# ChenWu98/cycle-diffusion

Measured on AMD Instinct MI355X. Metric: images/sec, SD-v1.4 512px CycleDiffusion 100+100 steps, 1/2/4/8 MI355X, higher is better.
Workload: dtype fp16; 1 GPU; C2: Stable-Diffusion-v1.4-shaped U-Net + KL-f8 VAE, 512x512, custom_steps=99 white_box_steps=100 eta=0.1 skip 0, 1 trial, encoder scale 1, decoder CFG 3; batch_per_gpu=4, global_batch=4, parallelism=dp1, steps_per_launch_set=5, launch_set_cap=16, launch_sets_in_flight_per_gpu=1, images_in_flight_per_gpu=20, distributed=single process, weights=synthetic(seed=0)

## Files before the change

cycle-diffusion_amd/_ffi.py:

```python
import ctypes as C
import os

import numpy as np

_HERE = os.path.dirname(os.path.abspath(__file__))
LIB_PATH = os.path.join(_HERE, "lib", "libcyclediff.so")

CD_NET_UNET_OPENAI, CD_NET_UNET_HO, CD_NET_VAE_KL, CD_NET_CLIP_TEXT, CD_NET_BERT_XTR = 1, 2, 3, 4, 5
CD_NET_OCLIP_TEXT, CD_NET_OCLIP_VISION, CD_NET_INCEPTION_FID = 6, 7, 8
CD_SCHED_DDIM, CD_SCHED_DDPM = 0, 1
CD_PREC_16, CD_PREC_F32, CD_PREC_F32X3 = 0, 1, 2
CD_MASK_QSAMPLE, CD_MASK_ENCODER = 0, 1
MASK_SOURCES = {"q_sample": CD_MASK_QSAMPLE, "encoder": CD_MASK_ENCODER}
ACT_NONE, ACT_SILU, ACT_GELU, ACT_GEGLU, ACT_QGELU, ACT_RELU = 0, 1, 2, 3, 4, 5


class NetDesc(C.Structure):
    _fields_ = [
        ("kind", C.c_int), ("image_size", C.c_int), ("in_channels", C.c_int), ("out_channels", C.c_int),
        ("model_channels", C.c_int), ("num_res_blocks", C.c_int),
        ("n_mult", C.c_int), ("channel_mult", C.c_int * 8),
        ("n_attn", C.c_int), ("attn", C.c_int * 8),
        ("num_heads", C.c_int), ("num_head_channels", C.c_int),
        ("use_spatial_transformer", C.c_int), ("context_dim", C.c_int), ("transformer_depth", C.c_int),
        ("use_scale_shift_norm", C.c_int), ("resblock_updown", C.c_int), ("conv_resample", C.c_int),
        ("z_channels", C.c_int), ("embed_dim", C.c_int), ("double_z", C.c_int),
        ("precision", C.c_int), ("n_embed", C.c_int), ("reserved", C.c_int * 6),
    ]


class StepCoef(C.Structure):
    _fields_ = [("sa", C.c_float), ("s1a", C.c_float), ("sap", C.c_float), ("dirc", C.c_float),
                ("sigma", C.c_float), ("r", C.c_float), ("t_mask", C.c_float), ("t", C.c_int32)]


STEP_COEF_DTYPE = np.dtype([("sa", "<f4"), ("s1a", "<f4"), ("sap", "<f4"), ("dirc", "<f4"), ("sigma", "<f4"),
                            ("r", "<f4"), ("t_mask", "<f4"), ("t", "<i4")])

_VP, _I, _F, _U64, _SZ, _I64 = C.c_void_p, C.c_int, C.c_float, C.c_uint64, C.c_size_t, C.c_int64

SIGNATURES = {
    "cd_last_error": [],
    "cd_version": [],
    "cd_act_format": [],
    "cd_engine_create": [_VP, _SZ, C.POINTER(_VP)],
    "cd_engine_destroy": [_VP],
    "cd_engine_synchronize": [_VP],
    "cd_engine_workspace_high_water": [_VP, C.POINTER(_SZ)],
    "cd_prof_enable": [_VP, _I],
    "cd_prof_collect": [_VP, C.POINTER(_I), C.POINTER(C.c_double), C.POINTER(C.c_double)],
    "cd_net_create": [_VP, C.POINTER(NetDesc), C.POINTER(_I)],
    "cd_net_param_count": [_VP, _I, C.POINTER(_I)],
    "cd_net_param_info": [_VP, _I, _I, C.c_char_p, _I, C.POINTER(_I), C.POINTER(_I64)],
    "cd_net_load_param": [_VP, _I, C.c_char_p, _VP, _I, C.POINTER(_I64)],
    "cd_net_missing_params": [_VP, _I, C.POINTER(_I), C.c_char_p, _I],
    "cd_unet_forward": [_VP, _I, _VP, _VP, _VP, _I, _I, _VP],
    "cd_text_encode": [_VP, _I, _VP, _I, _I, _VP],
    "cd_clip_text_features": [_VP, _I, _VP, _I, _I, _VP],
    "cd_clip_image_features": [_VP, _I, _VP, _I, _VP],
    "cd_inception_features": [_VP, _I, _VP, _I, _I, _VP],
    "cd_vae_encode": [_VP, _I, _VP, _VP, _U64, _I, _I, _I, _F, _VP],
    "cd_vae_decode": [_VP, _I, _VP, _I, _I, _F, _F, _F, _VP],
    "cd_dpm_encode": [_VP, _I, _I, _VP, _VP, _VP, _I, _F, _I, _I, _VP, _VP, _U64, _I, _VP],
    "cd_ddim_decode": [_VP, _I, _I, _VP, _I, _I, _VP, _VP, _I, _F, _I, _I, _VP, _VP, _U64, _VP],
    "cd_ddim_decode_v": [_VP, _I, _I, _VP, _I, _I, _VP, _VP, _I, _VP, _I, _I, _VP, _VP, _U64, _VP],
    "cd_ddim_invert": [_VP, _I, _I, _VP, _VP, _VP, _I, _F, _I, _I, _VP, _VP, _VP],
    "cd_cycle_translate": [_VP, _I, _I, _VP, _VP, _VP, _F, _VP, _VP, _F, _VP, _I, _I, _I, _I, _VP, _VP, _VP, _U64, _I, _VP,
                           _VP],
    "cd_ddim_decode_masked": [_VP, _I, _I, _VP, _I, _I, _VP, _VP, _I, _F, _VP, _I, _I, _VP, _VP, _U64, _VP, _VP, _I, _I, _VP, _VP,
                              _U64, _VP],
    "cd_cycle_translate_masked": [_VP, _I, _I, _VP, _VP, _VP, _F, _VP, _VP, _F, _VP, _I, _I, _I, _I, _VP, _VP, _VP, _U64, _I,
                                  _VP, _VP, _I, _I, _VP, _VP, _U64, _VP, _VP],
    "cd_pix_refine": [_VP, _I, _I, _VP, _I, _I, _VP, _VP, _U64],
    "cd_op_pack_conv_weight": [_VP, _VP, _I, _I, _I, _I, _I, C.POINTER(_VP), C.POINTER(_I), C.POINTER(_I)],
    "cd_op_free": [_VP, _VP],
    "cd_op_conv2d": [_VP, _VP, _I, _VP, _I, _I, _I, _I, _VP, _I, _I, _I, _I, _I, _I, _I, _VP, _VP, _VP, _I, _I, _VP],
    "cd_op_conv2d_16": [_VP, _VP, _I, _VP, _I, _I, _I, _I, _VP, _I, _I, _I, _I, _I, _I, _I, _VP, _VP, _VP, _I, _I, _VP,
                        _VP],
    "cd_op_last_gemm_config": [_VP] + [C.POINTER(_I)] * 5,
    "cd_op_groupnorm": [_VP, _VP, _I, _I, _I, _I, _I, _F, _VP, _VP, _VP, _I, _VP],
    "cd_op_layernorm": [_VP, _VP, _I, _I, _VP, _VP, _F, _VP],
    "cd_op_attention": [_VP, _VP, _VP, _VP, _I, _I, _I, _I, _I, _F, _I, _VP],
    "cd_op_softmax_rows": [_VP, _VP, _I64, _I, _VP],
    "cd_op_timestep_embedding": [_VP, _VP, _I, _I, _I, _VP],
    "cd_op_sched_step": [_VP, _I, _I, _VP, _VP, _VP, _VP, _I, _F, _VP, _VP, _I, _I, _I, _I, _VP],
    "cd_op_sched_step_masked": [_VP, _I, _VP, _VP, _VP, _I, _F, _VP, _VP, _VP, _I, _I, _F, _F, _VP, _I, _I, _I, _I, _VP, _I],
    "cd_op_bench_conv": [_VP, _I, _I, _I, _I, _I, _I, _I, _I, _I, _I, _I, _I, C.POINTER(C.c_float)],
    "cd_op_bench_mfma_sustained": [_VP, _I, C.POINTER(C.c_float), C.POINTER(C.c_float)],
    "cd_op_probe": [_VP, _I, _VP, _VP, _SZ],
}
_RESTYPES = {"cd_last_error": C.c_char_p}

_lib = None


class EngineError(RuntimeError):
    pass


def load_library(build_if_missing=True):
    global _lib
    if _lib is not None:
        return _lib
    if not os.path.exists(LIB_PATH):
        if not build_if_missing:
            raise EngineError("libcyclediff.so has not been built: run `python -c 'import __graft_entry__ as g; g.build()'`")
        import importlib.util
        spec = importlib.util.spec_from_file_location("_cd_build", os.path.join(_HERE, "build.py"))
        mod = importlib.util.module_from_spec(spec)
        spec.loader.exec_module(mod)
        mod.build()
    os.environ.setdefault("CYCLEDIFF_TUNE_DEFAULT", os.path.join(_HERE, "tune_gfx950.txt"))
    lib = C.CDLL(os.environ.get("CYCLEDIFF_LIB") or LIB_PATH)
    for name, args in SIGNATURES.items():
        fn = getattr(lib, name)
        fn.argtypes = args
        fn.restype = _RESTYPES.get(name, C.c_int)
    _lib = lib
    return lib


def check(rc):
    if rc != 0:
        raise EngineError(load_library().cd_last_error().decode("utf-8", "replace"))


def ptr(t):
    if t is None:
        return None
    if not t.is_contiguous():
        raise EngineError("tensor crossing the C ABI must be contiguous")
    return C.c_void_p(t.data_ptr())


def coef_array(rows):
    arr = np.zeros(len(rows), dtype=STEP_COEF_DTYPE)
    for i, r in enumerate(rows):
        arr[i] = tuple(r)
    return arr
```

cycle-diffusion_amd/csrc/capi.hip:

```cpp
#include <stdlib.h>
#include <string.h>
#include <unistd.h>

#include <algorithm>

#include "engine.h"

using namespace cd;

struct StepPacer {
  static constexpr int kAhead = 2, kRing = kAhead + 1;
  hipEvent_t ev[kRing] = {nullptr, nullptr, nullptr};
  long n = 0;
  bool enabled = true;
  void init() {
    const char* e = getenv("CYCLEDIFF_HOST_PACING");
    enabled = !(e && e[0] == '0');
    for (auto& x : ev) HIP_CHECK(hipEventCreateWithFlags(&x, hipEventBlockingSync | hipEventDisableTiming));
  }
  static void sleep_until_done(hipEvent_t e) {
    for (;;) {
      const hipError_t q = hipEventQuery(e);
      if (q == hipSuccess) return;
      if (q != hipErrorNotReady) HIP_CHECK(q);
// ... 698 lines not shown
    CD_CHECK(Dc > 0 && ctx_len > 0, "network has no cross-attention but a context was given");
    const size_t esz = f32 ? 4 : 2, per = (size_t)ctx_len * Dc;
    char* cx = (char*)h->arena.alloc((size_t)Bn * per * esz);
    auto put = [&](const float* src, int rows, size_t row0) {
      if (f32) HIP_CHECK(hipMemcpyAsync(cx + row0 * per * 4, src, (size_t)rows * per * 4, hipMemcpyDeviceToDevice, h->st));
      else launch_nchw_to_nhwc(h->st, src, (bf16_t*)cx + row0 * per, rows * ctx_len, Dc, 1, Dc, 1.f, 0.f, 0);
    };
    if (ge.cfg) { put(enc_ctx_uc, B, 0); put(enc_ctx_c, B, B); } else put(ge.ctx_single, B, 0);
    if (gd.cfg) { put(dec_ctx_uc, Bd, Ben); put(dec_ctx_c, Bd, Ben + Bd); } else put(gd.ctx_single, Bd, Ben);
    u->set_context(c, (const bf16_t*)cx, Bn, ctx_len);
  } else {
    CD_CHECK(u->desc.context_dim <= 0 || !u->desc.use_spatial_transformer, "network expects a cross-attention context");
  }
  const size_t esz = f32 ? 4 : 2;
  const int64_t chw = (int64_t)C * HW, n = (int64_t)B * chw;
  float* xt_e = (float*)h->arena.alloc((size_t)B * chw * 4);
  float* xt_d = (float*)h->arena.alloc((size_t)Bd * chw * 4);
  char* xin = (char*)h->arena.alloc((size_t)Bn * HW * cpad * esz);
  HIP_CHECK(hipMemsetAsync(xin, 0, (size_t)Bn * HW * cpad * esz, h->st));
  float* eh = (float*)h->arena.alloc((size_t)Bn * HW * out_ld * 4);
  const size_t row_in = (size_t)HW * cpad * esz;
  bf16_t* xin_e = f32 ? nullptr : (bf16_t*)xin;
  bf16_t* xin_d = f32 ? nullptr : (bf16_t*)(xin + (size_t)Ben * row_in);
  EpsHat eh_e, eh_d;
  eh_e.p = eh; eh_e.sb = (int64_t)HW * out_ld; eh_e.sc = 1; eh_e.sp = out_ld; eh_e.cfg = ge.cfg ? 1 : 0; eh_e.g = enc_guidance;
  eh_d = eh_e; eh_d.p = eh + (int64_t)Ben * HW * out_ld; eh_d.cfg = gd.cfg ? 1 : 0; eh_d.g = dec_guidance;
  eh_d.gvec = dec_guidance_per_sample;
  StepCoef* tab_e = upload_coef(h, coef_enc_host, K + 1);
  StepCoef* tab_d = upload_coef(h, coef_dec_host, K);
  const int64_t zbs = (int64_t)(K + 1) * chw;
  launch_init_xt(h->st, x0, noise, seed, 0u, xt_e, z_out, zbs, B, C, HW, tab_e, K, xin_e, cpad, ge.cfg ? 1 : 0);
  for (int j = 0; j < n_dec; ++j)
    HIP_CHECK(hipMemcpyAsync(xt_d + (int64_t)j * n, xt_e, (size_t)n * 4, hipMemcpyDeviceToDevice, h->st));
  const float2* qtab = nullptr;
  if (mk && mk->source == CD_MASK_QSAMPLE) qtab = (const float2*)upload_table(h, mk->qcoef_host, (size_t)K * 2 * sizeof(float));
  auto blend_of = [&](int k, int slot) {
    MaskBlend b = mask_blend_of(*mk, qtab, k, slot, (int64_t)Bd * chw);
    if (mk->source == CD_MASK_ENCODER) { b.src = xt_e; b.src_bmod = B; }
    return b;
  };
  if (mk) launch_mask_blend_init(h->st, xt_d, blend_of(K - 1, 0), Bd, C, HW, xin_d, cpad, gd.cfg ? 1 : 0);
  else if (!f32) launch_nchw_to_nhwc(h->st, xt_d, xin_d, Bd, C, HW, cpad, 1.f, 0.f, gd.cfg ? 1 : 0);
  const int dup_tail = (gd.cfg && !ge.cfg) ? Bd : 0;
  for (int i = 0; i < K; ++i) {
    const int k = K - 1 - i;
    if (f32) {
      float* xf = (float*)xin;
      launch_nchw_to_nhwc_f32(h->st, xt_e, xf, B, C, HW, cpad, 1.f, 0.f, u->x3 ? 1 : 0, h->overflow_dev);
      if (ge.cfg) launch_nchw_to_nhwc_f32(h->st, xt_e, xf + (size_t)B * HW * cpad, B, C, HW, cpad, 1.f, 0.f, u->x3 ? 1 : 0, h->overflow_dev);
      float* xd = xf + (size_t)Ben * HW * cpad;
      launch_nchw_to_nhwc_f32(h->st, xt_d, xd, Bd, C, HW, cpad, 1.f, 0.f, u->x3 ? 1 : 0, h->overflow_dev);
      if (gd.cfg) launch_nchw_to_nhwc_f32(h->st, xt_d, xd + (size_t)Bd * HW * cpad, Bd, C, HW, cpad, 1.f, 0.f, u->x3 ? 1 : 0, h->overflow_dev);
    }
    UNetIO io;
    io.xin = (const bf16_t*)xin; io.B = Bn; io.tab = tab_d; io.step = k; io.t_shared = true;
    io.dup_tail = dup_tail;
    io.out = eh; io.out_ld = out_ld;
    u->forward(c, io);
    const int is_last = (last_uses_x0 && k == 0) ? 1 : 0;
    const float* nz = (noise && !is_last) ? noise + (int64_t)(1 + i) * n : nullptr;
    float* zslot = z_out + (1 + i) * chw;
    launch_encode_step(h->st, sched_kind, x0, xt_e, eh_e, nz, seed, (uint32_t)(1 + i), zslot, zbs, B, C, HW, tab_e, nullptr, k,
                       is_last, xin_e, cpad, ge.cfg ? 1 : 0);
    if (mk)
      launch_decode_step_masked(h->st, xt_d, eh_d, zslot, zbs, nullptr, seed, (uint32_t)(0x1000 + i), Bd, C, HW, tab_d, nullptr, k,
                                xin_d, cpad, gd.cfg ? 1 : 0, n_dec > 1 ? B : 0, blend_of(k - 1, i + 1), k > 0 ? 1 : 0);
    else
    launch_decode_step(h->st, sched_kind, xt_d, eh_d, zslot, zbs, nullptr, seed, (uint32_t)(0x1000 + i), Bd, C, HW, tab_d,
                       nullptr, k, xin_d, cpad, gd.cfg ? 1 : 0, nullptr, n_dec > 1 ? B : 0);
    h->pacer.tick(h->st);
  }
  HIP_CHECK(hipMemcpyAsync(x_out, xt_d, (size_t)Bd * chw * 4, hipMemcpyDeviceToDevice, h->st));
}

int cd_cycle_translate(cd_handle h, int net, int sched_kind, const float* x0, const float* enc_ctx_c,
                       const float* enc_ctx_uc, float enc_guidance, const float* dec_ctx_c, const float* dec_ctx_uc,
                       float dec_guidance, const float* dec_guidance_per_sample, int ctx_len, int B, int n_dec, int K,
                       const cd_step_coef* coef_enc_host, const cd_step_coef* coef_dec_host, const float* noise,
                       uint64_t seed, int last_uses_x0, float* z_out, float* x_out) {
  CD_API_BEGIN
  enter_engine(h);
  cycle_translate_impl(h, net, sched_kind, x0, enc_ctx_c, enc_ctx_uc, enc_guidance, dec_ctx_c, dec_ctx_uc, dec_guidance,
                       dec_guidance_per_sample, ctx_len, B, n_dec, K, coef_enc_host, coef_dec_host, noise, seed, last_uses_x0,
                       z_out, x_out, nullptr);
  CD_API_END
}

int cd_cycle_translate_masked(cd_handle h, int net, int sched_kind, const float* x0, const float* enc_ctx_c,
                              const float* enc_ctx_uc, float enc_guidance, const float* dec_ctx_c, const float* dec_ctx_uc,
                              float dec_guidance, const float* dec_guidance_per_sample, int ctx_len, int B, int n_dec, int K,
                              const cd_step_coef* coef_enc_host, const cd_step_coef* coef_dec_host, const float* noise,
                              uint64_t seed, int last_uses_x0, const float* mask, const float* mask_x0, int B_mask,
                              int mask_source, const float* qsample_coef_host, const float* mask_noise, uint64_t mask_seed,
                              float* z_out, float* x_out) {
  CD_API_BEGIN
  enter_engine(h);
  MaskArgs mk;
  mk.mask = mask; mk.x0 = mask_x0; mk.B_mask = B_mask; mk.source = mask_source; mk.qcoef_host = qsample_coef_host;
  mk.noise = mask_noise; mk.seed = mask_seed;
  cycle_translate_impl(h, net, sched_kind, x0, enc_ctx_c, enc_ctx_uc, enc_guidance, dec_ctx_c, dec_ctx_uc, dec_guidance,
                       dec_guidance_per_sample, ctx_len, B, n_dec, K, coef_enc_host, coef_dec_host, noise, seed, last_uses_x0,
                       z_out, x_out, &mk);
  CD_API_END
}

int cd_pix_refine(cd_handle h, int net, int sched_kind, float* x, int B, int R, const cd_step_coef* coef_host,
                  const float* noise, uint64_t seed) {
  CD_API_BEGIN
  enter_engine(h);
  CD_CHECK(h && x && coef_host && B > 0 && R > 0, "bad argument");
  ArenaScope arena_scope(h->arena);
  SamplerState s = setup_sampler(h, net, nullptr, nullptr, 0, 1.f, B);
  s.tab = upload_coef(h, coef_host, R + 1);
  const int64_t n = (int64_t)B * s.C * s.HW;
  launch_init_xt(h->st, x, noise, seed, 0x2000u, s.xt, nullptr, 0, B, s.C, s.HW, s.tab, R, s.xin16(), s.cpad, 0);
  for (int i = 0; i < R; ++i) {
    const int k = R - 1 - i;
    run_unet(h, s, k);
    const float* nz = noise ? noise + (int64_t)(1 + i) * n : nullptr;
    launch_decode_step(h->st, sched_kind, s.xt, s.ehv, nullptr, 0, nz, seed, (uint32_t)(0x2001 + i), B, s.C,
                       s.HW, s.tab, nullptr, k, s.xin16(), s.cpad, 0, nullptr);
    h->pacer.tick(h->st);
  }
  HIP_CHECK(hipMemcpyAsync(x, s.xt, (size_t)n * 4, hipMemcpyDeviceToDevice, h->st));
  CD_API_END
}

int cd_op_pack_conv_weight(cd_handle h, const float* w_host, int N, int Cin, int KH, int KW, int geglu,
                           void** packed_dev, int* Npad, int* Cpad) {
  CD_API_BEGIN
  enter_engine(h);
  CD_CHECK(h && w_host && packed_dev, "bad argument");
  static int counter = 0;
  ConvW* c = h->op_params.new_conv(N, Cin, KH, KW, false, geglu != 0);
  const std::string name = "op." + std::to_string(counter++);
  h->op_params.conv_weight(name, c);
  int64_t shape[4] = {N, Cin, KH, KW};
  h->op_params.load(h->st, name, w_host, 4, shape);
  *packed_dev = c;
  if (Npad) *Npad = c->Npad;
  if (Cpad) *Cpad = c->Cpad;
  CD_API_END
}

int cd_op_free(cd_handle, void*) { return 0; }

static void op_conv2d(cd_handle h, const float* x0, int C0, const float* x1, int C1, int B, int H, int W,
                      const void* packed_w, int N, int KH, int KW, int stride, int pad, int asym_pad, int up,
                      const float* bias, const float* rowvec, const float* resid, int act, int tile, bool out16,
                      float* y, float* stats) {
  CD_CHECK(h && x0 && packed_w && y, "bad argument");
  ArenaScope arena_scope(h->arena);
  Ctx c = h->ctx();
  ConvW w = *(const ConvW*)packed_w;
  CD_CHECK(w.N == N && w.KH == KH && w.KW == KW, "packed weight does not match the call");
  w.b = const_cast<float*>(bias);
  const int c0p = x1 ? C0 : round_up(C0, 32);
  Act a0 = alloc_act(c, B, H, W, c0p);
  launch_nchw_to_nhwc(h->st, x0, a0.p, B, C0, H * W, c0p, 1.f, 0.f, 0);
  Act a1;
  if (x1) {
    a1 = alloc_act(c, B, H, W, C1);
    launch_nchw_to_nhwc(h->st, x1, a1.p, B, C1, H * W, C1, 1.f, 0.f, 0);
  }
  ConvOpts o; o.stride = stride; o.pad = pad; o.asym = asym_pad != 0; o.up = up != 0; o.tile = tile;
  if (act & 0x400) {
    CD_CHECK(out16 && conv_ln_fold_available(c, w, (int64_t)B * H * W) , "LayerNorm fold needs tile 30 shapes");
    o.ln_fold = true;
    act &= ~0x400;
  }
  o.act = act;
  o.out_f32 = !out16;
  o.want_stats = stats != nullptr;
  const int Hin = up ? 2 * H : H, Win = up ? 2 * W : W;
  const int Ho = asym_pad ? (Hin + 1 - KH) / stride + 1 : (Hin + 2 * pad - KH) / stride + 1;
  const int Wo = asym_pad ? (Win + 1 - KW) / stride + 1 : (Win + 2 * pad - KW) / stride + 1;
  const int Nout = w.geglu ? N / 2 : N;
  if (rowvec) { o.rowvec = rowvec; o.rowvec_ld = N; o.rows_per_vec = Ho * Wo; }
  Act r;
  if (resid) {
    r = alloc_act(c, B, Ho, Wo, Nout);
    launch_nchw_to_nhwc(h->st, resid, r.p, B, Nout, Ho * Wo, Nout, 1.f, 0.f, 0);
    o.resid = &r;
  }
  Act out = conv_fwd(c, w, a0, x1 ? &a1 : nullptr, o);
  launch_nhwc_to_nchw(h->st, out.p, out16 ? 0 : 1, out.ld, y, B, Nout, Ho * Wo, 1.f, 0.f);
  if (stats) {
    CD_CHECK(out.stats, "this convolution produces no GroupNorm statistics (GEGLU, or rows %% 32 != 0)");
    HIP_CHECK(hipMemcpyAsync(stats, out.stats, (size_t)(out.rows() / 32) * 2 * Nout * sizeof(float),
                             hipMemcpyDeviceToDevice, h->st));
  }
}

int cd_op_conv2d(cd_handle h, const float* x0, int C0, const float* x1, int C1, int B, int H, int W,
                 const void* packed_w, int N, int KH, int KW, int stride, int pad, int asym_pad, int up,
                 const float* bias, const float* rowvec, const float* resid, int act, int tile, float* y) {
  CD_API_BEGIN
  enter_engine(h);
  op_conv2d(h, x0, C0, x1, C1, B, H, W, packed_w, N, KH, KW, stride, pad, asym_pad, up, bias, rowvec, resid, act, tile,
            false, y, nullptr);
  CD_API_END
}

int cd_op_conv2d_16(cd_handle h, const float* x0, int C0, const float* x1, int C1, int B, int H, int W,
                    const void* packed_w, int N, int KH, int KW, int stride, int pad, int asym_pad, int up,
                    const float* bias, const float* rowvec, const float* resid, int act, int tile, float* y,
                    float* stats) {
  CD_API_BEGIN
  enter_engine(h);
  op_conv2d(h, x0, C0, x1, C1, B, H, W, packed_w, N, KH, KW, stride, pad, asym_pad, up, bias, rowvec, resid, act, tile,
            true, y, stats);
  CD_API_END
}

int cd_op_last_gemm_config(cd_handle h, int* tile_id, int* bk, int* splitk, int* chm, int* tile_group) {
  CD_API_BEGIN
  CD_CHECK(h, "bad argument");
  const GemmLaunchInfo li = conv_gemm_last_launch();
  if (tile_id) *tile_id = li.tile_id;
  if (bk) *bk = li.bk;
  if (splitk) *splitk = li.splitk;
  if (chm) *chm = li.chm;
  if (tile_group) *tile_group = li.tile_group;
  CD_API_END
}

int cd_op_groupnorm(cd_handle h, const float* x, int B, int C, int H, int W, int G, float eps,
                    const float* gamma, const float* beta, const float* film, int silu, float* y) {
  CD_API_BEGIN
  enter_engine(h);
  CD_CHECK(h && x && y && G == 32, "bad argument (G must be 32)");
  ArenaScope arena_scope(h->arena);
  Ctx c = h->ctx();
  Act a = alloc_act(c, B, H, W, C);
  launch_nchw_to_nhwc(h->st, x, a.p, B, C, H * W, C, 1.f, 0.f, 0);
  GNW w; w.g = const_cast<float*>(gamma); w.b = const_cast<float*>(beta); w.C = C; w.eps = eps;
  Act o = groupnorm_fwd(c, w, a, nullptr, silu != 0, film, film ? 2 * C : 0);
  launch_nhwc_to_nchw(h->st, o.p, 0, o.ld, y, B, C, H * W, 1.f, 0.f);
  CD_API_END
}

int cd_op_layernorm(cd_handle h, const float* x, int rows, int C, const float* gamma, const float* beta,
                    float eps, float* y) {
  CD_API_BEGIN
  enter_engine(h);
  CD_CHECK(h && x && y, "bad argument");
  ArenaScope arena_scope(h->arena);
  bf16_t* a = (bf16_t*)h->arena.alloc((size_t)rows * C * 2);
  bf16_t* o = (bf16_t*)h->arena.alloc((size_t)rows * C * 2);
  launch_nchw_to_nhwc(h->st, x, a, rows, C, 1, C, 1.f, 0.f, 0);
  launch_layernorm(h->st, a, C, o, C, rows, C, gamma, beta, eps);
  launch_nhwc_to_nchw(h->st, o, 0, C, y, rows, C, 1, 1.f, 0.f);
  CD_API_END
}

int cd_op_attention(cd_handle h, const float* q, const float* k, const float* v, int B, int H, int Tq,
                    int Tk, int D, float scale, int use_transpose_kernel, float* o) {
  CD_API_BEGIN
  enter_engine(h);
  CD_CHECK(h && q && k && v && o, "bad argument");
  ArenaScope arena_scope(h->arena);
  const int C = H * D, Tpad = round_up(Tk, 64);
  bf16_t* qb = (bf16_t*)h->arena.alloc((size_t)B * Tq * C * 2);
  bf16_t* kb = (bf16_t*)h->arena.alloc((size_t)B * Tk * C * 2);
  bf16_t* vb = (bf16_t*)h->arena.alloc((size_t)B * Tk * C * 2);
  bf16_t* ob = (bf16_t*)h->arena.alloc((size_t)B * Tq * C * 2);
  launch_nchw_to_nhwc(h->st, q, qb, B * Tq, C, 1, C, 1.f, 0.f, 0);
  launch_nchw_to_nhwc(h->st, k, kb, B * Tk, C, 1, C, 1.f, 0.f, 0);
  launch_nchw_to_nhwc(h->st, v, vb, B * Tk, C, 1, C, 1.f, 0.f, 0);
  AttnParams p;
  p.q = qb; p.k = kb; p.o = ob; p.B = B; p.H = H; p.Tq = Tq; p.Tk = Tk; p.D = D;
  p.ldq = C; p.ldk = C; p.ldo = C; p.q_bs = (int64_t)Tq * C; p.k_bs = (int64_t)Tk * C; p.o_bs = (int64_t)Tq * C;
  p.scale = scale;
  if (use_transpose_kernel) {
    bf16_t* vt = (bf16_t*)h->arena.alloc((size_t)B * C * Tpad * 2);
    launch_transpose_v(h->st, vb, C, (int64_t)Tk * C, vt, B, H, Tk, D, D, Tpad);
    p.vt = vt; p.vt_dpad = D; p.vt_tpad = Tpad;
  } else {
    p.v = vb; p.ldv = C; p.v_bs = (int64_t)Tk * C;
  }
  launch_attention(h->st, p);
  launch_nhwc_to_nchw(h->st, ob, 0, C, o, B * Tq, C, 1, 1.f, 0.f);
  CD_API_END
}

int cd_op_softmax_rows(cd_handle h, const float* s, int64_t rows, int cols, float* p) {
  CD_API_BEGIN
  enter_engine(h);
  CD_CHECK(h && s && p, "bad argument");
  ArenaScope arena_scope(h->arena);
  bf16_t* pb = (bf16_t*)h->arena.alloc((size_t)rows * cols * 2);
  launch_softmax_rows(h->st, s, cols, pb, cols, rows, cols);
  launch_nhwc_to_nchw(h->st, pb, 0, cols, p, (int)rows, cols, 1, 1.f, 0.f);
  CD_API_END
}

int cd_op_timestep_embedding(cd_handle h, const float* t, int B, int dim, int mode, float* out) {
  CD_API_BEGIN
  enter_engine(h);
  CD_CHECK(h && t && out, "bad argument");
  launch_timestep_embedding(h->st, nullptr, nullptr, 0, t, out, B, dim, mode);
  CD_API_END
}

int cd_op_sched_step(cd_handle h, int mode, int sched_kind, const cd_step_coef* coef_host, const float* x0,
                     float* xt, const float* eps_hat, int cfg, float guidance, const float* noise,
                     const float* eps_in, int is_last, int B, int C, int HW, float* z_slot) {
  CD_API_BEGIN
  enter_engine(h);
  CD_CHECK(h && coef_host && xt, "bad argument");
  ArenaScope arena_scope(h->arena);
  StepCoef* tab = upload_coef(h, coef_host, 1);
  const int64_t chw = (int64_t)C * HW;
  EpsHat eh; eh.p = eps_hat; eh.sb = chw; eh.sc = HW; eh.sp = 1; eh.cfg = cfg; eh.g = guidance;
  if (mode == 0) {
    launch_init_xt(h->st, x0, noise, 0, 0, xt, z_slot, chw, B, C, HW, tab, 0, nullptr, 0, 0);
  } else if (mode == 1) {
    launch_encode_step(h->st, sched_kind, x0, xt, eh, noise, 0, 0, z_slot, chw, B, C, HW, tab, nullptr, 0,
                       is_last, nullptr, 0, 0);
  } else {
    launch_decode_step(h->st, sched_kind, xt, eh, eps_in, chw, noise, 0, 0, B, C, HW, tab, nullptr, 0, nullptr,
                       0, 0, nullptr);
  }
  HIP_CHECK(hipStreamSynchronize(h->st));
  CD_API_END
}

int cd_op_sched_step_masked(cd_handle h, int mode, const cd_step_coef* coef_host, float* x, const float* eps_hat, int cfg,
                            float guidance, const float* eps_in, const float* mask, const float* src, int B_mask,
                            int mask_source, float qa, float qb, const float* mask_noise, int blend, int B, int C, int HW,
                            void* xin16_out, int cfg_dup) {
  CD_API_BEGIN
  enter_engine(h);
  CD_CHECK(h && x && mask && src && B > 0 && C > 0 && HW > 0, "bad argument");
  CD_CHECK(B_mask > 0 && B % B_mask == 0, "mask shape mismatch: %d mask rows for a batch of %d", B_mask, B);
  CD_CHECK(mode == 0 || (coef_host && eps_hat), "bad argument");
  ArenaScope arena_scope(h->arena);
  const int64_t chw = (int64_t)C * HW;
  MaskBlend mk;
  mk.mask = mask; mk.src = src; mk.mask_bmod = mk.src_bmod = B_mask; mk.noise = mask_noise;
  if (mask_source == CD_MASK_QSAMPLE) {
    CD_CHECK(mask_noise, "q_sample mode needs the noise tensor here");
    const float q[2] = {qa, qb};
    mk.qtab = (const float2*)upload_table(h, q, sizeof(q));
  }
  if (mode == 0) {
    launch_mask_blend_init(h->st, x, mk, B, C, HW, (bf16_t*)xin16_out, C, cfg_dup);
  } else {
    StepCoef* tab = upload_coef(h, coef_host, 1);
    EpsHat eh; eh.p = eps_hat; eh.sb = chw; eh.sc = HW; eh.sp = 1; eh.cfg = cfg; eh.g = guidance;
    launch_decode_step_masked(h->st, x, eh, eps_in, chw, nullptr, 0, 0, B, C, HW, tab, nullptr, 0, (bf16_t*)xin16_out, C,
                              cfg_dup, 0, mk, blend);
  }
  HIP_CHECK(hipStreamSynchronize(h->st));
  CD_API_END
}

}

namespace {
__global__ void k_probe_mfma(float* out) {
  const int lane = threadIdx.x & 63;
  bf16x8 a = {0, 0, 0, 0, 0, 0, 0, 0}, b = {0, 0, 0, 0, 0, 0, 0, 0};
  f32x16 acc;
// ... 167 lines not shown
```

cycle-diffusion_amd/csrc/conv_gemm.hip:

```cpp
#include <stdio.h>
#include <stdlib.h>
#include <string.h>

#include <algorithm>
#include <map>
#include <mutex>
#include <string>

#include "common.h"
#include "kernels.h"

namespace cd {

namespace gemm_detail {

#ifndef CD_EPI_STORE_AUX
#define CD_EPI_STORE_AUX 0
#endif
#ifndef CD_EPI_RESID_AUX
#define CD_EPI_RESID_AUX 0
#endif

typedef const __attribute__((address_space(1))) void* gptr_t;
typedef __attribute__((address_space(3))) void* lptr_t;

template <int BM, int BN, int BK, int WM, int WN, int NSTAGE>
struct TileCfg {
  static constexpr int NW = WM * WN;
  static constexpr int CPR = BK / 8;
  static constexpr int RPI = 64 / CPR;
  static constexpr int A_IPW = BM / RPI / NW;
  static constexpr int B_IPW = BN / RPI / NW;
  static constexpr int LPT = A_IPW + B_IPW;
  static constexpr int TM = BM / WM, TN = BN / WN;
  static constexpr int MT = TM / 32, NT = TN / 32;
  static constexpr int KS = BK / 16;
  static constexpr int SWZ_SHIFT = (CPR == 8) ? 1 : 2;
  static constexpr int CW = TN >= 64 ? 64 : TN;
  static constexpr int EPI_LD = CW + 4;
  static constexpr int PF = (MT * NT >= 8) ? 1 : 2;
  static constexpr int A_BYTES = BM * BK * 2, B_BYTES = BN * BK * 2;
  static constexpr int STAGE_BYTES = A_BYTES + B_BYTES;
  static constexpr int EPI_BYTES = NW * TM * EPI_LD * 4;
  static constexpr int LDS_BYTES = STAGE_BYTES * NSTAGE > EPI_BYTES ? STAGE_BYTES * NSTAGE : EPI_BYTES;
  static constexpr int TAB_BIAS_I = (BN / 4 + 63) / 64;
  static constexpr int TAB_RV_I = ((BM / 32) * (BN / 4) + 63) / 64;
  static constexpr bool HAS_TAB = LDS_BYTES + (TAB_BIAS_I + TAB_RV_I) * 1024 <= 160 * 1024;
  static constexpr int TAB_BYTES = HAS_TAB ? (TAB_BIAS_I + TAB_RV_I) * 1024 : 0;
  static_assert(NW == 4 || NW == 8 || NW == 16, "4, 8 or 16 waves");
  static_assert(A_IPW >= 1 && B_IPW >= 1, "tile too small for the wave count");
  static_assert(A_IPW * RPI * NW == BM && B_IPW * RPI * NW == BN, "tile rows must split evenly over waves");
  static_assert(MT >= 1 && NT >= 1, "wave tile");
  static_assert(NSTAGE >= 2 && NSTAGE <= 8, "ring depth");
  static_assert((NSTAGE - 2) * LPT <= 63, "vmcnt field");
  static_assert(LDS_BYTES + TAB_BYTES <= 160 * 1024, "LDS");
};

template <int N>
__device__ __forceinline__ void wait_vmcnt_barrier() {
  asm volatile("s_waitcnt vmcnt(%0)\n\ts_barrier" ::"n"(N) : "memory");
}

#ifdef CD_PROBE
__device__ __forceinline__ unsigned long long probe_time() {
  unsigned long long t;
  asm volatile("s_memtime %0\n\ts_waitcnt lgkmcnt(0)" : "=s"(t)::"memory");
  return t;
}
__device__ __forceinline__ unsigned long long probe_realtime() {
  unsigned long long t;
  asm volatile("s_memrealtime %0\n\ts_waitcnt lgkmcnt(0)" : "=s"(t)::"memory");
  return t;
}
#define CD_PROBE_ONLY(...) __VA_ARGS__
#else
#define CD_PROBE_ONLY(...)
#endif

__device__ __forceinline__ __amdgpu_buffer_rsrc_t uniform_rsrc(const void* base, int bytes) {
  const uint64_t u = (uint64_t)base;
  const uint32_t lo = (uint32_t)__builtin_amdgcn_readfirstlane((int)(uint32_t)u);
  const uint32_t hi = (uint32_t)__builtin_amdgcn_readfirstlane((int)(uint32_t)(u >> 32));
  return __builtin_amdgcn_make_buffer_rsrc((void*)(((uint64_t)hi << 32) | lo), 0, __builtin_amdgcn_readfirstlane(bytes), 0x00020000);
}

__device__ __forceinline__ bool fast_epilogue(const ConvGemmParams& p) {
  return p.act == ACT_NONE && !p.out_f32 && !p.resid_f32 && (p.N & 7) == 0 && (p.out_ld & 7) == 0 &&
         (((uintptr_t)p.out | (uintptr_t)p.resid | (uintptr_t)p.rowvec) & 15) == 0 && (p.o_bs & 7) == 0 &&
         (!p.resid || (p.resid_ld & 7) == 0) &&
         (!p.rowvec || ((p.rowvec_ld & 3) == 0 && (p.rows_per_vec >= p.M || (p.rows_per_vec & 31) == 0)));
}

template <int BM, int BN, int BK, int WM, int WN, int NSTAGE, bool CHM = false>
__global__ __launch_bounds__(64 * WM * WN, (WM * WN == 4 && BK == 32 && NSTAGE == 3 && BM * BN >= 128 * 256) ? 2 : 1) void k_conv_gemm(ConvGemmParams p) {
#if defined(__HIP_DEVICE_COMPILE__)
  using T = TileCfg<BM, BN, BK, WM, WN, NSTAGE>;
  constexpr int CPR = T::CPR, RPI = T::RPI, A_IPW = T::A_IPW, B_IPW = T::B_IPW, NW = T::NW;
  constexpr int MT = T::MT, NT = T::NT, KS = T::KS, TM = T::TM, TN = T::TN, LPT = T::LPT;
  extern __shared__ __attribute__((aligned(16))) char smem[];

  const int tid = threadIdx.x;
  const int lane = tid & 63;
  const int wave = __builtin_amdgcn_readfirstlane(tid >> 6);
  const int wm = wave / WN, wn = wave % WN;
  if constexpr (WM * WN == 4 && BK == 32 && NSTAGE == 3 && BM * BN >= 128 * 256) {
    if (p.dephase_ticks > 0 && (int)(blockIdx.x + gridDim.x * (blockIdx.y + gridDim.y * blockIdx.z)) < 2 * p.num_cus) {
      unsigned hwid;
      asm volatile("s_getreg_b32 %0, hwreg(HW_REG_HW_ID)" : "=s"(hwid));
      if (tid == 0) *(volatile int*)smem = (int)(hwid & 1u);
      __syncthreads();
      const int odd = *(volatile int*)smem;
      __syncthreads();
      if (odd) {
        unsigned long long t0, t1;
        asm volatile("s_memtime %0\n\ts_waitcnt lgkmcnt(0)" : "=s"(t0)::"memory");
        do {
          __builtin_amdgcn_s_sleep(32);
          asm volatile("s_memtime %0\n\ts_waitcnt lgkmcnt(0)" : "=s"(t1)::"memory");
        } while ((long long)(t1 - t0) < (long long)p.dephase_ticks);
      }
    }
  }
  CD_PROBE_ONLY(
  const unsigned long long pr_rt0 = probe_realtime();
  unsigned long long pr_t0 = probe_time(), pr_prol = 0, pr_first = 0, pr_wait = 0, pr_comp = 0, pr_maxw = 0, pr_loop = 0,
                     pr_drain = 0, pr_stage = 0, pr_rows = 0, pr_issued = 0, pr_last = 0;
  unsigned* pr_log = (unsigned*)(smem + T::LDS_BYTES + T::TAB_BYTES) + wave * 64;
  if (lane < 64) pr_log[lane] = 0;)

  const int tiles_n = (p.N + BN - 1) / BN;
  const int tiles_m = (p.M + BM - 1) / BM;
  const int ntiles = tiles_m * tiles_n;
  int tile;
  {
    const int bid = blockIdx.x;
    const int q = ntiles >> 3, r = ntiles & 7;
    const int xcd = bid & 7, loc = bid >> 3;
    tile = (xcd < r ? xcd * (q + 1) : r * (q + 1) + (xcd - r) * q) + loc;
  }
  const bool nmajor = (int64_t)p.N * p.Ktot > (int64_t)p.B * p.Hs * p.Ws * (p.C0 + p.C1);
  int tm, tn;
  if (p.tile_group > 0) {
    const int width = p.tile_group * tiles_n;
    const int grp = tile / width, within = tile - grp * width;
    const int first_m = grp * p.tile_group;
    const int gsz = (tiles_m - first_m) < p.tile_group ? (tiles_m - first_m) : p.tile_group;
    tn = within / gsz; tm = first_m + (within - tn * gsz);
  } else if (nmajor) { tn = tile / tiles_m; tm = tile - tn * tiles_m; }
  else { tm = tile / tiles_n; tn = tile - tm * tiles_n; }
  const int m0 = tm * BM, n0 = tn * BN;
  const int zb = blockIdx.z;

  constexpr unsigned kRange = 0x7fffffffu, kInvalid = 0x80000000u;
  const int HWo = p.Hout * p.Wout;
  const bool pow2 = ((HWo & (HWo - 1)) == 0) && ((p.Wout & (p.Wout - 1)) == 0);
  const int sh_hw = 31 - __builtin_clz(HWo), sh_w = 31 - __builtin_clz(p.Wout);
  int b_first = pow2 ? (m0 >> sh_hw) : (m0 / HWo);
  CD_PROBE_ONLY(if (p.dbg & 4) b_first = 0;)
  const int64_t samp0 = (int64_t)b_first * p.Hs * p.Ws;
  const bf16_t* base0 = p.src0 + (int64_t)zb * p.a_bs + samp0 * p.ld0;
  const bf16_t* base1 = p.src1 ? p.src1 + (int64_t)zb * p.a_bs + samp0 * p.ld1 : base0;
  const __amdgpu_buffer_rsrc_t rsw =
      __builtin_amdgcn_make_buffer_rsrc((void*)(p.wgt + (int64_t)zb * p.w_bs), 0, kRange, 0x00020000);

  const int srow = lane / CPR;
  const int pchunk = lane % CPR;
  int a_iy0[A_IPW], a_ix0[A_IPW], a_boff[A_IPW], a_lc8[A_IPW];
  unsigned a_voff[A_IPW];
  unsigned a_mk[A_IPW], a_base[A_IPW];
#pragma unroll
  for (int i = 0; i < A_IPW; ++i) {
    const int row = (i * NW + wave) * RPI + srow;
    int m = m0 + row;
    CD_PROBE_ONLY(if (p.dbg & 4) m = (m0 & 0x3ff) + row;)
    a_lc8[i] = (pchunk ^ ((row >> T::SWZ_SHIFT) & (CPR - 1))) * 8;
    a_voff[i] = kInvalid;
    a_mk[i] = 0; a_base[i] = 0;
    if (m < p.M) {
      int b, oy, ox;
      if (pow2) {
        b = m >> sh_hw;
        const int rem = m & (HWo - 1);
        oy = rem >> sh_w; ox = rem & (p.Wout - 1);
      } else {
        b = m / HWo;
        const int rem = m - b * HWo;
        oy = rem / p.Wout; ox = rem - oy * p.Wout;
      }
      a_iy0[i] = oy * p.stride - p.pad_t;
      a_ix0[i] = ox * p.stride - p.pad_l;
      a_boff[i] = (b - b_first) * p.Hs * p.Ws;
    } else {
      a_iy0[i] = -(1 << 28);
      a_ix0[i] = 0;
      a_boff[i] = 0;
    }
    if constexpr (CHM) {
      unsigned mk = 0;
      for (int r = 0; r < p.KH; ++r) mk |= ((unsigned)(a_iy0[i] + r) < (unsigned)p.Hin ? 1u : 0u) << r;
      for (int q = 0; q < p.KW; ++q) mk |= ((unsigned)(a_ix0[i] + q) < (unsigned)p.Win ? 1u : 0u) << (8 + q);
      a_mk[i] = mk;
    }
  }
  unsigned b_voff[B_IPW];
#pragma unroll
  for (int i = 0; i < B_IPW; ++i) {
    const int row = (i * NW + wave) * RPI + srow;
    const int lchunk = pchunk ^ ((row >> T::SWZ_SHIFT) & (CPR - 1));
    int nrow = n0 + row;
    if (nrow >= p.N) nrow = p.N - 1;
    b_voff[i] = (unsigned)((nrow * (p.ldw ? p.ldw : p.Ktot) + lchunk * 8) * 2);
  }

  const int Ctot = p.C0 + p.C1;
  const int nk = p.Ktot / BK;
  const int nsplit = gridDim.y, sidx = blockIdx.y;
  const int kper = (nk + nsplit - 1) / nsplit;
  const int kt0 = sidx * kper;
  const int kt1 = (kt0 + kper < nk) ? kt0 + kper : nk;
  int kr, kss, kc;
  if constexpr (CHM) {
    const int ntaps = p.KH * p.KW;
    const int slice = kt0 / ntaps, tap = kt0 - slice * ntaps;
    kc = slice * BK;
    kr = tap / p.KW;
    kss = tap - kr * p.KW;
  } else {
    const int k_el = kt0 * BK;
    const int tap = k_el / Ctot;
    kc = k_el - tap * Ctot;
    kr = tap / p.KW;
    kss = tap - kr * p.KW;
  }
  bool st_force = true;

  char* As = smem;
  char* Bs = smem + NSTAGE * T::A_BYTES;

  bool st_live = false;
  int st_soffa = 0, st_soffb = 0;
  const bf16_t* st_base = base0;
  auto prepare = [&](int kt) {
    st_live = kt < kt1;
    const int c_kc = kc, c_kr = kr, c_kss = kss;
    if constexpr (CHM) {
      const bool wk = c_kss + 1 >= p.KW;
      const bool wr = wk && (c_kr + 1 >= p.KH);
      kss = wk ? 0 : c_kss + 1;
      kr = wr ? 0 : c_kr + (wk ? 1 : 0);
      kc = c_kc + (wr ? BK : 0);
      if (st_live) {
        const int ld = (c_kc < p.C0) ? p.ld0 : p.ld1;
        if (st_force || ((c_kr | c_kss) == 0 && (c_kc == 0 || c_kc == p.C0))) {
          st_force = false;
#pragma unroll
          for (int i = 0; i < A_IPW; ++i) {
            const int pix = a_boff[i] + a_iy0[i] * p.Ws + a_ix0[i];
            a_base[i] = (unsigned)((pix * ld + a_lc8[i]) * 2);
          }
        }
        const unsigned dt = (unsigned)((c_kr * p.Ws + c_kss) * ld * 2);
#pragma unroll
        for (int i = 0; i < A_IPW; ++i) {
          const unsigned ok = (a_mk[i] >> c_kr) & (a_mk[i] >> (8 + c_kss)) & 1u;
          a_voff[i] = ok ? a_base[i] + dt : kInvalid;
        }
      }
    } else {
      kc += BK;
      if (kc >= Ctot) {
        kc = 0;
        if (++kss >= p.KW) { kss = 0; ++kr; }
      }
      if (st_live && (c_kc == 0 || c_kc == p.C0 || st_force)) {
        st_force = false;
        const int ld = (c_kc < p.C0) ? p.ld0 : p.ld1;
#pragma unroll
        for (int i = 0; i < A_IPW; ++i) {
          int iy = a_iy0[i] + c_kr, ix = a_ix0[i] + c_kss;
          const bool ok = ((unsigned)iy < (unsigned)p.Hin) && ((unsigned)ix < (unsigned)p.Win);
          if (p.up) { iy >>= 1; ix >>= 1; }
          const int pix = a_boff[i] + iy * p.Ws + ix;
          a_voff[i] = ok ? (unsigned)((pix * ld + a_lc8[i]) * 2) : kInvalid;
        }
      }
    }
    const bool first = c_kc < p.C0;
    st_base = first ? base0 : base1;
    st_soffa = (first ? c_kc : c_kc - p.C0) * 2;
    st_soffb = st_live ? (CHM ? ((c_kr * p.KW + c_kss) * Ctot + c_kc) * 2 : kt * (BK * 2)) : 0;
  };
  auto issue = [&](int idx, int buf) {
    if (idx < A_IPW) {
      const __amdgpu_buffer_rsrc_t rsa = __builtin_amdgcn_make_buffer_rsrc((void*)st_base, 0, kRange, 0x00020000);
      char* l = As + buf * T::A_BYTES + ((idx * NW + wave) * RPI) * (BK * 2);
      __builtin_amdgcn_raw_ptr_buffer_load_lds(rsa, (lptr_t)l, 16, st_live ? a_voff[idx < A_IPW ? idx : 0] : kInvalid,
                                               st_soffa, 0, 0);
    } else {
      const int i = idx - A_IPW;
      char* l = Bs + buf * T::B_BYTES + ((i * NW + wave) * RPI) * (BK * 2);
      __builtin_amdgcn_raw_ptr_buffer_load_lds(rsw, (lptr_t)l, 16, st_live ? b_voff[i < B_IPW ? i : 0] : kInvalid,
                                               st_soffb, 0, 0);
    }
  };

  f32x16 acc[MT][NT];
#pragma unroll
  for (int i = 0; i < MT; ++i)
#pragma unroll
    for (int j = 0; j < NT; ++j)
#pragma unroll
      for (int r = 0; r < 16; ++r) acc[i][j][r] = 0.0f;

  const int frow = lane & 31;
  const int fhalf = lane >> 5;

  constexpr int PF = T::PF, SYNC = KS - PF, NMF = MT * NT, HALF = NMF / 2;
  constexpr int SPREAD = (NSTAGE == 2) ? 1 : KS;
  static_assert(SYNC >= 0 && (NSTAGE - 1) * LPT <= 63, "fragment prefetch depth / vmcnt field");
#pragma unroll
  for (int s = 0; s < NSTAGE; ++s) {
    prepare(kt0 + s);
#pragma unroll
    for (int l = 0; l < LPT; ++l) issue(l, s);
  }
  constexpr int TAB_N = T::TAB_BIAS_I + T::TAB_RV_I;
  constexpr int TABI = T::HAS_TAB ? (TAB_N + NW - 1) / NW : 0;
  if constexpr (TABI > 0) {
    const bool fe = fast_epilogue(p);
    const bool tb = (fe || p.act == ACT_GEGLU) && p.bias != nullptr;
    char* tab = smem + T::LDS_BYTES;
    const __amdgpu_buffer_rsrc_t rsb = __builtin_amdgcn_make_buffer_rsrc(
        (void*)(tb ? (const void*)p.bias : (const void*)p.wgt), 0, tb ? p.N * 4 : 0, 0x00020000);
    const __amdgpu_buffer_rsrc_t rsv = __builtin_amdgcn_make_buffer_rsrc(
        (void*)((fe && p.rowvec) ? (const void*)p.rowvec : (const void*)p.wgt), 0, (fe && p.rowvec) ? kRange : 0, 0x00020000);
    const unsigned rpv = (unsigned)p.rows_per_vec;
    const bool rpv_pow2 = (rpv & (rpv - 1)) == 0;
    const int rpv_sh = 31 - __builtin_clz(rpv | 1u);
#pragma unroll
    for (int i = 0; i < TABI; ++i) {
      const int j = (i * NW + wave) % TAB_N;
      if (j < T::TAB_BIAS_I) {
        const int c4 = j * 64 + lane;
// ... 364 lines not shown
            __builtin_amdgcn_raw_buffer_store_b128((u32x4e){pk.x, pk.y, pk.z, pk.w}, rs_o,
                                                   vo_out + (unsigned)((rb * 32 + ps * 16) * p.out_ld * 2), 0, 0);
          }
        }
        CD_PROBE_ONLY(pr_rows += probe_time() - pr_c1;)
        continue;
      }
      float bias_v[8];
#pragma unroll
      for (int e = 0; e < 8; ++e) bias_v[e] = (p.bias && e < nvalid) ? p.bias[n + e] : 0.0f;
      float ssum[8], ssq[8];
#pragma unroll
      for (int e = 0; e < 8; ++e) { ssum[e] = 0.f; ssq[e] = 0.f; }
      for (int r0 = 0; r0 < TM; r0 += rpp) {
        const int row = r0 + vr;
        const int m = m0 + wm * TM + row;
        if (row < TM && m < p.M && n < p.N) {
        float v[8];
        {
          const f32x4 lo = *(const f32x4*)(E + row * T::EPI_LD + col);
          const f32x4 hi = *(const f32x4*)(E + row * T::EPI_LD + col + 4);
          v[0] = lo[0]; v[1] = lo[1]; v[2] = lo[2]; v[3] = lo[3];
          v[4] = hi[0]; v[5] = hi[1]; v[6] = hi[2]; v[7] = hi[3];
        }
#pragma unroll
        for (int e = 0; e < 8; ++e) v[e] += bias_v[e];
        int on = n;
        if (geglu) {
          float gt[8];
          const f32x4 lo = *(const f32x4*)(E + row * T::EPI_LD + col + 32);
          const f32x4 hi = *(const f32x4*)(E + row * T::EPI_LD + col + 36);
          gt[0] = lo[0]; gt[1] = lo[1]; gt[2] = lo[2]; gt[3] = lo[3];
          gt[4] = hi[0]; gt[5] = hi[1]; gt[6] = hi[2]; gt[7] = hi[3];
#pragma unroll
          for (int e = 0; e < 8; ++e) {
            const float gg = gt[e] + (p.bias ? p.bias[n + 32 + e] : 0.0f);
            v[e] = v[e] * gelu_fast(gg);
          }
          on = (n / 64) * 32 + (n % 64);
        } else {
          if (p.rowvec) {
            const int rvi = (p.rows_per_vec >= p.M) ? 0 : m / p.rows_per_vec;
            const float* rv = p.rowvec + (int64_t)rvi * p.rowvec_ld + n;
#pragma unroll
            for (int e = 0; e < 8; ++e) if (e < nvalid) v[e] += rv[e];
          }
          if (p.act == ACT_SILU) {
#pragma unroll
            for (int e = 0; e < 8; ++e) v[e] = silu_f(v[e]);
          } else if (p.act == ACT_GELU) {
#pragma unroll
            for (int e = 0; e < 8; ++e) {
              v[e] = gelu_fast(v[e]);
              if constexpr (NW == 16) {
                if (e == 3) asm volatile("" : "+v"(v[0]), "+v"(v[1]), "+v"(v[2]), "+v"(v[3]), "+v"(v[4]), "+v"(v[5]), "+v"(v[6]), "+v"(v[7]));
              }
            }
          } else if (p.act == ACT_QGELU) {
#pragma unroll
            for (int e = 0; e < 8; ++e) v[e] = v[e] / (1.0f + __expf(-1.702f * v[e]));
          } else if (p.act == ACT_RELU) {
#pragma unroll
            for (int e = 0; e < 8; ++e) v[e] = fmaxf(v[e], 0.0f);
          }
        }
        if (p.resid && p.resid_f32) {
          const float* rp = (const float*)p.resid + (int64_t)zb * p.o_bs + (int64_t)m * p.resid_ld + on;
          if (nvalid == 8 && ((p.resid_ld & 3) == 0)) {
            const f32x4 r0 = *(const f32x4*)rp, r1 = *(const f32x4*)(rp + 4);
#pragma unroll
            for (int e = 0; e < 4; ++e) { v[e] += r0[e]; v[4 + e] += r1[e]; }
          } else {
#pragma unroll
            for (int e = 0; e < 8; ++e) if (e < nvalid) v[e] += rp[e];
          }
        } else if (p.resid) {
          const bf16_t* rp = p.resid + (int64_t)zb * p.o_bs + (int64_t)m * p.resid_ld + on;
          if (nvalid == 8 && ((p.resid_ld & 7) == 0)) {
            float rr[8];
            unpack8(*(const uint4*)rp, rr);
#pragma unroll
            for (int e = 0; e < 8; ++e) v[e] += rr[e];
          } else {
#pragma unroll
            for (int e = 0; e < 8; ++e) if (e < nvalid) v[e] += bf2f(rp[e]);
          }
        }
        CD_PROBE_ONLY(if (!(p.dbg & 1)))
        if (p.out_f32) {
          float* op = (float*)outp + (int64_t)m * p.out_ld + on;
          if (nvalid == 8 && ((p.out_ld & 3) == 0)) {
            *(f32x4*)op = (f32x4){v[0], v[1], v[2], v[3]};
            *(f32x4*)(op + 4) = (f32x4){v[4], v[5], v[6], v[7]};
          } else {
#pragma unroll
            for (int e = 0; e < 8; ++e) if (e < nvalid) op[e] = v[e];
          }
        } else {
          bf16_t* op = (bf16_t*)outp + (int64_t)m * p.out_ld + on;
          if (nvalid == 8 && ((p.out_ld & 7) == 0)) {
            *(uint4*)op = pack8(v);
          } else {
#pragma unroll
            for (int e = 0; e < 8; ++e) if (e < nvalid) op[e] = f2bf(v[e]);
          }
        }
        CD_PROBE_ONLY(if (p.dbg & 1) { if (v[0] == 1.2345e-33f) ((float*)outp)[0] = v[1] + v[2] + v[3] + v[4] + v[5] + v[6] + v[7]; })
        if (p.stats) {
#pragma unroll
          for (int e = 0; e < 8; ++e) { ssum[e] += v[e]; ssq[e] += v[e] * v[e]; }
        }
        }
        if (p.stats && ((r0 + rpp) & 31) == 0) {
          for (int o = vpr; o < 64; o <<= 1) {
#pragma unroll
            for (int e = 0; e < 8; ++e) { ssum[e] += __shfl_xor(ssum[e], o); ssq[e] += __shfl_xor(ssq[e], o); }
          }
          const int rb = (m0 + wm * TM + r0 + rpp - 32) >> 5;
          if (vr == 0 && n < p.N && (rb << 5) < p.M) {
            float* sp = p.stats + ((int64_t)zb * ((p.M + 31) >> 5) + rb) * 2 * p.N + n;
#pragma unroll
            for (int e = 0; e < 8; ++e) if (e < nvalid) { sp[e] = ssum[e]; sp[p.N + e] = ssq[e]; }
          }
#pragma unroll
          for (int e = 0; e < 8; ++e) { ssum[e] = 0.f; ssq[e] = 0.f; }
        }
      }
      CD_PROBE_ONLY(pr_rows += probe_time() - pr_c1;)
    }
  }
  CD_PROBE_ONLY({
    pr_issued = probe_time();
    asm volatile("s_waitcnt vmcnt(0)" ::: "memory");
    const unsigned long long pr_done = probe_time();
    if (p.probe) {
      unsigned hwid, xcc;
      asm volatile("s_getreg_b32 %0, hwreg(HW_REG_HW_ID)" : "=s"(hwid));
      asm volatile("s_getreg_b32 %0, hwreg(HW_REG_XCC_ID)" : "=s"(xcc));
      unsigned long long* o = p.probe + ((size_t)(blockIdx.x + gridDim.x * (blockIdx.y + gridDim.y * blockIdx.z)) * NW + wave) * kProbeWords;
      if (lane == 0) {
        o[0] = pr_t0; o[1] = pr_prol; o[2] = pr_first; o[3] = pr_wait; o[4] = pr_comp; o[5] = pr_maxw; o[6] = pr_loop;
        o[7] = pr_drain; o[8] = pr_stage; o[9] = pr_rows; o[10] = pr_issued; o[11] = pr_done; o[12] = kt1 - kt0;
        o[13] = ((unsigned long long)xcc << 32) | hwid; o[14] = pr_rt0; o[15] = probe_realtime();
      }
      ((unsigned*)(o + 16))[lane] = pr_log[lane];
    }
  })
#endif
}


inline bool takes_channel_major(const ConvGemmParams& p) {
  const int64_t a_bytes = (int64_t)p.B * p.Hs * p.Ws * (p.C0 + p.C1) * 2;
  return p.korder != 0 && p.KH * p.KW > 1 && p.KH <= 8 && p.KW <= 8 && !p.up &&
         (p.korder == 2 || (p.Hs * p.Ws >= 4096 && a_bytes >= (32ll << 20)));
}

template <int BM, int BN, int BK, int WM, int WN, int NSTAGE>
int launch_cfg(hipStream_t st, const ConvGemmParams& p) {
  using T = TileCfg<BM, BN, BK, WM, WN, NSTAGE>;
  const int tiles = ceil_div(p.M, BM) * ceil_div(p.N, BN);
  const int split = p.splitk > 1 ? p.splitk : 1;
#ifdef CD_PROBE
  constexpr int kLds = T::LDS_BYTES + T::TAB_BYTES + T::NW * 256;
#else
  constexpr int kLds = T::LDS_BYTES + T::TAB_BYTES;
#endif
  const bool chm = takes_channel_major(p);
  static PerDeviceOnce attr_once;
  auto kern0 = k_conv_gemm<BM, BN, BK, WM, WN, NSTAGE, false>;
  auto kern1 = k_conv_gemm<BM, BN, BK, WM, WN, NSTAGE, true>;
  attr_once([&]() {
    HIP_CHECK(hipFuncSetAttribute((const void*)kern0, hipFuncAttributeMaxDynamicSharedMemorySize, kLds));
    HIP_CHECK(hipFuncSetAttribute((const void*)kern1, hipFuncAttributeMaxDynamicSharedMemorySize, kLds));
  });
  auto kern = chm ? kern1 : kern0;
  if (split > 1) {
    const SplitKWorkspace& ws = g_conv_splitk;
    CD_CHECK(p.sk_scratch && p.sk_flags, "conv_gemm: split-K without workspace");
    CD_CHECK((size_t)tiles * p.nbatch * split * BM * BN * 4 <= ws.scratch_bytes && tiles * p.nbatch <= ws.nflags,
             "conv_gemm: split-K workspace too small");
  }
  hipLaunchKernelGGL(kern, dim3(tiles, split, p.nbatch), dim3(64 * T::NW), kLds, st, p);
  return 0;
}

struct CfgInfo { int id, BM, BN, TN; const char* name; };
const CfgInfo kCfgs[] = {
    {1, 128, 128, 64, "128x128 w2x2 s2"},
    {2, 128, 64, 64, "128x64 w4x1 s2"},
    {3, 64, 64, 32, "64x64 w2x2 s2"},
    {4, 128, 128, 64, "128x128 w2x2 s3"},
    {5, 256, 128, 64, "256x128 w4x2 s3"},
    {6, 128, 256, 64, "128x256 w2x4 s3"},
    {7, 128, 64, 64, "128x64 w4x1 s4"},
    {8, 64, 64, 32, "64x64 w2x2 s4"},
    {9, 256, 64, 64, "256x64 w8x1 s4"},
    {10, 128, 128, 64, "128x128 w2x2 s4"},
    {11, 64, 128, 64, "64x128 w2x2 s4"},
    {12, 128, 64, 64, "128x64 w4x1 s3"},
    {13, 256, 64, 64, "256x64 w8x1 s3"},
    {14, 128, 128, 64, "128x128 w4x2 s3"},
    {15, 64, 64, 32, "64x64 w2x2 s8"},
    {16, 128, 64, 64, "128x64 w4x1 s6"},
    {17, 64, 128, 64, "64x128 w2x2 s6"},
    {18, 256, 128, 32, "256x128 w4x4 s3"},
    {19, 256, 128, 64, "256x128 w8x2 s3"},
    {20, 256, 320, 160, "256x320 w4x2 s2"},
    {21, 128, 320, 160, "128x320 w2x2 s2"},
    {22, 256, 256, 128, "256x256 w4x2 s2"},
    {23, 128, 320, 160, "128x320 w4x2 s2"},
    {24, 128, 256, 128, "128x256 w2x2 s3 bk32 x2/CU"},
    {25, 256, 128, 128, "256x128 w4x1 s3 bk32 x2/CU"},
};
inline bool cfg_needs_bk64(int id) { return id == 20 || id == 21 || id == 23; }
constexpr int kNumCfgs = sizeof(kCfgs) / sizeof(kCfgs[0]);
inline int bk32_alias(int id) { return id == 9 ? 7 : id == 13 ? 12 : id == 18 ? 5 : id == 19 ? 5 : id; }
inline bool cfg_always_bk32(int id) { return id == 24 || id == 25; }

}
thread_local SplitKWorkspace g_conv_splitk;
thread_local unsigned long long* g_conv_probe = nullptr;
namespace gemm_detail {

template <int BK>
int dispatch(hipStream_t st, const ConvGemmParams& p, int id) {
  switch (id) {
    case 1: return launch_cfg<128, 128, BK, 2, 2, 2>(st, p);
    case 2: return launch_cfg<128, 64, BK, 4, 1, 2>(st, p);
    case 3: return launch_cfg<64, 64, BK, 2, 2, 2>(st, p);
    case 4: return launch_cfg<128, 128, BK, 2, 2, 3>(st, p);
    case 5: return launch_cfg<256, 128, BK, 4, 2, 3>(st, p);
    case 6: return launch_cfg<128, 256, BK, 2, 4, 3>(st, p);
    case 7: return launch_cfg<128, 64, BK, 4, 1, 4>(st, p);
    case 8: return launch_cfg<64, 64, BK, 2, 2, 4>(st, p);
    case 9:
      if constexpr (BK == 64) return launch_cfg<256, 64, 64, 8, 1, 4>(st, p);
      else return launch_cfg<128, 64, 32, 4, 1, 4>(st, p);
     
    case 10: return launch_cfg<128, 128, BK, 2, 2, 4>(st, p);
    case 11: return launch_cfg<64, 128, BK, 2, 2, 4>(st, p);
    case 12: return launch_cfg<128, 64, BK, 4, 1, 3>(st, p);
    case 13:
      if constexpr (BK == 64) return launch_cfg<256, 64, 64, 8, 1, 3>(st, p);
      else return launch_cfg<128, 64, 32, 4, 1, 3>(st, p);
     
    case 14: return launch_cfg<128, 128, BK, 4, 2, 3>(st, p);
    case 15: return launch_cfg<64, 64, BK, 2, 2, 8>(st, p);
    case 16: return launch_cfg<128, 64, BK, 4, 1, 6>(st, p);
    case 17: return launch_cfg<64, 128, BK, 2, 2, 6>(st, p);
    case 18:
      if constexpr (BK == 64) return launch_cfg<256, 128, 64, 4, 4, 3>(st, p);
      else return launch_cfg<256, 128, 32, 4, 2, 3>(st, p);
     
    case 19:
      if constexpr (BK == 64) return launch_cfg<256, 128, 64, 8, 2, 3>(st, p);
      else return launch_cfg<256, 128, 32, 4, 2, 3>(st, p);
     
    case 20: case 21: case 22: case 23:
      if constexpr (BK == 64) {
        if (id == 20) return launch_cfg<256, 320, 64, 4, 2, 2>(st, p);
        else if (id == 21) return launch_cfg<128, 320, 64, 2, 2, 2>(st, p);
        else if (id == 22) return launch_cfg<256, 256, 64, 4, 2, 2>(st, p);
        else return launch_cfg<128, 320, 64, 4, 2, 2>(st, p);
      } else {
        if (id == 22) return launch_cfg<256, 256, 32, 4, 2, 4>(st, p);
        CD_CHECK(false, "conv_gemm: tile configuration %d needs channel counts that are multiples of 64", id);
      }
      return 0;
    case 24: return launch_cfg<128, 256, 32, 2, 2, 3>(st, p);
    case 25: return launch_cfg<256, 128, 32, 4, 1, 3>(st, p);
    default: CD_CHECK(false, "conv_gemm: unknown tile configuration %d", id);
  }
  return 0;
}

thread_local const char* g_last_cfg = "";
thread_local GemmLaunchInfo g_last_launch;

int device_cu_count() {
  static std::atomic<int> ncu_of[64];
  int dev = 0;
  if (hipGetDevice(&dev) != hipSuccess) return 256;
  int n = ncu_of[dev & 63].load(std::memory_order_relaxed);
  if (!n) {
    hipDeviceProp_t prop;
    n = (hipGetDeviceProperties(&prop, dev) == hipSuccess && prop.multiProcessorCount > 0) ? prop.multiProcessorCount : 256;
    ncu_of[dev & 63].store(n, std::memory_order_relaxed);
  }
  return n;
}

int pick_config(const ConvGemmParams& p) {
  const int64_t ncu = device_cu_count();
  const int64_t t128 = (int64_t)ceil_div(p.M, 128) * ceil_div(p.N, 128) * p.nbatch;
  const int64_t t12864 = (int64_t)ceil_div(p.M, 128) * ceil_div(p.N, 64) * p.nbatch;
  if (p.act == ACT_GEGLU) return (2 * t128 >= 3 * ncu) ? 1 : 2;
  if (2 * t128 >= 3 * ncu && p.N % 128 == 0) return 1;
  if (t128 >= 2 * ncu) return 1;
  if (t12864 >= ncu) return 2;
  return 3;
}

}
using namespace gemm_detail;

const char* conv_gemm_last_config() { return g_last_cfg; }
GemmLaunchInfo conv_gemm_last_launch() { return g_last_launch; }

thread_local KernelProfiler* g_conv_prof = nullptr;

void KernelProfiler::next_pair(hipEvent_t* a, hipEvent_t* b, double fl, const std::string& what) {
  labels.push_back(what);
  if (used + 2 > (int)events.size()) {
    const size_t old = events.size();
    events.resize(old + 1024);
    for (size_t i = old; i < events.size(); ++i) HIP_CHECK(hipEventCreate(&events[i]));
  }
  *a = events[used]; *b = events[used + 1];
  used += 2;
  flops.push_back(fl);
}
void KernelProfiler::collect(int* launches, double* total_ms, double* total_flops) {
  double ms = 0, fl = 0;
  for (int i = 0; i + 1 < used; i += 2) {
    HIP_CHECK(hipEventSynchronize(events[i + 1]));
    float t = 0;
    HIP_CHECK(hipEventElapsedTime(&t, events[i], events[i + 1]));
    ms += t; fl += flops[i / 2];
    if (verbose) {
      auto& e = per_shape[labels[i / 2]];
      e.n += 1; e.ms += t; e.flops += flops[i / 2];
    }
  }
  if (verbose) {
    std::vector<std::pair<std::string, Entry>> v(per_shape.begin(), per_shape.end());
    std::sort(v.begin(), v.end(), [](const auto& x, const auto& y) { return x.second.ms > y.second.ms; });
    fprintf(stderr, "[conv_gemm] %d launches %.3f ms %.1f TFLOP/s\n", used / 2, ms, fl / ms * 1e-9);
    for (auto& kv : v)
      fprintf(stderr, "  %-58s n=%4d %8.3f ms %7.1f us/launch %7.1f TF/s\n", kv.first.c_str(), kv.second.n,
              kv.second.ms, kv.second.ms / kv.second.n * 1e3, kv.second.flops / kv.second.ms * 1e-9);
    per_shape.clear();
  }
  *launches = used / 2; *total_ms = ms; *total_flops = fl;
  used = 0; flops.clear(); labels.clear();
}
KernelProfiler::~KernelProfiler() { for (auto e : events) (void)hipEventDestroy(e); }

ConvTuner g_conv_tuner;

namespace {
struct ShapeKey {
  int v[14];
  bool operator<(const ShapeKey& o) const { return memcmp(v, o.v, sizeof(v)) < 0; }
};
const char* tune_cache_path() {
  static const char* p = getenv("CYCLEDIFF_TUNE_CACHE");
  return (p && p[0]) ? p : nullptr;
}
std::map<ShapeKey, int>& tune_table() {
  static std::map<ShapeKey, int> t;
  static bool loaded = false;
  if (!loaded) {
    loaded = true;
    const char* paths[2] = {getenv("CYCLEDIFF_TUNE_DEFAULT"), tune_cache_path()};
    for (const char* path : paths) {
      if (!path || !path[0]) continue;
      if (FILE* f = fopen(path, "r")) {
        ShapeKey k; int val;
        for (;;) {
          int got = 0;
          for (int i = 0; i < 14; ++i) got += fscanf(f, "%d", &k.v[i]);
          got += fscanf(f, "%d", &val);
          if (got != 15) break;
          t[k] = val;
        }
        fclose(f);
      }
    }
  }
  return t;
}
void tune_cache_append(const ShapeKey& k, int val) {
  const char* path = tune_cache_path();
  if (!path) return;
  if (FILE* f = fopen(path, "a")) {
    for (int i = 0; i < 14; ++i) fprintf(f, "%d ", k.v[i]);
    fprintf(f, "%d\n", val);
    fclose(f);
  }
}

std::mutex g_tune_mu;

int tuned_config(hipStream_t st, const ConvGemmParams& p, bool k64) {
  std::lock_guard<std::mutex> lock(g_tune_mu);
  ConvTuner& tu = g_conv_tuner;
  if (!tu.enabled || !tu.scratch) return pick_config(p);
  const int nout = (p.act == ACT_GEGLU) ? p.N / 2 : p.N;
  const size_t need = (size_t)p.M * nout * (p.out_f32 ? 4 : 2) * p.nbatch;
  if (need > tu.scratch_bytes) return pick_config(p);
  ShapeKey key = {{p.M, p.N, p.Ktot, p.KH, p.C0, p.C1, p.stride, p.up, p.act, p.nbatch, p.out_f32, p.Hout, p.Wout,
                   (p.resid ? 1 : 0) | (p.rowvec ? 2 : 0)}};
  auto& tab = tune_table();
  auto it = tab.find(key);
  if (it != tab.end()) return it->second;
  ConvGemmParams q = p;
  q.out = tu.scratch; q.out_ld = nout; q.o_bs = (int64_t)p.M * nout;
  if (p.resid && p.nbatch > 1) q.resid = nullptr;
  hipEvent_t e0, e1;
  HIP_CHECK(hipEventCreate(&e0)); HIP_CHECK(hipEventCreate(&e1));
  int best = pick_config(p);
  float best_ms = 1e30f;
  const SplitKWorkspace& sk = g_conv_splitk;
  const int64_t t128 = (int64_t)ceil_div(p.M, 128) * ceil_div(p.N, 128) * p.nbatch;
  const int nk = p.Ktot / (k64 ? 64 : 32);
  static const int kSplits[] = {1, 2, 3, 4, 6, 8, 12, 16};
  static const bool tune_splitk = [] { const char* e = getenv("CYCLEDIFF_TUNE_SPLITK"); return e && e[0] == '1'; }();
  const int nbk = (k64 && p.Ktot <= 1280) ? 2 : 1;
  for (int bi = 0; bi < nbk; ++bi)
  for (int i = 0; i < kNumCfgs; ++i)
  for (int si = 0; si < 8; ++si) {
    const CfgInfo& c = kCfgs[i];
    const int split = kSplits[si];
    const bool use64 = k64 && bi == 0;
    if (bi == 1 && split > 1) continue;
    if (split > 1 && !tune_splitk) continue;
    if (p.act == ACT_GEGLU && (c.TN % 64) != 0) continue;
    if (c.BM >= 256 && p.M < 256) continue;
    if (cfg_needs_bk64(c.id) && !use64) continue;
    if ((c.id == 24 || c.id == 25) && bi == 1) continue;
    if (c.BN == 320 && (p.N % 320) != 0) continue;
    const int64_t tiles = (int64_t)ceil_div(p.M, c.BM) * ceil_div(p.N, c.BN) * p.nbatch;
    if (split > 1) {
      if (!sk.scratch || tiles >= device_cu_count() || nk < 4 * split || tiles * split > 2048) continue;
      if ((size_t)tiles * split * c.BM * c.BN * 4 > sk.scratch_bytes || tiles > sk.nflags) continue;
    }
    q.splitk = split; q.sk_scratch = sk.scratch; q.sk_flags = sk.flags;
    auto run = [&]() { if (use64) dispatch<64>(st, q, c.id); else dispatch<32>(st, q, c.id); };
    auto timed = [&](int reps) {
      HIP_CHECK(hipEventRecord(e0, st));
      for (int r = 0; r < reps; ++r) run();
      HIP_CHECK(hipEventRecord(e1, st));
      HIP_CHECK(hipEventSynchronize(e1));
      float t = 0;
      HIP_CHECK(hipEventElapsedTime(&t, e0, e1));
      return t / reps;
    };
    run();
    float ms = timed(2);
    const int reps = (int)fminf(24.f, fmaxf(2.f, 0.4f / fmaxf(ms, 1e-3f)));
    ms = fminf(ms, fminf(timed(reps), timed(reps)));
    if (ms < best_ms) { best_ms = ms; best = c.id | (split << 8) | ((k64 && !use64) ? (1 << 16) : 0); }
  }
  if (lin_stream_supports(q)) {
    auto timed = [&](int reps) {
      HIP_CHECK(hipEventRecord(e0, st));
      for (int r = 0; r < reps; ++r) launch_lin_stream(st, q);
      HIP_CHECK(hipEventRecord(e1, st));
      HIP_CHECK(hipEventSynchronize(e1));
      float t = 0;
      HIP_CHECK(hipEventElapsedTime(&t, e0, e1));
      return t / reps;
    };
    q.splitk = 0;
    launch_lin_stream(st, q);
    float ms = timed(2);
    const int reps = (int)fminf(24.f, fmaxf(2.f, 0.4f / fmaxf(ms, 1e-3f)));
    ms = fminf(ms, fminf(timed(reps), timed(reps)));
    if (ms < best_ms) { best_ms = ms; best = kLinStreamTile; }
  }
  (void)hipEventDestroy(e0); (void)hipEventDestroy(e1);
  tab[key] = best;
  tune_cache_append(key, best);
  ++tu.shapes_tuned;
  return best;
}
}

void launch_conv_gemm(hipStream_t st, const ConvGemmParams& p) {
  const int Ctot = p.C0 + p.C1;
  CD_CHECK(p.C0 % 32 == 0 && p.C1 % 32 == 0, "conv_gemm: channels must be multiples of 32 (C0=%d C1=%d)", p.C0, p.C1);
  CD_CHECK(p.Ktot == p.KH * p.KW * Ctot, "conv_gemm: Ktot mismatch");
  CD_CHECK(p.zeros != nullptr, "conv_gemm: zero page missing");
  CD_CHECK(p.M > 0 && p.N > 0, "conv_gemm: empty problem");
  CD_CHECK(((uintptr_t)p.src0 & 15) == 0 && ((uintptr_t)p.wgt & 15) == 0, "conv_gemm: 16-B alignment");
  CD_CHECK((p.ld0 % 8) == 0 && (p.src1 == nullptr || (p.ld1 % 8) == 0), "conv_gemm: ld must be a multiple of 8");
  if (p.act == ACT_GEGLU) CD_CHECK(p.N % 64 == 0, "GEGLU needs packed N %% 64 == 0");
  bool k64 = (p.C0 % 64 == 0) && (p.C1 % 64 == 0);
  if (p.ln_fold) CD_CHECK(p.tile == kLinStreamTile, "conv_gemm: a LayerNorm-folded layer runs on lin_stream only");
  int id = p.tile ? p.tile : tuned_config(st, p, k64);
  if (id & (1 << 16)) k64 = false;
  ConvGemmParams pk = p;
  id &= 0xffff;
  if ((id >> 8) > 1) pk.splitk = id >> 8;
  id &= 0xff;
  if (pk.splitk > 1 && !pk.sk_scratch) { pk.sk_scratch = g_conv_splitk.scratch; pk.sk_flags = g_conv_splitk.flags; }
  pk.probe = g_conv_probe;
  static const int korder_env = [] { const char* e = getenv("CYCLEDIFF_KORDER"); return e ? atoi(e) : -1; }();
  if (korder_env >= 0) pk.korder = korder_env;
  static const int tg_env = [] { const char* e = getenv("CYCLEDIFF_TILE_GROUP"); return e ? atoi(e) : 8; }();
  static const int tg_min_n = [] { const char* e = getenv("CYCLEDIFF_TILE_GROUP_MIN_N"); return e ? atoi(e) : 2048; }();
  if (tg_env > 0 && p.N >= tg_min_n && p.nbatch == 1) pk.tile_group = tg_env;
#ifdef CD_PROBE
  if (const char* e = getenv("CYCLEDIFF_PROBE_DBG")) pk.dbg = atoi(e);
  static const int dephase_env = [] { const char* e = getenv("CYCLEDIFF_DEPHASE_TICKS"); return e ? atoi(e) : 0; }();
  pk.dephase_ticks = dephase_env;
  pk.num_cus = device_cu_count();
  if (pk.dbg & 2) pk.stats = nullptr;
#endif
  static const CfgInfo kLinStreamCfg = {kLinStreamTile, 256, 64, 64, "lin_stream 256 x N, K = 320"};
  const CfgInfo* ci = nullptr;
  if (id == kLinStreamTile) {
    if (lin_stream_supports(pk)) ci = &kLinStreamCfg;
    else { CD_CHECK(!p.tile, "conv_gemm: lin_stream does not support this problem"); id = pick_config(p); }
  }
  for (int i = 0; i < kNumCfgs && !ci; ++i) if (kCfgs[i].id == id) ci = &kCfgs[i];
  CD_CHECK(ci, "conv_gemm: unknown tile configuration %d", id);
  if (p.act == ACT_GEGLU && (ci->TN % 64) != 0) { id = 2; ci = &kCfgs[1]; }
  if (cfg_needs_bk64(id)) CD_CHECK(k64, "conv_gemm: tile configuration %d needs channel counts that are multiples of 64", id);
  g_last_cfg = ci->name;
  {
    GemmLaunchInfo li;
    const bool lin = id == kLinStreamTile;
    li.bk = (lin || (k64 && !cfg_always_bk32(id))) ? 64 : 32;
    li.tile_id = li.bk == 32 ? bk32_alias(id) : id;
    li.splitk = pk.splitk > 1 ? pk.splitk : 1;
    li.chm = !lin && takes_channel_major(pk) ? 1 : 0;
    li.tile_group = lin ? 0 : pk.tile_group;
    g_last_launch = li;
  }
  static const bool trace = [] { const char* e = getenv("CYCLEDIFF_GEMM_TRACE"); return e && e[0] == '1'; }();
  if (trace) {
    const bool chm = id != kLinStreamTile && takes_channel_major(pk);
    fprintf(stderr, "[gemm_trace] %d %d %d %d %d %d %d %d %d %d %d %d | %s x%d\n", p.M, p.N, p.Ktot, p.KH, p.stride, p.up,
            p.src1 ? 1 : 0, p.nbatch, p.act, p.resid ? 1 : 0, p.out_f32, chm ? 1 : 0, ci->name, pk.splitk > 1 ? pk.splitk : 1);
  }
  KernelProfiler* prof = g_conv_prof;
  hipEvent_t e0 = nullptr, e1 = nullptr;
  if (prof && prof->enabled) {
    char what[112] = "";
    if (prof->verbose)
      snprintf(what, sizeof(what), "M%d N%d K%d k%d s%d%s%s z%d act%d | %s x%d", p.M, p.N, p.Ktot, p.KH, p.stride,
               p.up ? " up" : "", p.src1 ? " cat" : "", p.nbatch, p.act, ci->name, pk.splitk > 1 ? pk.splitk : 1);
    if (prof->verbose && !k64) strncat(what, " bk32", sizeof(what) - strlen(what) - 1);
    prof->next_pair(&e0, &e1, 2.0 * (double)p.M * (double)p.N * (double)p.Ktot * (double)p.nbatch * p.prof_flop_scale,
                    what);
    (void)hipEventRecord(e0, st);
  }
  struct Closer {
    hipEvent_t e; hipStream_t s;
    ~Closer() { if (e) (void)hipEventRecord(e, s); }
  } closer{e1, st};
  if (id == kLinStreamTile) launch_lin_stream(st, pk);
  else if (k64) dispatch<64>(st, pk, id);
  else dispatch<32>(st, pk, id);
}

int conv_gemm_num_configs() { return kNumCfgs; }
const char* conv_gemm_config_name(int id) {
  for (int i = 0; i < kNumCfgs; ++i) if (kCfgs[i].id == id) return kCfgs[i].name;
  return "?";
}

__global__ void k_repack_weight(const float* __restrict__ w, bf16_t* __restrict__ out, int N, int Cin,
                                int KH, int KW, int Npad, int Cpad, int geglu, int64_t src_row_offset) {
  const int64_t total = (int64_t)Npad * KH * KW * Cpad;
  for (int64_t i = blockIdx.x * (int64_t)blockDim.x + threadIdx.x; i < total;
       i += (int64_t)gridDim.x * blockDim.x) {
    const int c = (int)(i % Cpad);
    int64_t t = i / Cpad;
    const int s = (int)(t % KW); t /= KW;
    const int r = (int)(t % KH); t /= KH;
    const int np = (int)t;
    int n = np;
    if (geglu) {
      const int blk = np / 64, within = np % 64;
      n = (within < 32) ? blk * 32 + within : N / 2 + blk * 32 + (within - 32);
    }
    float v = 0.0f;
    if (np < N && c < Cin) v = w[(((int64_t)(n + src_row_offset) * Cin + c) * KH + r) * KW + s];
    out[i] = f2bf(v);
  }
}

void launch_repack_weight(hipStream_t st, const float* w, bf16_t* out, int N, int Cin, int KH,
                          int KW, int Npad, int Cpad, int geglu, int64_t src_row_offset) {
  const int64_t total = (int64_t)Npad * KH * KW * Cpad;
  int grid = (int)((total + 255) / 256);
  if (grid > 4096) grid = 4096;
  hipLaunchKernelGGL(k_repack_weight, dim3(grid), dim3(256), 0, st, w, out, N, Cin, KH, KW, Npad,
                     Cpad, geglu, src_row_offset);
}

}
```

cycle-diffusion_amd/csrc/elementwise.hip:

```cpp
#include "common.h"
#include <mutex>

#include "kernels.h"

namespace cd {

namespace {

__device__ inline void philox_round2(uint32_t (&c)[4], uint32_t k0, uint32_t k1) {
  const uint32_t M0 = 0xD2511F53u, M1 = 0xCD9E8D57u;
  uint32_t hi0 = __umulhi(M0, c[0]), lo0 = M0 * c[0];
  uint32_t hi1 = __umulhi(M1, c[2]), lo1 = M1 * c[2];
  uint32_t n0 = hi1 ^ c[1] ^ k0, n1 = lo1, n2 = hi0 ^ c[3] ^ k1, n3 = lo0;
  c[0] = n0; c[1] = n1; c[2] = n2; c[3] = n3;
}
__device__ inline float philox_normal2(uint64_t seed, uint32_t stream, uint64_t idx) {
  uint32_t c[4] = {(uint32_t)(idx >> 1), (uint32_t)(idx >> 33), stream, 0x9E3779B9u};
  uint32_t k0 = (uint32_t)seed, k1 = (uint32_t)(seed >> 32);
#pragma unroll
  for (int i = 0; i < 10; ++i) { philox_round2(c, k0, k1); k0 += 0x9E3779B9u; k1 += 0xBB67AE85u; }
  float u1 = ((float)(c[0] >> 8) + 0.5f) * (1.0f / 16777216.0f);
  float u2 = ((float)(c[1] >> 8) + 0.5f) * (1.0f / 16777216.0f);
  float rad = sqrtf(-2.0f * __logf(u1));
  float ang = 6.28318530717958647692f * u2;
// ... 46 lines not shown
    const float f = expf(-9.210340371976184f * (float)k / (float)half);
    const float a = t * f;
    o[k] = cosf(a);
    o[half + k] = sinf(a);
  } else {
    const float e = 9.210340371976184f / (float)(half - 1);
    const float f = expf((float)k * -e);
    const float a = t * f;
    o[k] = sinf(a);
    o[half + k] = cosf(a);
  }
  if ((dim & 1) && k == 0) o[dim - 1] = 0.f;
}

__global__ __launch_bounds__(256) void k_vec_linear(const float* __restrict__ x, int ldx,
                                                    const float* __restrict__ W,
                                                    const float* __restrict__ bias, float* __restrict__ y,
                                                    int ldy, int B, int K, int N, int silu_in,
                                                    int silu_out) {
  const int lane = threadIdx.x & 63;
  const int64_t o = (int64_t)blockIdx.x * 4 + (threadIdx.x >> 6);
  if (o >= (int64_t)B * N) return;
  const int b = (int)(o / N), n = (int)(o % N);
  const float* xr = x + (int64_t)b * ldx;
  const float* wr = W + (int64_t)n * K;
  float acc = 0.f;
  if ((K & 3) == 0 && (ldx & 3) == 0) {
    float a4[4] = {0.f, 0.f, 0.f, 0.f};
    const int nv = K >> 2;
    for (int v0 = lane; v0 < nv; v0 += 256) {
#pragma unroll
      for (int u = 0; u < 4; ++u) {
        const int v = v0 + u * 64;
        if (v < nv) {
          const f32x4 wv = __builtin_nontemporal_load((const f32x4*)wr + v);
          f32x4 xv = *((const f32x4*)xr + v);
          if (silu_in) { xv[0] = silu_acc(xv[0]); xv[1] = silu_acc(xv[1]); xv[2] = silu_acc(xv[2]); xv[3] = silu_acc(xv[3]); }
          a4[u] += xv[0] * wv[0] + xv[1] * wv[1] + xv[2] * wv[2] + xv[3] * wv[3];
        }
      }
    }
    acc = (a4[0] + a4[1]) + (a4[2] + a4[3]);
  } else {
    for (int k = lane; k < K; k += 64) {
      float xv = xr[k];
      if (silu_in) xv = silu_acc(xv);
      acc += xv * wr[k];
    }
  }
#pragma unroll
  for (int s = 32; s > 0; s >>= 1) acc += __shfl_xor(acc, s);
  if (lane == 0) {
    float v = acc + (bias ? bias[n] : 0.f);
    if (silu_out) v = silu_acc(v);
    y[(int64_t)b * ldy + n] = v;
  }
}

__global__ void k_embed_tokens(const int* __restrict__ ids, const float* __restrict__ tok,
                               const float* __restrict__ pos, bf16_t* __restrict__ out, int B, int L, int D, int vocab) {
  const int nvec = D / 8;
  const int64_t n = (int64_t)B * L * nvec;
  for (int64_t i = blockIdx.x * (int64_t)blockDim.x + threadIdx.x; i < n; i += (int64_t)gridDim.x * blockDim.x) {
    const int v = (int)(i % nvec);
    const int64_t bl = i / nvec;
    const int l = (int)(bl % L);
    int id = ids[bl];
    id = id < 0 ? 0 : (id >= vocab ? vocab - 1 : id);
    const float* tr = tok + (int64_t)id * D + v * 8;
    const float* pr = pos + (int64_t)l * D + v * 8;
    float f[8];
#pragma unroll
    for (int e = 0; e < 8; ++e) f[e] = tr[e] + pr[e];
    *(uint4*)(out + bl * D + v * 8) = pack8(f);
  }
}

__global__ void k_vit_tokens(const bf16_t* __restrict__ patch, const float* __restrict__ cls,
                             const float* __restrict__ pos, bf16_t* __restrict__ out, int B, int T, int D) {
  const int nvec = D / 8;
  const int64_t n = (int64_t)B * (T + 1) * nvec;
  for (int64_t i = blockIdx.x * (int64_t)blockDim.x + threadIdx.x; i < n; i += (int64_t)gridDim.x * blockDim.x) {
    const int v = (int)(i % nvec);
    const int64_t bt = i / nvec;
    const int t = (int)(bt % (T + 1));
    const int b = (int)(bt / (T + 1));
    float f[8];
    if (t == 0) {
#pragma unroll
      for (int e = 0; e < 8; ++e) f[e] = cls[v * 8 + e];
    } else {
      unpack8(*(const uint4*)(patch + ((int64_t)b * T + (t - 1)) * D + v * 8), f);
    }
    const float* pr = pos + (int64_t)t * D + v * 8;
#pragma unroll
    for (int e = 0; e < 8; ++e) f[e] += pr[e];
    *(uint4*)(out + bt * D + v * 8) = pack8(f);
  }
}

__global__ void k_gather_eot(const bf16_t* __restrict__ x, const int* __restrict__ ids, bf16_t* __restrict__ out,
                             int L, int D) {
  const int b = blockIdx.x;
  int best = 0, bv = ids[(int64_t)b * L];
  for (int l = 1; l < L; ++l) {
    const int v = ids[(int64_t)b * L + l];
    if (v > bv) { bv = v; best = l; }
  }
  const bf16_t* src = x + ((int64_t)b * L + best) * D;
  for (int i = threadIdx.x; i < D; i += blockDim.x) out[(int64_t)b * D + i] = src[i];
}

__global__ void k_avgpool2(const bf16_t* __restrict__ x, bf16_t* __restrict__ y, int B, int H, int W, int C) {
  const int Ho = H / 2, Wo = W / 2, nvec = C / 8;
  const int64_t n = (int64_t)B * Ho * Wo * nvec;
  for (int64_t i = blockIdx.x * (int64_t)blockDim.x + threadIdx.x; i < n;
       i += (int64_t)gridDim.x * blockDim.x) {
    const int v = (int)(i % nvec);
    int64_t t = i / nvec;
    const int ox = (int)(t % Wo); t /= Wo;
    const int oy = (int)(t % Ho);
    const int b = (int)(t / Ho);
    float a[8] = {0, 0, 0, 0, 0, 0, 0, 0};
#pragma unroll
    for (int dy = 0; dy < 2; ++dy)
#pragma unroll
      for (int dx = 0; dx < 2; ++dx) {
        float f[8];
        unpack8(*(const uint4*)(x + (((int64_t)b * H + oy * 2 + dy) * W + ox * 2 + dx) * C + v * 8), f);
#pragma unroll
        for (int e = 0; e < 8; ++e) a[e] += f[e];
      }
#pragma unroll
    for (int e = 0; e < 8; ++e) a[e] *= 0.25f;
    *(uint4*)(y + (((int64_t)b * Ho + oy) * Wo + ox) * C + v * 8) = pack8(a);
  }
}

__global__ void k_upsample2(const bf16_t* __restrict__ x, bf16_t* __restrict__ y, int B, int H, int W, int C) {
  const int Ho = H * 2, Wo = W * 2, nvec = C / 8;
  const int64_t n = (int64_t)B * Ho * Wo * nvec;
  for (int64_t i = blockIdx.x * (int64_t)blockDim.x + threadIdx.x; i < n;
       i += (int64_t)gridDim.x * blockDim.x) {
    const int v = (int)(i % nvec);
    int64_t t = i / nvec;
    const int ox = (int)(t % Wo); t /= Wo;
    const int oy = (int)(t % Ho);
    const int b = (int)(t / Ho);
    *(uint4*)(y + (((int64_t)b * Ho + oy) * Wo + ox) * C + v * 8) =
        *(const uint4*)(x + (((int64_t)b * H + (oy >> 1)) * W + (ox >> 1)) * C + v * 8);
  }
}

__global__ void k_posterior_sample(const float* __restrict__ mom, int ld, const float* __restrict__ noise,
                                   uint64_t seed, float* __restrict__ z, int B, int zc, int HW,
                                   float scale, int use_mean) {
  const int64_t n = (int64_t)B * zc * HW;
  for (int64_t i = blockIdx.x * (int64_t)blockDim.x + threadIdx.x; i < n;
       i += (int64_t)gridDim.x * blockDim.x) {
    const int pix = (int)(i % HW);
    const int64_t bc = i / HW;
    const int c = (int)(bc % zc);
    const int b = (int)(bc / zc);
    const float* m = mom + ((int64_t)b * HW + pix) * ld;
    const float mean = m[c];
    float v = mean;
    if (!use_mean) {
      float lv = m[zc + c];
      lv = fminf(fmaxf(lv, -30.0f), 20.0f);
      const float sd = expf(0.5f * lv);
      const float nz = noise ? noise[i] : philox_normal2(seed, 0x7a65u, (uint64_t)i);
      v = mean + sd * nz;
    }
    z[i] = scale * v;
  }
}

__global__ __launch_bounds__(256) void k_vq_quantize(const float* __restrict__ z, float in_mul,
                                                     const float* __restrict__ codebook, int n_embed, int zc, int B,
                                                     int HW, bf16_t* __restrict__ out, int Cpad) {
  extern __shared__ float cb[];
  for (int i = threadIdx.x; i < n_embed * zc; i += blockDim.x) cb[i] = codebook[i];
  __syncthreads();
  const int64_t n = (int64_t)B * HW;
  for (int64_t v = blockIdx.x * (int64_t)blockDim.x + threadIdx.x; v < n; v += (int64_t)gridDim.x * blockDim.x) {
    const int b = (int)(v / HW), pix = (int)(v - (int64_t)b * HW);
    float zv[8];
    float z2 = 0.f;
    for (int c = 0; c < zc; ++c) {
      zv[c] = z[((int64_t)b * zc + c) * HW + pix] * in_mul;
      z2 += zv[c] * zv[c];
    }
    int best = 0;
    float bd = INFINITY;
    for (int k = 0; k < n_embed; ++k) {
      const float* e = cb + k * zc;
      float e2 = 0.f, dot = 0.f;
      for (int c = 0; c < zc; ++c) { e2 += e[c] * e[c]; dot += zv[c] * e[c]; }
      const float d = (z2 + e2) - 2.0f * dot;
      if (d < bd) { bd = d; best = k; }
    }
    bf16_t* o = out + v * Cpad;
    for (int c = 0; c < Cpad; ++c) o[c] = f2bf(c < zc ? zv[c] + (cb[best * zc + c] - zv[c]) : 0.f);
  }
}

__global__ void k_fill_f32(float* p, float v, int64_t n) {
  for (int64_t i = blockIdx.x * (int64_t)blockDim.x + threadIdx.x; i < n;
       i += (int64_t)gridDim.x * blockDim.x) p[i] = v;
}

__global__ void k_copy_strided_bf16(const bf16_t* __restrict__ src, int lds_, bf16_t* __restrict__ dst,
                                    int ldd, int64_t rows, int cols) {
  const int nvec = cols / 8;
  const int64_t n = rows * nvec;
  for (int64_t i = blockIdx.x * (int64_t)blockDim.x + threadIdx.x; i < n;
       i += (int64_t)gridDim.x * blockDim.x) {
    const int64_t r = i / nvec;
    const int v = (int)(i % nvec);
    *(uint4*)(dst + r * ldd + v * 8) = *(const uint4*)(src + r * lds_ + v * 8);
  }
}

inline int ew_grid(int64_t n) {
  int64_t g = (n + 255) / 256;
  return (int)(g > 4096 ? 4096 : (g < 1 ? 1 : g));
}

}

void launch_nchw_to_nhwc(hipStream_t st, const float* x, bf16_t* y, int B, int C, int HW, int Cpad,
                         float scale, float shift, int dup) {
  const int64_t n = (int64_t)B * HW * Cpad;
  hipLaunchKernelGGL(k_nchw_to_nhwc, dim3(ew_grid(n)), dim3(256), 0, st, x, y, B, C, HW, Cpad, scale,
                     shift, dup);
}
void launch_nhwc_to_nchw(hipStream_t st, const void* x, int x_f32, int ldx, float* y, int B, int C,
                         int HW, float scale, float shift) {
  const int64_t n = (int64_t)B * C * HW;
  hipLaunchKernelGGL(k_nhwc_to_nchw, dim3(ew_grid(n)), dim3(256), 0, st, x, x_f32, ldx, y, B, C, HW,
                     scale, shift);
}
void launch_timestep_embedding(hipStream_t st, const StepCoef* tab, const int* step_ptr, int step,
                               const float* t_explicit, float* out, int B, int dim, int mode) {
  const int n = B * (dim / 2);
  hipLaunchKernelGGL(k_timestep_embedding, dim3(ceil_div(n, 256)), dim3(256), 0, st, tab, step_ptr,
                     step, t_explicit, out, B, dim, mode);
}
void launch_vec_linear(hipStream_t st, const float* x, int ldx, const float* W, const float* bias,
                       float* y, int ldy, int B, int K, int N, int silu_in, int silu_out) {
  const int64_t outs = (int64_t)B * N;
  hipLaunchKernelGGL(k_vec_linear, dim3((unsigned)ceil_div64(outs, 4)), dim3(256), 0, st, x, ldx, W,
                     bias, y, ldy, B, K, N, silu_in, silu_out);
}
void launch_avgpool2(hipStream_t st, const bf16_t* x, bf16_t* y, int B, int H, int W, int C) {
  const int64_t n = (int64_t)B * (H / 2) * (W / 2) * (C / 8);
  hipLaunchKernelGGL(k_avgpool2, dim3(ew_grid(n)), dim3(256), 0, st, x, y, B, H, W, C);
}
void launch_upsample2(hipStream_t st, const bf16_t* x, bf16_t* y, int B, int H, int W, int C) {
  const int64_t n = (int64_t)B * H * 2 * W * 2 * (C / 8);
  hipLaunchKernelGGL(k_upsample2, dim3(ew_grid(n)), dim3(256), 0, st, x, y, B, H, W, C);
}
void launch_posterior_sample(hipStream_t st, const float* mom, int ld, const float* noise,
                             uint64_t seed, float* z, int B, int zc, int HW, float scale,
                             int use_mean) {
  const int64_t n = (int64_t)B * zc * HW;
  hipLaunchKernelGGL(k_posterior_sample, dim3(ew_grid(n)), dim3(256), 0, st, mom, ld, noise, seed, z,
                     B, zc, HW, scale, use_mean);
}
void launch_vq_quantize(hipStream_t st, const float* z, float in_mul, const float* codebook, int n_embed, int zc,
                        int B, int HW, bf16_t* out, int Cpad) {
  CD_CHECK(zc >= 1 && zc <= 8 && n_embed > 0, "vq_quantize: embed_dim %d / n_embed %d", zc, n_embed);
  const size_t lds = (size_t)n_embed * zc * sizeof(float);
  CD_CHECK(lds <= 150 * 1024, "vq_quantize: codebook of %zu bytes does not fit LDS", lds);
  static PerDeviceOnce attr_once;
  attr_once([&]() {
    HIP_CHECK(hipFuncSetAttribute((const void*)k_vq_quantize, hipFuncAttributeMaxDynamicSharedMemorySize, 150 * 1024));
  });
  const int64_t n = (int64_t)B * HW;
  int grid = (int)((n + 255) / 256);
  if (grid > 512) grid = 512;
  hipLaunchKernelGGL(k_vq_quantize, dim3(grid), dim3(256), lds, st, z, in_mul, codebook, n_embed, zc, B, HW, out, Cpad);
}
void launch_embed_tokens(hipStream_t st, const int* ids, const float* tok, const float* pos, bf16_t* out, int B,
                         int L, int D, int vocab) {
  CD_CHECK(D % 8 == 0, "embed_tokens: width %% 8");
  const int64_t n = (int64_t)B * L * (D / 8);
  hipLaunchKernelGGL(k_embed_tokens, dim3(ew_grid(n)), dim3(256), 0, st, ids, tok, pos, out, B, L, D, vocab);
}
void launch_vit_tokens(hipStream_t st, const bf16_t* patch, const float* cls, const float* pos, bf16_t* out, int B,
                       int T, int D) {
  CD_CHECK(D % 8 == 0, "vit_tokens: width %% 8");
  const int64_t n = (int64_t)B * (T + 1) * (D / 8);
  hipLaunchKernelGGL(k_vit_tokens, dim3(ew_grid(n)), dim3(256), 0, st, patch, cls, pos, out, B, T, D);
}
void launch_gather_eot(hipStream_t st, const bf16_t* x, const int* ids, bf16_t* out, int B, int L, int D) {
  hipLaunchKernelGGL(k_gather_eot, dim3(B), dim3(256), 0, st, x, ids, out, L, D);
}
void launch_fill_f32(hipStream_t st, float* p, float v, int64_t n) {
  hipLaunchKernelGGL(k_fill_f32, dim3(ew_grid(n)), dim3(256), 0, st, p, v, n);
}
void launch_copy_strided_bf16(hipStream_t st, const bf16_t* src, int lds_, bf16_t* dst, int ldd,
                              int64_t rows, int cols) {
  const int64_t n = rows * (cols / 8);
  hipLaunchKernelGGL(k_copy_strided_bf16, dim3(ew_grid(n)), dim3(256), 0, st, src, lds_, dst, ldd,
                     rows, cols);
}

}
```

cycle-diffusion_amd/csrc/engine.h:

```cpp
#pragma once
#include <map>
#include <memory>
#include <string>
#include <vector>

#include "common.h"
#include "kernels.h"
#include "../../include/cyclediff.h"

namespace cd {

class Arena {
 public:
  ~Arena();
  void init(size_t bytes);
  void* alloc(size_t bytes);
  size_t mark() const { return off_; }
  void release(size_t m) { off_ = m; }
  void reset() { off_ = 0; }
  size_t capacity() const { return cap_; }
  size_t high_water() const { return high_; }
 private:
  char* base_ = nullptr;
  size_t cap_ = 0, off_ = 0, high_ = 0;
};

struct Act {
  bf16_t* p = nullptr;
  int B = 0, H = 0, W = 0, C = 0;
  int ld = 0;
  bool f32 = false;
  bool split = false;
  float* pf() const { return (float*)p; }
  float* stats = nullptr;
  float* stats_buf = nullptr;
  int64_t rows() const { return (int64_t)B * H * W; }
};

struct ConvW {
  bf16_t* w = nullptr;
  bf16_t* wfrag = nullptr;
  bf16_t* w3 = nullptr;
  bool f32 = false;
  float* b = nullptr;
  int N = 0, Cin = 0, Cpad = 0, KH = 1, KW = 1, Npad = 0;
  bool geglu = false;
  int Ktot() const { return KH * KW * Cpad; }
};

struct PackTarget {
  enum Kind { MATRIX_BF16, VECTOR_F32, MATRIX_F32 } kind;
  ConvW* conv = nullptr;
  int dst_row0 = 0, rows = 0, src_base = 0, grp = 0, grp_stride = 0;
  float* fdst = nullptr;
  int dst_off = 0, K = 1;
  bool geglu = false;
  int geglu_N = 0;
  float scale = 1.f;
};

struct ParamDecl {
  std::string name;
  std::vector<int64_t> shape;
  std::vector<PackTarget> targets;
  bool loaded = false;
  bool transposed = false;
};

class ParamStore {
 public:
  ~ParamStore();
  bool f32 = false;
  bool x3 = false;
  int* overflow = nullptr;
  int version = 0;
  ConvW* new_conv(int N, int Cin, int KH, int KW, bool bias, bool geglu = false);
  float* new_vec(int n, float init = 0.f);
  ParamDecl& declare(const std::string& name, std::vector<int64_t> shape);
  void conv_weight(const std::string& name, ConvW* c, int ref_ndim = 0, float scale = 1.f);
  void conv_weight_t(const std::string& name, ConvW* c);
  void conv_bias(const std::string& name, ConvW* c);
  void conv_rows(const std::string& name, std::vector<int64_t> shape, ConvW* c, int dst_row0, int rows,
                 int src_base, int grp, int grp_stride, float scale = 1.f);
  void bias_rows(const std::string& name, int64_t n_total, float* dst, int dst_off, int rows, int src_base,
                 int grp, int grp_stride);
  void vec(const std::string& name, float* dst, int n);
  void mat_f32(const std::string& name, float* dst, int N, int K, int dst_row0 = 0);

  void load(hipStream_t st, const std::string& name, const float* host, int ndim, const int64_t* shape);
  int missing(std::string* first = nullptr) const;
  const std::vector<std::unique_ptr<ParamDecl>>& decls() const { return decls_; }
  size_t device_bytes() const { return dev_bytes_; }
 private:
  std::vector<std::unique_ptr<ParamDecl>> decls_;
  std::map<std::string, ParamDecl*> by_name_;
  std::vector<std::unique_ptr<ConvW>> convs_;
  std::vector<void*> allocs_;
  float* staging_ = nullptr;
  size_t staging_bytes_ = 0;
  size_t dev_bytes_ = 0;
  void* dmalloc(size_t bytes);
};

struct Ctx {
  hipStream_t st = nullptr;
  Arena* arena = nullptr;
  const bf16_t* zeros = nullptr;
  float* gn_partial = nullptr;
  size_t gn_partial_floats = 0;
  bool f32 = false;
  bool x3 = false;
  int* overflow = nullptr;
};

struct ConvOpts {
  int stride = 1;
  int pad = 1;
  bool asym = false;
  bool up = false;
  const float* rowvec = nullptr; int rowvec_ld = 0; int rows_per_vec = 1;
  const Act* resid = nullptr;
  int act = ACT_NONE;
  float alpha = 1.f;
  bool out_f32 = false;
  void* out = nullptr;
  int out_ld = 0;
  bool ln_fold = false;
  float ln_eps = 1e-5f;
  bool raw_geglu = false;
  bool want_stats = false;
  float* out_stats = nullptr;
  int tile = 0;
};
Act attention_flash_f32_fwd(Ctx& c, const float* q, int ldq, const float* k, int ldk, int64_t k_bs, const float* v, int ldv,
                            int64_t v_bs, int B, int H, int Tq, int Tk, int D, float scale, int Himg, int Wimg, bool q_log2);
Act geglu_f32_fwd(Ctx& c, const Act& h);
Act split_rows_f32_fwd(Ctx& c, const Act& x, const Act* x2 = nullptr);
Act alloc_act(Ctx& c, int B, int H, int W, int C, bool with_stats = false);
Act conv_fwd(Ctx& c, const ConvW& w, const Act& x, const Act* x2, const ConvOpts& o);
bool conv_ln_fold_available(const Ctx& c, const ConvW& w, int64_t rows);

struct GNW { float* g = nullptr; float* b = nullptr; int C = 0; float eps = 1e-5f; };
Act groupnorm_fwd(Ctx& c, const GNW& w, const Act& x, const Act* x2, bool silu, const float* film = nullptr,
                  int film_ld = 0);
struct LNW { float* g = nullptr; float* b = nullptr; int C = 0; };
Act layernorm_fwd(Ctx& c, const LNW& w, const Act& x);

Act avgpool2_fwd(Ctx& c, const Act& x);
Act upsample2_fwd(Ctx& c, const Act& x);
Act attention_f32_fwd(Ctx& c, const Act& qk, const Act& v, int H, int D, float scale, const float* obias);

Act attention_fwd(Ctx& c, const bf16_t* q, int ldq, const bf16_t* k, int ldk, const bf16_t* v, int ldv, int B,
                  int H, int Tq, int Tk, int D, float scale, int Himg, int Wimg, bool q_log2 = false);
Act attention_vt_fwd(Ctx& c, const bf16_t* q, int ldq, const bf16_t* k, int ldk, const bf16_t* vt, int B,
                     int H, int Tq, int Tk, int Tpad, int D, float scale, int Himg, int Wimg, bool q_log2 = false);

class Net {
 public:
  virtual ~Net() {}
  ParamStore params;
  cd_net_desc desc;
  bool f32 = false;
  bool x3 = false;
  virtual int kind() const = 0;
};

struct TimeEmb {
  int mode = 0, dim = 0, hidden = 0;
  float *w0 = nullptr, *b0 = nullptr, *w1 = nullptr, *b1 = nullptr;
  float* proj_w = nullptr; float* proj_b = nullptr;
  int proj_total = 0;
};

struct UNetIO {
  const bf16_t* xin = nullptr;
  int B = 0;
  const StepCoef* tab = nullptr; const int* step_ptr = nullptr; int step = 0;
  const float* t_explicit = nullptr;
  bool t_shared = true;
  bool cfg_dup = false;
  int dup_tail = 0;
  float* out = nullptr;
  int out_ld = 0;
};

class UNet : public Net {
 public:
  virtual void forward(Ctx& c, const UNetIO& io) = 0;
  virtual void set_context(Ctx& c, const bf16_t* ctx, int B, int L) { (void)c; (void)ctx; (void)B; (void)L; }
  int in_cpad = 32;
  int out_channels = 0;
  int image_size = 0;
  virtual size_t workspace_hint(int B) const = 0;
};

std::unique_ptr<UNet> make_unet_openai(const cd_net_desc& d);
std::unique_ptr<UNet> make_unet_ho(const cd_net_desc& d);

class VAE : public Net {
 public:
  int kind() const override { return CD_NET_VAE_KL; }
  virtual void encode_moments(Ctx& c, const bf16_t* img_nhwc, int B, int R, float* moments) = 0;
  virtual void decode(Ctx& c, const bf16_t* z_nhwc, int B, int h, float* img) = 0;
  int z_channels = 4, factor = 8;
  int moments_channels = 8;
  const float* codebook = nullptr;
  int n_embed = 0;
};
std::unique_ptr<VAE> make_vae_kl(const cd_net_desc& d);

class TextEncoder : public Net {
 public:
  virtual void encode(Ctx& c, const int* ids_dev, int B, int L, float* out) = 0;
  virtual void text_features(Ctx&, const int*, int, int, float*) { CD_CHECK(false, "net has no pooled text features"); }
  virtual void image_features(Ctx&, const float*, int, float*) { CD_CHECK(false, "net has no image tower"); }
  virtual int width() const = 0;
  virtual int max_positions() const = 0;
};
std::unique_ptr<TextEncoder> make_clip_text(const cd_net_desc& d);

std::unique_ptr<Net> make_inception_fid(const cd_net_desc& d);
void inception_fid_features(Net* n, Ctx& c, const float* img, int B, int stop_block, float* out);

}
```

cycle-diffusion_amd/csrc/engine.hip:

```cpp
#include <stdlib.h>

#include "engine.h"

#include <string.h>

namespace cd {

Arena::~Arena() { if (base_) (void)hipFree(base_); }
void Arena::init(size_t bytes) {
  if (base_) { (void)hipFree(base_); base_ = nullptr; }
  HIP_CHECK(hipMalloc((void**)&base_, bytes));
  cap_ = bytes; off_ = 0; high_ = 0;
}
void* Arena::alloc(size_t bytes) {
  size_t a = (off_ + 255) & ~(size_t)255;
  CD_CHECK(a + bytes <= cap_, "workspace arena exhausted: need %zu more bytes (capacity %zu); "
           "create the engine with a larger workspace", a + bytes - cap_, cap_);
  off_ = a + bytes;
  if (off_ > high_) high_ = off_;
  return base_ + a;
}

ParamStore::~ParamStore() {
  for (void* p : allocs_) (void)hipFree(p);
  if (staging_) (void)hipFree(staging_);
}
void* ParamStore::dmalloc(size_t bytes) {
  void* p = nullptr;
  HIP_CHECK(hipMalloc(&p, bytes < 256 ? 256 : bytes));
  HIP_CHECK(hipMemset(p, 0, bytes < 256 ? 256 : bytes));
  allocs_.push_back(p);
  dev_bytes_ += bytes;
  return p;
}
ConvW* ParamStore::new_conv(int N, int Cin, int KH, int KW, bool bias, bool geglu) {
  convs_.emplace_back(new ConvW());
  ConvW* c = convs_.back().get();
  c->N = N; c->Cin = Cin; c->KH = KH; c->KW = KW; c->geglu = geglu;
  c->Cpad = round_up(Cin, 32);
  c->Npad = round_up(N, 128);
  c->f32 = f32;
  c->w = (bf16_t*)dmalloc((size_t)c->Npad * c->Ktot() * (f32 ? sizeof(float) : sizeof(bf16_t)));
  if (!f32 && KH == 1 && KW == 1 && c->Cpad == 320)
    c->wfrag = (bf16_t*)dmalloc((size_t)c->Npad * c->Cpad * sizeof(bf16_t));
  if (f32 && x3) c->w3 = (bf16_t*)dmalloc((size_t)c->Npad * c->Ktot() * 3 * sizeof(bf16_t));
  if (bias) c->b = (float*)dmalloc((size_t)c->Npad * sizeof(float));
  return c;
}
float* ParamStore::new_vec(int n, float init) {
  float* p = (float*)dmalloc((size_t)n * sizeof(float));
  if (init != 0.f) {
    std::vector<float> h(n, init);
    HIP_CHECK(hipMemcpy(p, h.data(), (size_t)n * sizeof(float), hipMemcpyHostToDevice));
  }
  return p;
}
ParamDecl& ParamStore::declare(const std::string& name, std::vector<int64_t> shape) {
  auto it = by_name_.find(name);
  if (it != by_name_.end()) {
    CD_CHECK(it->second->shape == shape, "parameter %s declared twice with different shapes", name.c_str());
    return *it->second;
  }
  decls_.emplace_back(new ParamDecl());
  ParamDecl* d = decls_.back().get();
  d->name = name; d->shape = std::move(shape);
  by_name_[name] = d;
  return *d;
}
void ParamStore::conv_weight(const std::string& name, ConvW* c, int ref_ndim, float scale) {
  std::vector<int64_t> shape;
  if (ref_ndim == 0) ref_ndim = (c->KH == 1 && c->KW == 1) ? 2 : 4;
  if (ref_ndim == 2) shape = {c->N, c->Cin};
  else if (ref_ndim == 3) shape = {c->N, c->Cin, 1};
  else shape = {c->N, c->Cin, c->KH, c->KW};
  ParamDecl& d = declare(name, shape);
  PackTarget t; t.kind = PackTarget::MATRIX_BF16; t.conv = c; t.dst_row0 = 0; t.rows = c->N;
  t.src_base = 0; t.grp = c->N; t.grp_stride = 0; t.geglu = c->geglu; t.scale = scale;
  d.targets.push_back(t);
}
void ParamStore::conv_weight_t(const std::string& name, ConvW* c) {
  CD_CHECK(c->KH == 1 && c->KW == 1, "transposed weights are linear layers");
  ParamDecl& d = declare(name, {c->Cin, c->N});
  d.transposed = true;
  PackTarget t; t.kind = PackTarget::MATRIX_BF16; t.conv = c; t.dst_row0 = 0; t.rows = c->N;
  t.src_base = 0; t.grp = c->N; t.grp_stride = 0; t.geglu = false;
  d.targets.push_back(t);
}
void ParamStore::conv_bias(const std::string& name, ConvW* c) {
  CD_CHECK(c->b, "conv %s has no bias storage", name.c_str());
  ParamDecl& d = declare(name, {c->N});
  PackTarget t; t.kind = PackTarget::VECTOR_F32; t.fdst = c->b; t.dst_off = 0; t.rows = c->N;
  t.src_base = 0; t.grp = c->N; t.grp_stride = 0; t.geglu = c->geglu; t.geglu_N = c->N;
  d.targets.push_back(t);
}
void ParamStore::conv_rows(const std::string& name, std::vector<int64_t> shape, ConvW* c, int dst_row0,
                           int rows, int src_base, int grp, int grp_stride, float scale) {
  ParamDecl& d = declare(name, std::move(shape));
  PackTarget t; t.kind = PackTarget::MATRIX_BF16; t.conv = c; t.dst_row0 = dst_row0; t.rows = rows;
  t.src_base = src_base; t.grp = grp; t.grp_stride = grp_stride; t.scale = scale;
  d.targets.push_back(t);
}
void ParamStore::bias_rows(const std::string& name, int64_t n_total, float* dst, int dst_off, int rows,
                           int src_base, int grp, int grp_stride) {
  ParamDecl& d = declare(name, {n_total});
  PackTarget t; t.kind = PackTarget::VECTOR_F32; t.fdst = dst; t.dst_off = dst_off; t.rows = rows;
  t.src_base = src_base; t.grp = grp; t.grp_stride = grp_stride;
  d.targets.push_back(t);
}
void ParamStore::vec(const std::string& name, float* dst, int n) {
  bias_rows(name, n, dst, 0, n, 0, n, 0);
}
void ParamStore::mat_f32(const std::string& name, float* dst, int N, int K, int dst_row0) {
  ParamDecl& d = declare(name, {N, K});
  PackTarget t; t.kind = PackTarget::MATRIX_F32; t.fdst = dst; t.dst_off = dst_row0; t.rows = N; t.K = K;
  t.src_base = 0; t.grp = N; t.grp_stride = 0;
  d.targets.push_back(t);
}

template <typename OutT>
__global__ void k_pack_rows(const float* __restrict__ w, OutT* __restrict__ out, int rows, int Cin,
                            int KH, int KW, int Cpad, int dst_row0, int src_base, int grp,
                            int grp_stride, int geglu, int Ntot, float scale) {
  const int64_t total = (int64_t)rows * KH * KW * Cpad;
  for (int64_t i = blockIdx.x * (int64_t)blockDim.x + threadIdx.x; i < total;
       i += (int64_t)gridDim.x * blockDim.x) {
    const int c = (int)(i % Cpad);
    int64_t t = i / Cpad;
    const int s = (int)(t % KW); t /= KW;
    const int r = (int)(t % KH); t /= KH;
    const int j = (int)t;
    int jj = j;
    if (geglu) {
      const int blk = j / 64, within = j % 64;
      jj = (within < 32) ? blk * 32 + within : Ntot / 2 + blk * 32 + (within - 32);
    }
    const int src = src_base + (jj / grp) * grp_stride + (jj % grp);
    float v = 0.f;
    if (c < Cin) v = w[(((int64_t)src * Cin + c) * KH + r) * KW + s] * scale;
    const int64_t o = ((int64_t)(dst_row0 + j) * KH * KW + (int64_t)r * KW + s) * Cpad + c;
    if constexpr (sizeof(OutT) == 4) out[o] = v;
    else out[o] = f2bf(v);
  }
}

void ParamStore::load(hipStream_t st, const std::string& name, const float* host, int ndim,
                      const int64_t* shape) {
  ++version;
  auto it = by_name_.find(name);
  CD_CHECK(it != by_name_.end(), "unknown parameter name '%s'", name.c_str());
  ParamDecl& d = *it->second;
  int64_t n = 1, nd = 1;
  for (int i = 0; i < ndim; ++i) n *= shape[i];
  for (auto s : d.shape) nd *= s;
  bool ok = (n == nd) && ndim >= 1 && shape[0] == d.shape[0];
  if (ok && d.shape.size() >= 2 && ndim >= 2) ok = (shape[1] == d.shape[1]);
  CD_CHECK(ok, "parameter %s: shape mismatch (got %lld elements, ndim %d; expected %lld)", name.c_str(),
           (long long)n, ndim, (long long)nd);
  const size_t bytes = (size_t)n * sizeof(float);
  if (bytes > staging_bytes_) {
    if (staging_) HIP_CHECK(hipFree(staging_));
    staging_bytes_ = bytes < (1u << 20) ? (1u << 20) : bytes;
    HIP_CHECK(hipMalloc((void**)&staging_, staging_bytes_));
  }
  HIP_CHECK(hipStreamSynchronize(st));
  if (d.transposed) {
    const int64_t K = d.shape[0], N = d.shape[1];
    std::vector<float> tr((size_t)n);
    for (int64_t k = 0; k < K; ++k)
      for (int64_t j = 0; j < N; ++j) tr[(size_t)j * K + k] = host[(size_t)k * N + j];
    HIP_CHECK(hipMemcpy(staging_, tr.data(), bytes, hipMemcpyHostToDevice));
  } else {
    HIP_CHECK(hipMemcpy(staging_, host, bytes, hipMemcpyHostToDevice));
  }
  for (const PackTarget& t : d.targets) {
    if (t.kind == PackTarget::MATRIX_BF16) {
      const ConvW* c = t.conv;
      const int64_t total = (int64_t)t.rows * c->KH * c->KW * c->Cpad;
      int grid = (int)((total + 255) / 256);
      if (grid > 8192) grid = 8192;
      if (c->f32)
        hipLaunchKernelGGL(k_pack_rows<float>, dim3(grid), dim3(256), 0, st, staging_, (float*)c->w, t.rows, c->Cin,
                           c->KH, c->KW, c->Cpad, t.dst_row0, t.src_base, t.grp, t.grp_stride, t.geglu ? 1 : 0, c->N,
                           t.scale);
      else
        hipLaunchKernelGGL(k_pack_rows<bf16_t>, dim3(grid), dim3(256), 0, st, staging_, c->w, t.rows, c->Cin, c->KH,
                           c->KW, c->Cpad, t.dst_row0, t.src_base, t.grp, t.grp_stride, t.geglu ? 1 : 0, c->N, t.scale);
      if (c->wfrag) launch_pack_wfrag(st, c->w, c->Ktot(), c->wfrag, c->Npad);
      if (c->w3) launch_pack_w3(st, (const float*)c->w, c->w3, c->Npad, c->KH * c->KW, c->Cpad, overflow);
    } else {
      const int K = (t.kind == PackTarget::MATRIX_F32) ? t.K : 1;
      std::vector<float> tmp((size_t)t.rows * K);
      for (int j = 0; j < t.rows; ++j) {
        int jj = j;
        if (t.geglu) {
          const int blk = j / 64, within = j % 64;
          jj = (within < 32) ? blk * 32 + within : t.geglu_N / 2 + blk * 32 + (within - 32);
        }
        const int src = t.src_base + (jj / t.grp) * t.grp_stride + (jj % t.grp);
        memcpy(&tmp[(size_t)j * K], host + (size_t)src * K, (size_t)K * sizeof(float));
      }
      HIP_CHECK(hipMemcpy(t.fdst + (size_t)t.dst_off * K, tmp.data(), tmp.size() * sizeof(float),
                          hipMemcpyHostToDevice));
    }
  }
  HIP_CHECK(hipStreamSynchronize(st));
  d.loaded = true;
}

int ParamStore::missing(std::string* first) const {
  int n = 0;
  for (auto& d : decls_)
    if (!d->loaded) {
      if (n == 0 && first) *first = d->name;
      ++n;
    }
  return n;
}

Act alloc_act(Ctx& c, int B, int H, int W, int C, bool with_stats) {
  Act a; a.B = B; a.H = H; a.W = W; a.C = C; a.ld = C; a.f32 = c.f32;
  a.p = (bf16_t*)c.arena->alloc((size_t)B * H * W * C * (c.f32 ? sizeof(float) : sizeof(bf16_t)));
  if ((!c.f32 || c.x3) && with_stats && ((H * W) % 32) == 0)
    a.stats_buf = (float*)c.arena->alloc((size_t)(B * H * W / 32) * 2 * C * sizeof(float));
  return a;
}

static Act conv_split_fwd(Ctx& c, const ConvW& w, const Act& x, const ConvOpts& o) {
  CD_CHECK(c.f32 && c.x3 && w.w3 && (!w.geglu || o.raw_geglu), "conv: split input outside the split-fp16 mode");
  CD_CHECK(x.C == w.Cpad && x.ld == 2 * x.C, "conv: split input of %d channels (ld %d) against Cpad %d", x.C, x.ld, w.Cpad);
  CD_CHECK(!o.ln_fold && (!o.resid || (o.resid->f32 && !o.resid->split)), "conv: split-mode operands");
  ConvGemmParams p;
  p.src0 = x.p; p.C0 = 2 * x.C; p.ld0 = x.ld;
  p.src1 = x.p; p.C1 = x.C; p.ld1 = x.ld;
  p.B = x.B; p.Hs = x.H; p.Ws = x.W; p.up = o.up ? 1 : 0;
  p.Hin = o.up ? x.H * 2 : x.H; p.Win = o.up ? x.W * 2 : x.W;
  p.KH = w.KH; p.KW = w.KW; p.stride = o.stride;
  if (o.asym) { p.pad_t = 0; p.pad_l = 0; p.Hout = (p.Hin + 1 - w.KH) / o.stride + 1; p.Wout = (p.Win + 1 - w.KW) / o.stride + 1; }
  else {
    p.pad_t = o.pad; p.pad_l = o.pad;
    p.Hout = (p.Hin + 2 * o.pad - w.KH) / o.stride + 1;
    p.Wout = (p.Win + 2 * o.pad - w.KW) / o.stride + 1;
  }
  p.M = x.B * p.Hout * p.Wout;
  p.wgt = w.w3; p.Ktot = 3 * w.Ktot(); p.N = w.N;
  p.alpha = o.alpha * (1.0f / (kX3ActScale * kX3WgtScale)); p.bias = w.b;
  p.rowvec = o.rowvec; p.rowvec_ld = o.rowvec_ld; p.rows_per_vec = o.rows_per_vec;
  p.act = o.act;
  Act y; y.B = x.B; y.H = p.Hout; y.W = p.Wout; y.C = w.N; y.f32 = true;
  if (o.out) { y.p = (bf16_t*)o.out; y.ld = o.out_ld; }
  else { y.ld = w.N; y.p = (bf16_t*)c.arena->alloc((size_t)p.M * w.N * 4); }
  if (o.resid) {
    CD_CHECK(o.resid->rows() == p.M && o.resid->C == w.N, "conv: residual shape mismatch");
    p.resid = o.resid->p; p.resid_ld = o.resid->ld; p.resid_f32 = 1;
  }
  p.out = y.p; p.out_ld = y.ld; p.out_f32 = 1;
  p.zeros = c.zeros; p.tile = o.tile;
  p.prof_flop_scale = 1.0f / 3.0f;
  if (((p.Hout * p.Wout) % 32) == 0) {
    if (o.out && o.out_stats) y.stats_buf = o.out_stats;
    else if (!o.out && o.want_stats)
      y.stats_buf = (float*)c.arena->alloc((size_t)(p.M / 32) * 2 * w.N * sizeof(float));
    p.stats = y.stats_buf;
    y.stats = y.stats_buf;
  }
  launch_conv_gemm(c.st, p);
  return y;
}

Act conv_fwd(Ctx& c, const ConvW& w, const Act& x, const Act* x2, const ConvOpts& o) {
  if (x.split) {
    CD_CHECK(!x2, "conv: a split activation cannot be concatenated");
    return conv_split_fwd(c, w, x, o);
  }
  ConvGemmParams p;
  CD_CHECK(w.f32 == c.f32 && x.f32 == c.f32 && (!x2 || x2->f32 == c.f32) && (!o.resid || o.resid->f32 == c.f32),
           "conv: operand precision does not match the running network");
  CD_CHECK((!x2 || !x2->split) && (!o.resid || !o.resid->split), "conv: split activation as a second source / residual");
  p.src0 = x.p; p.C0 = round_up(x.C, 32); p.ld0 = x.ld;
  if (x2) {
    CD_CHECK(x2->B == x.B && x2->H == x.H && x2->W == x.W, "conv: concat sources differ in shape");
    p.src1 = x2->p; p.C1 = x2->C; p.ld1 = x2->ld;
    CD_CHECK(x.C % 32 == 0 && x2->C % 32 == 0, "conv: concat channels must be multiples of 32");
  }
  CD_CHECK(p.C0 + p.C1 == w.Cpad, "conv: input channels %d+%d do not match weight Cpad %d", p.C0, p.C1, w.Cpad);
  CD_CHECK(x.ld >= p.C0, "conv: source row shorter than padded channel count");
  p.B = x.B; p.Hs = x.H; p.Ws = x.W; p.up = o.up ? 1 : 0;
  p.Hin = o.up ? x.H * 2 : x.H; p.Win = o.up ? x.W * 2 : x.W;
  p.KH = w.KH; p.KW = w.KW; p.stride = o.stride;
  if (o.asym) { p.pad_t = 0; p.pad_l = 0; p.Hout = (p.Hin + 1 - w.KH) / o.stride + 1; p.Wout = (p.Win + 1 - w.KW) / o.stride + 1; }
  else {
    p.pad_t = o.pad; p.pad_l = o.pad;
    p.Hout = (p.Hin + 2 * o.pad - w.KH) / o.stride + 1;
    p.Wout = (p.Win + 2 * o.pad - w.KW) / o.stride + 1;
  }
  p.M = x.B * p.Hout * p.Wout;
  p.wgt = w.w; p.wgt_frag = w.wfrag; p.Ktot = w.Ktot(); p.N = w.N;
  p.alpha = o.alpha; p.bias = w.b;
  p.rowvec = o.rowvec; p.rowvec_ld = o.rowvec_ld; p.rows_per_vec = o.rows_per_vec;
  const bool fuse_geglu = w.geglu && !o.raw_geglu;
  p.act = fuse_geglu ? ACT_GEGLU : o.act;
  const int Nout = fuse_geglu ? w.N / 2 : w.N;
  Act y; y.B = x.B; y.H = p.Hout; y.W = p.Wout; y.C = Nout; y.f32 = c.f32;
  if (o.out) { y.p = (bf16_t*)o.out; y.ld = o.out_ld; }
  else {
    y.ld = Nout;
    y.p = (bf16_t*)c.arena->alloc((size_t)p.M * Nout * ((o.out_f32 || c.f32) ? 4 : 2));
  }
  if (o.resid) {
    CD_CHECK(o.resid->rows() == p.M && o.resid->C == Nout, "conv: residual shape mismatch");
    p.resid = o.resid->p; p.resid_ld = o.resid->ld;
  }
  p.out = y.p; p.out_ld = y.ld; p.out_f32 = o.out_f32 ? 1 : 0;
  p.zeros = c.zeros; p.tile = o.tile;
  if (o.ln_fold) { p.ln_fold = 1; p.ln_eps = o.ln_eps; p.tile = kLinStreamTile; }
  if (c.f32) {
    p.out_f32 = 1;
    launch_conv_gemm_f32(c.st, p);
    return y;
  }
  if (!w.geglu && !o.out_f32 && ((p.Hout * p.Wout) % 32) == 0) {
    if (o.out && o.out_stats) y.stats_buf = o.out_stats;
    else if (!o.out && o.want_stats)
      y.stats_buf = (float*)c.arena->alloc((size_t)(p.M / 32) * 2 * Nout * sizeof(float));
    p.stats = y.stats_buf;
    y.stats = y.stats_buf;
  }
  launch_conv_gemm(c.st, p);
  return y;
}

bool conv_ln_fold_available(const Ctx& c, const ConvW& w, int64_t rows) {
  static const bool on = [] { const char* e = getenv("CYCLEDIFF_LN_FOLD"); return !(e && e[0] == '0'); }();
  static const int64_t min_rows = [] { const char* e = getenv("CYCLEDIFF_LN_FOLD_MIN_ROWS"); return e ? atoll(e) : 32768ll; }();
  return on && !c.f32 && w.wfrag && w.KH == 1 && w.KW == 1 && w.Cpad == 320 && rows >= min_rows && rows % 32 == 0 &&
         w.N % 64 == 0 && w.N <= 2560;
}

Act groupnorm_fwd(Ctx& c, const GNW& w, const Act& x, const Act* x2, bool silu, const float* film,
                  int film_ld) {
  GroupNormParams p;
  p.x = x.p; p.C0 = x.C; p.ld0 = x.ld;
  if (x2) { p.x1 = x2->p; p.C1 = x2->C; p.ld1 = x2->ld; }
  const int C = p.C0 + p.C1;
  CD_CHECK(C == w.C, "groupnorm: channels %d != weight %d", C, w.C);
  p.B = x.B; p.HW = x.H * x.W; p.G = 32; p.eps = w.eps; p.gamma = w.g; p.beta = w.b;
  p.film = film; p.film_ld = film_ld; p.silu = silu ? 1 : 0;
  Act y = alloc_act(c, x.B, x.H, x.W, C);
  p.y = y.p;
  if (c.f32) {
    CD_CHECK(x.f32 && (!x2 || x2->f32) && !x.split && (!x2 || !x2->split), "groupnorm: operand precision");
    if (c.x3) { p.split_out = 1; p.overflow = c.overflow; y.split = true; y.ld = 2 * C; }
    if (x.stats && x.ld == x.C && (!x2 || (x2->stats && x2->ld == x2->C))) {
      p.pre0 = x.stats;
      p.pre1 = x2 ? x2->stats : nullptr;
    }
    const size_t mk = c.arena->mark();
    void* ws = c.arena->alloc(groupnorm_f32_workspace(p.B, p.HW, C));
    launch_groupnorm_f32(c.st, p, ws);
    c.arena->release(mk);
    return y;
  }
  p.S = groupnorm_slabs(p.B, p.HW, C);
  const size_t part_floats = round_up((size_t)p.B * p.S * p.G * 2, (size_t)64);
  CD_CHECK(part_floats + (size_t)p.B * 2 * C <= c.gn_partial_floats, "groupnorm: workspace too small");
  p.partial = c.gn_partial;
  p.coef = c.gn_partial + part_floats;
  if (x.stats && x.ld == x.C && (!x2 || (x2->stats && x2->ld == x2->C))) {
    p.pre0 = x.stats;
    p.pre1 = x2 ? x2->stats : nullptr;
  }
  launch_groupnorm(c.st, p);
  return y;
}

Act avgpool2_fwd(Ctx& c, const Act& x) {
  if (x.split) {
    Act y = alloc_act(c, x.B, x.H / 2, x.W / 2, x.C);
    y.split = true; y.ld = 2 * x.C;
    launch_avgpool2_split(c.st, x.p, y.p, x.B, x.H, x.W, x.C, c.overflow);
    return y;
  }
  CD_CHECK(x.ld == x.C, "avgpool: dense input expected");
  Act y = alloc_act(c, x.B, x.H / 2, x.W / 2, x.C);
  if (c.f32) launch_avgpool2_f32(c.st, x.pf(), y.pf(), x.B, x.H, x.W, x.C);
  else launch_avgpool2(c.st, x.p, y.p, x.B, x.H, x.W, x.C);
  return y;
}
Act upsample2_fwd(Ctx& c, const Act& x) {
  CD_CHECK(x.ld == x.C && !x.split, "upsample: dense input expected");
  Act y = alloc_act(c, x.B, x.H * 2, x.W * 2, x.C);
  if (c.f32) launch_upsample2_f32(c.st, x.pf(), y.pf(), x.B, x.H, x.W, x.C);
  else launch_upsample2(c.st, x.p, y.p, x.B, x.H, x.W, x.C);
  return y;
}
Act attention_f32_fwd(Ctx& c, const Act& qk, const Act& v, int H, int D, float scale, const float* obias) {
  CD_CHECK(c.f32 && qk.f32 && v.f32 && !qk.split && !v.split && qk.C == 2 * H * D && v.C == H * D,
           "attention_f32: operands");
  Act o = alloc_act(c, qk.B, qk.H, qk.W, H * D);
  const int T = qk.H * qk.W;
  if (D <= 160 && (D % 4) == 0 && (qk.ld % 4) == 0 && (v.ld % 4) == 0) {
    launch_flash_f32(c.st, qk.pf(), qk.ld, (int64_t)T * qk.ld, qk.pf() + H * D, qk.ld, (int64_t)T * qk.ld, v.pf(), v.ld,
                     (int64_t)T * v.ld, o.pf(), o.ld, (int64_t)T * o.ld, qk.B, H, T, T, D, scale * 1.44269504088896340736f, 0,
                     c.overflow, obias);
    return o;
  }
  launch_attention_f32(c.st, qk.pf(), qk.ld, qk.pf() + H * D, qk.ld, v.pf(), v.ld, o.pf(), o.ld, qk.B, H, T, D, scale, obias);
  return o;
}

Act layernorm_fwd(Ctx& c, const LNW& w, const Act& x) {
  CD_CHECK(x.C == w.C, "layernorm: channels");
  if (c.f32) {
    CD_CHECK(x.f32 && !x.split, "layernorm_f32: operand precision");
    Act y = alloc_act(c, x.B, x.H, x.W, x.C);
    if (c.x3) { y.split = true; y.ld = 2 * x.C; }
    launch_layernorm_f32(c.st, x.pf(), x.ld, y.pf(), x.rows(), x.C, w.g, w.b, 1e-5f, c.x3 ? 1 : 0, c.overflow);
    return y;
  }
  Act y = alloc_act(c, x.B, x.H, x.W, x.C);
  launch_layernorm(c.st, x.p, x.ld, y.p, y.ld, (int)x.rows(), x.C, w.g, w.b, 1e-5f);
  return y;
}
// ... 61 lines not shown
```

cycle-diffusion_amd/csrc/kernels.h:

```cpp
#pragma once
#include <map>
#include <string>
#include <vector>

#include "common.h"

namespace cd {

struct StepCoef {
  float sa, s1a, sap, dirc, sigma, r, t_mask;
  int t;
};
enum { SCHED_DDIM = 0, SCHED_DDPM = 1 };

struct EpsHat {
  const float* p;
  int64_t sb, sc, sp;
  int cfg;
  float g;
  const float* gvec = nullptr;
};

void launch_init_xt(hipStream_t st, const float* x0, const float* noise, uint64_t seed,
                    uint32_t stream, float* xt, float* z, int64_t z_bstride, int B, int C, int HW,
                    const StepCoef* tab, int step, bf16_t* xin, int xin_cpad, int cfg_dup);
void launch_encode_step(hipStream_t st, int kind, const float* x0, float* xt, const EpsHat& eh,
                        const float* noise, uint64_t seed, uint32_t stream, float* z,
                        int64_t z_bstride, int B, int C, int HW, const StepCoef* tab,
                        const int* step_ptr, int step, int is_last, bf16_t* xin, int xin_cpad,
                        int cfg_dup_next);
void launch_decode_step(hipStream_t st, int kind, float* x, const EpsHat& eh, const float* eps,
                        int64_t eps_bstride, const float* noise, uint64_t seed, uint32_t stream,
                        int B, int C, int HW, const StepCoef* tab, const int* step_ptr, int step,
                        bf16_t* xin, int xin_cpad, int cfg_dup_next, float* x0_pred, int eps_bmod = 0);
struct MaskBlend {
  const float* mask = nullptr;
  const float* src = nullptr;
  int mask_bmod = 1, src_bmod = 1;
  const float2* qtab = nullptr;
  int qrow = 0;
  const float* noise = nullptr;
  uint64_t seed = 0;
  uint32_t stream = 0;
};
void launch_mask_blend_init(hipStream_t st, float* x, const MaskBlend& mk, int B, int C, int HW, bf16_t* xin, int xin_cpad,
                            int cfg_dup);
void launch_decode_step_masked(hipStream_t st, float* x, const EpsHat& eh, const float* eps, int64_t eps_bstride,
                               const float* noise, uint64_t seed, uint32_t stream, int B, int C, int HW,
                               const StepCoef* tab, const int* step_ptr, int step, bf16_t* xin, int xin_cpad,
                               int cfg_dup_next, int eps_bmod, const MaskBlend& mk, int blend);
void launch_set_int(hipStream_t st, int* p, int v);
void launch_add_int(hipStream_t st, int* p, int d);

enum { ACT_NONE = 0, ACT_SILU = 1, ACT_GELU = 2, ACT_GEGLU = 3, ACT_QGELU = 4, ACT_RELU = 5 };

struct ConvGemmParams {
  const bf16_t* src0 = nullptr;
  const bf16_t* src1 = nullptr;
  int C0 = 0, C1 = 0;
  int ld0 = 0, ld1 = 0;
  int B = 1, Hs = 1, Ws = 1;
  int up = 0;
  int Hin = 1, Win = 1;
  int KH = 1, KW = 1, stride = 1, pad_t = 0, pad_l = 0;
  int Hout = 1, Wout = 1;
  int M = 0;
  const bf16_t* wgt = nullptr;
  const bf16_t* wgt_frag = nullptr;
  int Ktot = 0, N = 0;
  int ldw = 0;
  int nbatch = 1;
  int64_t a_bs = 0, w_bs = 0, o_bs = 0;
  float alpha = 1.0f;
  const float* bias = nullptr;
  const float* rowvec = nullptr;
  int rowvec_ld = 0, rows_per_vec = 1;
  const bf16_t* resid = nullptr;
  int resid_ld = 0;
  int resid_f32 = 0;
  int act = ACT_NONE;
  void* out = nullptr;
  int out_ld = 0;
  int out_f32 = 0;
  float* stats = nullptr;
  const bf16_t* zeros = nullptr;
  int ln_fold = 0;
  float ln_eps = 1e-5f;
  int tile = 0;
  float prof_flop_scale = 1.f;
  int splitk = 0;
  float* sk_scratch = nullptr;
  int* sk_flags = nullptr;
  unsigned long long* probe = nullptr;
  int korder = 1;
  int tile_group = 0;
  int dephase_ticks = 0;
  int num_cus = 256;
  int dbg = 0;
};
constexpr int kProbeWords = 48;
extern thread_local unsigned long long* g_conv_probe;
struct SplitKWorkspace {
  float* scratch = nullptr;
  size_t scratch_bytes = 0;
  int* flags = nullptr;
  int nflags = 0;
};
extern thread_local SplitKWorkspace g_conv_splitk;
void launch_conv_gemm(hipStream_t st, const ConvGemmParams& p);
const char* conv_gemm_last_config();
struct GemmLaunchInfo {
  int tile_id = 0;
  int bk = 0;
  int splitk = 1;
  int chm = 0;
  int tile_group = 0;
};
GemmLaunchInfo conv_gemm_last_launch();
int conv_gemm_num_configs();
const char* conv_gemm_config_name(int id);

struct LinStreamParams {
  const bf16_t* a = nullptr; int lda = 0;
  const bf16_t* wfrag = nullptr;
  const float* bias = nullptr;
  const bf16_t* resid = nullptr; int ldr = 0;
  bf16_t* out = nullptr; int ldo = 0;
  float* stats = nullptr;
  int M = 0, N = 0;
  float ln_eps = 1e-5f;
  int geglu_direct = 0;
};
constexpr int kLinStreamTile = 30;
bool lin_stream_supports(const ConvGemmParams& p);
void launch_lin_stream(hipStream_t st, const ConvGemmParams& p);
void launch_fold_ln(hipStream_t st, const bf16_t* w, int ldw, const float* gamma, const float* beta, const float* bias,
                    bf16_t* w_out, float* bias_out, int N, int Kc);
void launch_pack_wfrag(hipStream_t st, const bf16_t* w, int ldw, bf16_t* out, int N);

struct KernelProfiler {
  bool enabled = false;
  std::vector<hipEvent_t> events;
  std::vector<double> flops;
  std::vector<std::string> labels;
  int used = 0;
  bool verbose = false;
  struct Entry { int n = 0; double ms = 0, flops = 0; };
  std::map<std::string, Entry> per_shape;
  void next_pair(hipEvent_t* a, hipEvent_t* b, double fl, const std::string& what);
  void collect(int* launches, double* total_ms, double* total_flops);
  ~KernelProfiler();
};
extern thread_local KernelProfiler* g_conv_prof;

struct ConvTuner {
  bool enabled = false;
  void* scratch = nullptr;
  size_t scratch_bytes = 0;
  int shapes_tuned = 0;
};
extern ConvTuner g_conv_tuner;

void launch_repack_weight(hipStream_t st, const float* w, bf16_t* out, int N, int Cin, int KH,
                          int KW, int Npad, int Cpad, int geglu, int64_t src_row_offset);

struct GroupNormParams {
  const bf16_t* x = nullptr;
  const bf16_t* x1 = nullptr;
  int C0 = 0, C1 = 0, ld0 = 0, ld1 = 0;
  int B = 0, HW = 0, G = 32;
  float eps = 1e-5f;
  const float* gamma = nullptr;
  const float* beta = nullptr;
  const float* film = nullptr;
  int film_ld = 0;
  int silu = 0;
  int split_out = 0;
  int* overflow = nullptr;
  bf16_t* y = nullptr;
  float* partial = nullptr;
  int S = 0;
  float* coef = nullptr;
  const float* pre0 = nullptr;
  const float* pre1 = nullptr;
};
int groupnorm_slabs(int B, int HW, int C);
void launch_groupnorm(hipStream_t st, const GroupNormParams& p);

void launch_layernorm(hipStream_t st, const bf16_t* x, int ldx, bf16_t* y, int ldy, int rows,
                      int C, const float* gamma, const float* beta, float eps);
void launch_softmax_rows(hipStream_t st, const float* s, int lds, bf16_t* p, int ldp, int64_t rows,
                         int cols);

struct AttnParams {
  const bf16_t* q = nullptr;
  const bf16_t* k = nullptr;
  const bf16_t* v = nullptr;
  const bf16_t* vt = nullptr;
  int ldv = 0; int64_t v_bs = 0;
  bf16_t* o = nullptr;
  int B = 0, H = 0, Tq = 0, Tk = 0, D = 0;
  int ldq = 0, ldk = 0, ldo = 0;
  int64_t q_bs = 0, k_bs = 0, o_bs = 0;
  int vt_dpad = 0, vt_tpad = 0;
  float scale = 1.0f;
  int q_log2 = 0;
  const float* obias = nullptr;
  int causal = 0;
};
void launch_attention(hipStream_t st, const AttnParams& p);
void launch_transpose_v(hipStream_t st, const bf16_t* v, int ldv, int64_t v_bs, bf16_t* vt, int B,
                        int H, int Tk, int D, int Dpad, int Tpad);

void launch_mfma_sustained(hipStream_t st, int target_ms, float* tflops, float* ghz);

void launch_nchw_to_nhwc(hipStream_t st, const float* x, bf16_t* y, int B, int C, int HW, int Cpad,
                         float scale, float shift, int dup);
void launch_nhwc_to_nchw(hipStream_t st, const void* x, int x_f32, int ldx, float* y, int B, int C,
                         int HW, float scale, float shift);
void launch_timestep_embedding(hipStream_t st, const StepCoef* tab, const int* step_ptr, int step,
                               const float* t_explicit, float* out, int B, int dim, int mode);
void launch_vec_linear(hipStream_t st, const float* x, int ldx, const float* W, const float* bias,
                       float* y, int ldy, int B, int K, int N, int silu_in, int silu_out);
void launch_avgpool2(hipStream_t st, const bf16_t* x, bf16_t* y, int B, int H, int W, int C);
void launch_upsample2(hipStream_t st, const bf16_t* x, bf16_t* y, int B, int H, int W, int C);
void launch_posterior_sample(hipStream_t st, const float* mom, int ld, const float* noise,
                             uint64_t seed, float* z, int B, int zc, int HW, float scale,
                             int use_mean);
void launch_vq_quantize(hipStream_t st, const float* z, float in_mul, const float* codebook, int n_embed, int zc,
                        int B, int HW, bf16_t* out, int Cpad);
void launch_fill_f32(hipStream_t st, float* p, float v, int64_t n);
void launch_vit_tokens(hipStream_t st, const bf16_t* patch, const float* cls, const float* pos, bf16_t* out, int B,
                       int T, int D);
void launch_gather_eot(hipStream_t st, const bf16_t* x, const int* ids, bf16_t* out, int B, int L, int D);
void launch_embed_tokens(hipStream_t st, const int* ids, const float* tok, const float* pos, bf16_t* out, int B,
                         int L, int D, int vocab);
void launch_conv_gemm_f32(hipStream_t st, const ConvGemmParams& p);
size_t groupnorm_f32_workspace(int B, int HW, int C);
void launch_groupnorm_f32(hipStream_t st, const GroupNormParams& p, void* workspace);
void launch_attention_f32(hipStream_t st, const float* q, int ldq, const float* k, int ldk, const float* v, int ldv,
                          float* o, int ldo, int B, int H, int T, int D, float scale, const float* obias);
void launch_nchw_to_nhwc_f32(hipStream_t st, const float* x, float* y, int B, int C, int HW, int Cpad, float scale,
                             float shift, int split = 0, int* overflow = nullptr);
void launch_avgpool2_f32(hipStream_t st, const float* x, float* y, int B, int H, int W, int C);
void launch_flash_f32(hipStream_t st, const float* q, int ldq, int64_t q_bs, const float* k, int ldk, int64_t k_bs,
                      const float* v, int ldv, int64_t v_bs, float* o, int ldo, int64_t o_bs, int B, int H, int Tq, int Tk,
                      int D, float qmul, int split, int* overflow, const float* obias = nullptr);
void launch_layernorm_f32(hipStream_t st, const float* x, int ldx, float* y, int64_t rows, int C, const float* gamma,
                          const float* beta, float eps, int split, int* overflow);
void launch_geglu_f32(hipStream_t st, const float* h, float* y, int64_t rows, int Nout, int split, int* overflow);
void launch_split_rows_f32(hipStream_t st, const float* x0, int ld0, int C0, const float* x1, int ld1, int C1, bf16_t* y,
                           int64_t rows, int* overflow);
void launch_upsample2_f32(hipStream_t st, const float* x, float* y, int B, int H, int W, int C);
constexpr float kX3ActScale = 16.f;
constexpr float kX3WgtScale = 256.f;
void launch_pack_w3(hipStream_t st, const float* w, bf16_t* w3, int Npad, int taps, int Cpad, int* overflow);
void launch_avgpool2_split(hipStream_t st, const bf16_t* x, bf16_t* y, int B, int H, int W, int C, int* overflow);

void launch_copy_strided_bf16(hipStream_t st, const bf16_t* src, int lds, bf16_t* dst, int ldd,
                              int64_t rows, int cols);

}
```

cycle-diffusion_amd/csrc/unet_openai.hip:

```cpp
#include <limits.h>

#include <algorithm>

#include "engine.h"

namespace cd {

namespace {

struct ResW {
  int cin = 0, cout = 0;
  bool up = false, down = false, film = false;
  GNW gn1, gn2;
  ConvW *conv1 = nullptr, *conv2 = nullptr, *skip = nullptr;
  int emb_off = 0;
};

struct STW {
  int C = 0, heads = 0, dh = 0, ctx = 0;
  GNW norm;
  ConvW *proj_in = nullptr, *proj_out = nullptr;
  LNW ln1, ln2, ln3;
  ConvW *qkv1 = nullptr, *qk1 = nullptr, *v1 = nullptr, *o1 = nullptr;
  ConvW *q2 = nullptr, *k2 = nullptr, *v2 = nullptr, *o2 = nullptr;
// ... 76 lines not shown
}

int UNetOpenAI::add_res(const std::string& pfx, int cin, int cout, bool up, bool down) {
  ResW r; r.cin = cin; r.cout = cout; r.up = up; r.down = down; r.film = desc.use_scale_shift_norm != 0;
  r.gn1 = make_gn(params, pfx + ".in_layers.0", cin, 1e-5f);
  r.conv1 = make_conv(params, pfx + ".in_layers.2", cout, cin, 3, true);
  r.gn2 = make_gn(params, pfx + ".out_layers.0", cout, 1e-5f);
  r.conv2 = make_conv(params, pfx + ".out_layers.3", cout, cout, 3, true);
  if (cin != cout) r.skip = make_conv(params, pfx + ".skip_connection", cout, cin, 1, true);
  r.emb_off = te_.proj_total;
  te_.proj_total += r.film ? 2 * cout : cout;
  res_.push_back(r);
  return (int)res_.size() - 1;
}

int UNetOpenAI::add_st(const std::string& pfx, int C, int heads, int dh) {
  STW s; s.C = C; s.heads = heads; s.dh = dh; s.ctx = desc.context_dim;
  CD_CHECK(heads * dh == C, "spatial transformer: inner dim %d != channels %d", heads * dh, C);
  CD_CHECK(desc.transformer_depth == 1, "only transformer_depth=1 is supported");
  s.norm = make_gn(params, pfx + ".norm", C, 1e-6f);
  s.proj_in = make_conv(params, pfx + ".proj_in", C, C, 1, true);
  s.proj_out = make_conv(params, pfx + ".proj_out", C, C, 1, true);
  const std::string tb = pfx + ".transformer_blocks.0";
  s.ln1 = make_ln(params, tb + ".norm1", C);
  s.ln2 = make_ln(params, tb + ".norm2", C);
  s.ln3 = make_ln(params, tb + ".norm3", C);
  const float qscale = 1.44269504088896340736f / sqrtf((float)dh);
  if (dh == 40) {
    s.qk1 = params.new_conv(2 * C, C, 1, 1, false);
    params.conv_rows(tb + ".attn1.to_q.weight", {C, C}, s.qk1, 0, C, 0, C, 0, qscale);
    params.conv_rows(tb + ".attn1.to_k.weight", {C, C}, s.qk1, C, C, 0, C, 0);
    s.v1 = make_conv(params, tb + ".attn1.to_v", C, C, 1, false, false, 2);
  } else {
    s.qkv1 = params.new_conv(3 * C, C, 1, 1, false);
    params.conv_rows(tb + ".attn1.to_q.weight", {C, C}, s.qkv1, 0, C, 0, C, 0, qscale);
    params.conv_rows(tb + ".attn1.to_k.weight", {C, C}, s.qkv1, C, C, 0, C, 0);
    params.conv_rows(tb + ".attn1.to_v.weight", {C, C}, s.qkv1, 2 * C, C, 0, C, 0);
  }
  s.o1 = make_conv(params, tb + ".attn1.to_out.0", C, C, 1, true, false, 2);
  s.q2 = make_conv(params, tb + ".attn2.to_q", C, C, 1, false, false, 2, qscale);
  s.k2 = make_conv(params, tb + ".attn2.to_k", C, s.ctx, 1, false, false, 2);
  s.v2 = make_conv(params, tb + ".attn2.to_v", C, s.ctx, 1, false, false, 2);
  s.o2 = make_conv(params, tb + ".attn2.to_out.0", C, C, 1, true, false, 2);
  s.ff1 = make_conv(params, tb + ".ff.net.0.proj", 8 * C, C, 1, true, true, 2);
  s.ff2 = make_conv(params, tb + ".ff.net.2", C, 4 * C, 1, true, false, 2);
  if (s.q2->wfrag) {
    s.q2_ln = params.new_conv(C, C, 1, 1, true);
    s.ff1_ln = params.new_conv(8 * C, C, 1, 1, true, true);
  }
  st_.push_back(s);
  return (int)st_.size() - 1;
}

int UNetOpenAI::add_ab(const std::string& pfx, int C, int heads) {
  ABW a; a.C = C; a.heads = heads; a.dh = C / heads;
  a.norm = make_gn(params, pfx + ".norm", C, 1e-5f);
  const int ch = a.dh;
  a.qk = params.new_conv(2 * C, C, 1, 1, true);
  a.v = params.new_conv(C, C, 1, 1, false);
  a.vbias = params.new_vec(C);
  const std::string wn = pfx + ".qkv.weight", bn = pfx + ".qkv.bias";
  params.conv_rows(wn, {3 * C, C, 1}, a.qk, 0, C, 0, ch, 3 * ch);
  params.conv_rows(wn, {3 * C, C, 1}, a.qk, C, C, ch, ch, 3 * ch);
  params.conv_rows(wn, {3 * C, C, 1}, a.v, 0, C, 2 * ch, ch, 3 * ch);
  params.bias_rows(bn, 3 * C, a.qk->b, 0, C, 0, ch, 3 * ch);
  params.bias_rows(bn, 3 * C, a.qk->b, C, C, ch, ch, 3 * ch);
  params.bias_rows(bn, 3 * C, a.vbias, 0, C, 2 * ch, ch, 3 * ch);
  a.proj = make_conv(params, pfx + ".proj_out", C, C, 1, true, false, 3);
  ab_.push_back(a);
  return (int)ab_.size() - 1;
}

UNetOpenAI::UNetOpenAI(const cd_net_desc& d) {
  desc = d;
  f32 = d.precision == CD_PREC_F32 || d.precision == CD_PREC_F32X3;
  x3 = d.precision == CD_PREC_F32X3;
  params.f32 = f32; params.x3 = x3;

  mc_ = d.model_channels; hidden_ = 4 * mc_;
  image_size = d.image_size; out_channels = d.out_channels;
  in_cpad = round_up(d.in_channels, 32);
  CD_CHECK(mc_ % 32 == 0, "model_channels must be a multiple of 32");
  const bool use_st = d.use_spatial_transformer != 0;
  auto has_attn = [&](int ds) { for (int i = 0; i < d.n_attn; ++i) if (d.attn[i] == ds) return true; return false; };
  auto heads_for = [&](int ch, int& heads, int& dh) {
    if (d.num_head_channels == -1) { heads = d.num_heads; dh = ch / heads; }
    else { heads = ch / d.num_head_channels; dh = d.num_head_channels; }
  };
  std::vector<std::string> res_pfx;
  auto add_res_named = [&](const std::string& pfx, int cin, int cout, bool up, bool down) {
    res_pfx.push_back(pfx);
    return add_res(pfx, cin, cout, up, down);
  };
  auto add_attn = [&](Block& blk, const std::string& pfx, int ch) {
    int heads, dh; heads_for(ch, heads, dh);
    Layer l;
    if (use_st) { l.kind = Layer::ST; l.idx = add_st(pfx, ch, heads, dh); }
    else { l.kind = Layer::AB; l.idx = add_ab(pfx, ch, heads); }
    blk.layers.push_back(l);
  };

  {
    Block b; Layer l; l.kind = Layer::CONV_IN;
    l.conv = make_conv(params, "input_blocks.0.0", mc_, d.in_channels, 3, true);
    b.layers.push_back(l); in_blocks_.push_back(b);
  }
  std::vector<int> chans{mc_};
  int ch = mc_, ds = 1, bi = 1;
  for (int level = 0; level < d.n_mult; ++level) {
    const int mult = d.channel_mult[level];
    for (int r = 0; r < d.num_res_blocks; ++r) {
      Block b; Layer l; l.kind = Layer::RES;
      const std::string pfx = "input_blocks." + std::to_string(bi);
      l.idx = add_res_named(pfx + ".0", ch, mult * mc_, false, false);
      b.layers.push_back(l);
      ch = mult * mc_;
      if (has_attn(ds)) add_attn(b, pfx + ".1", ch);
      in_blocks_.push_back(b); chans.push_back(ch); ++bi;
    }
    if (level != d.n_mult - 1) {
      Block b; Layer l;
      const std::string pfx = "input_blocks." + std::to_string(bi) + ".0";
      if (d.resblock_updown) { l.kind = Layer::RES; l.idx = add_res_named(pfx, ch, ch, false, true); }
      else {
        CD_CHECK(d.conv_resample, "Downsample without conv (avg-pool) only exists inside resblock_updown");
        l.kind = Layer::DOWN_CONV; l.conv = make_conv(params, pfx + ".op", ch, ch, 3, true);
      }
      b.layers.push_back(l); in_blocks_.push_back(b); chans.push_back(ch); ++bi; ds *= 2;
    }
  }
  {
    Layer l; l.kind = Layer::RES; l.idx = add_res_named("middle_block.0", ch, ch, false, false);
    mid_.layers.push_back(l);
    add_attn(mid_, "middle_block.1", ch);
    Layer l2; l2.kind = Layer::RES; l2.idx = add_res_named("middle_block.2", ch, ch, false, false);
    mid_.layers.push_back(l2);
  }
  int oi = 0;
  for (int level = d.n_mult - 1; level >= 0; --level) {
    const int mult = d.channel_mult[level];
    for (int i = 0; i <= d.num_res_blocks; ++i) {
      const int ich = chans.back(); chans.pop_back();
      Block b; Layer l; l.kind = Layer::RES;
      const std::string pfx = "output_blocks." + std::to_string(oi);
      l.idx = add_res_named(pfx + ".0", ch + ich, mc_ * mult, false, false);
      b.layers.push_back(l);
      ch = mc_ * mult;
      int sub = 1;
      if (has_attn(ds)) { add_attn(b, pfx + "." + std::to_string(sub), ch); ++sub; }
      if (level && i == d.num_res_blocks) {
        Layer u;
        const std::string up = pfx + "." + std::to_string(sub);
        if (d.resblock_updown) { u.kind = Layer::RES; u.idx = add_res_named(up, ch, ch, true, false); }
        else { u.kind = Layer::UP_CONV; u.conv = make_conv(params, up + ".conv", ch, ch, 3, true); }
        b.layers.push_back(u);
        ds /= 2;
      }
      out_blocks_.push_back(b); ++oi;
    }
  }
  out_norm_ = make_gn(params, "out.0", ch, 1e-5f);
  out_conv_ = make_conv(params, "out.2", d.out_channels, mc_, 3, true);
  CD_CHECK(ch == mc_, "channel bookkeeping: final channels %d != model_channels %d", ch, mc_);

  te_.mode = 0; te_.dim = mc_; te_.hidden = hidden_;
  te_.w0 = params.new_vec(hidden_ * mc_); te_.b0 = params.new_vec(hidden_);
  te_.w1 = params.new_vec(hidden_ * hidden_); te_.b1 = params.new_vec(hidden_);
  params.mat_f32("time_embed.0.weight", te_.w0, hidden_, mc_);
  params.vec("time_embed.0.bias", te_.b0, hidden_);
  params.mat_f32("time_embed.2.weight", te_.w1, hidden_, hidden_);
  params.vec("time_embed.2.bias", te_.b1, hidden_);
  te_.proj_w = params.new_vec(te_.proj_total * hidden_);
  te_.proj_b = params.new_vec(te_.proj_total);
  for (size_t i = 0; i < res_.size(); ++i) {
    const int n = res_[i].film ? 2 * res_[i].cout : res_[i].cout;
    params.mat_f32(res_pfx[i] + ".emb_layers.1.weight", te_.proj_w, n, hidden_, res_[i].emb_off);
    params.bias_rows(res_pfx[i] + ".emb_layers.1.bias", n, te_.proj_b, res_[i].emb_off, n, 0, n, 0);
  }
}

size_t UNetOpenAI::workspace_hint(int B) const {
  const size_t hw = (size_t)image_size * image_size;
  size_t widest = 0;
  for (auto& r : res_) widest = std::max(widest, (size_t)std::max(r.cin, r.cout));
  return (size_t)B * hw * std::max(widest, (size_t)8 * mc_) * 2 * 24 + (64u << 20);
}

Act UNetOpenAI::res_fwd(Ctx& c, const ResW& r, const Act& x, const Act* x2, const float* proj, int proj_ld,
                        bool t_shared) {
  const int Ho = r.up ? x.H * 2 : (r.down ? x.H / 2 : x.H);
  const int Wo = r.up ? x.W * 2 : (r.down ? x.W / 2 : x.W);
  Act out = alloc_act(c, x.B, Ho, Wo, r.cout, true);
  const int rpv = t_shared ? INT_MAX : Ho * Wo;
  const size_t mk = c.arena->mark();
  Act h = groupnorm_fwd(c, r.gn1, x, x2, true);
  Act xs = x;
  const Act* xs2 = x2;
  bool up_in_conv = false;
  if (r.down) {
    CD_CHECK(!x2, "resblock_updown with concat input is not produced by the reference");
    h = avgpool2_fwd(c, h);
    xs = avgpool2_fwd(c, x); xs2 = nullptr;
  } else if (r.up) {
    CD_CHECK(!x2, "resblock_updown with concat input is not produced by the reference");
    up_in_conv = true;
    xs = upsample2_fwd(c, x); xs2 = nullptr;
  }
  ConvOpts o1; o1.up = up_in_conv; o1.want_stats = true;
  const float* pr = proj + r.emb_off;
  if (!r.film) { o1.rowvec = pr; o1.rowvec_ld = proj_ld; o1.rows_per_vec = rpv; }
  Act h2 = conv_fwd(c, *r.conv1, h, nullptr, o1);
  Act h3;
  if (r.film) h3 = groupnorm_fwd(c, r.gn2, h2, nullptr, true, pr, t_shared ? 0 : proj_ld);
  else h3 = groupnorm_fwd(c, r.gn2, h2, nullptr, true);
  Act skip;
  if (r.skip) {
    ConvOpts os; os.pad = 0;
    skip = conv_fwd(c, *r.skip, xs, xs2, os);
  } else {
    CD_CHECK(!xs2, "identity skip with concat input");
    skip = xs;
  }
  ConvOpts o2; o2.resid = &skip; o2.out = out.p; o2.out_ld = out.ld; o2.out_stats = out.stats_buf;
  conv_fwd(c, *r.conv2, h3, nullptr, o2);
  out.stats = out.stats_buf;
  c.arena->release(mk);
  return out;
}

static void vt_gemm(Ctx& c, const ConvW& wv, const bf16_t* x, int ldx, int B, int T, int Tpad, bf16_t* vt) {
  ConvGemmParams p;
  p.src0 = wv.w; p.C0 = wv.Cpad; p.ld0 = wv.Cpad;
  p.B = 1; p.Hs = wv.N; p.Ws = 1; p.Hin = wv.N; p.Win = 1; p.Hout = wv.N; p.Wout = 1;
  p.M = wv.N;
  p.wgt = x; p.Ktot = wv.Cpad; p.N = T;
  CD_CHECK(ldx == wv.Cpad, "vt_gemm: token row stride %d must equal K %d", ldx, wv.Cpad);
  p.nbatch = B; p.a_bs = 0; p.w_bs = (int64_t)T * ldx; p.o_bs = (int64_t)wv.N * Tpad;
  p.out = vt; p.out_ld = Tpad; p.zeros = c.zeros;
  launch_conv_gemm(c.st, p);
}

void UNetOpenAI::set_context(Ctx& c, const bf16_t* ctx, int B, int L) {
  if (st_.empty()) return;
  if (B != ctx_B_ || L != ctx_L_) {
    for (void* p : ctx_allocs_) (void)hipFree(p);
    ctx_allocs_.clear();
    const size_t esz = f32 ? 4 : 2;
    for (auto& s : st_) {
      HIP_CHECK(hipMalloc((void**)&s.k2c, (size_t)B * L * s.C * esz + 256));
      HIP_CHECK(hipMalloc((void**)&s.v2c, (size_t)B * L * s.C * esz + 256));
      ctx_allocs_.push_back(s.k2c); ctx_allocs_.push_back(s.v2c);
    }
    ctx_B_ = B; ctx_L_ = L;
  }
  const bool keep_f32 = c.f32, keep_x3 = c.x3;
  c.f32 = f32; c.x3 = x3;
  Act cx; cx.p = (bf16_t*)ctx; cx.B = 1; cx.H = B * L; cx.W = 1; cx.C = st_[0].ctx; cx.ld = cx.C; cx.f32 = f32;
  for (auto& s : st_) {
    ConvOpts o; o.pad = 0; o.out = s.k2c; o.out_ld = s.C;
    conv_fwd(c, *s.k2, cx, nullptr, o);
    o.out = s.v2c;
    conv_fwd(c, *s.v2, cx, nullptr, o);
  }
  c.f32 = keep_f32; c.x3 = keep_x3;
}

static void dup_rows(Ctx& c, const bf16_t* src, bf16_t* dst, int64_t n, int64_t tail, int cols) {
  launch_copy_strided_bf16(c.st, src, cols, dst, cols, n, cols);
  launch_copy_strided_bf16(c.st, src + (n - tail) * cols, cols, dst + n * cols, cols, tail, cols);
}

Act UNetOpenAI::st_fwd(Ctx& c, STW& s, const Act& x_in, int dup_tail) {
  int B = x_in.B;
  const bool dup = dup_tail > 0;
  const int T = x_in.H * x_in.W, C = s.C;
  CD_CHECK(dup_tail >= 0 && dup_tail <= B, "transformer block: %d repeated samples of %d", dup_tail, B);
  Act out = alloc_act(c, B + dup_tail, x_in.H, x_in.W, C, true);
  Act x = x_in;
  if (dup) {
    CD_CHECK(x_in.ld == C, "transformer block: dense input expected");
    x = alloc_act(c, B + dup_tail, x_in.H, x_in.W, C);
    dup_rows(c, x_in.p, x.p, (int64_t)B * T, (int64_t)dup_tail * T, C);
  }
  const size_t mk = c.arena->mark();
  CD_CHECK(s.k2c && ctx_B_ == B + dup_tail, "cross-attention context not set for batch %d", B + dup_tail);
  if (c.f32) {
    ConvOpts p0; p0.pad = 0;
    Act n = groupnorm_fwd(c, s.norm, x_in, nullptr, false);
    Act h = conv_fwd(c, *s.proj_in, n, nullptr, p0);
    const float scale = 1.0f / sqrtf((float)s.dh);
    CD_CHECK(!dup, "transformer block: prefix sharing is a 16-bit path feature");
    const float* ck = (const float*)s.k2c;
    const float* cv = (const float*)s.v2c;
    {
      const size_t m2 = c.arena->mark();
      Act n1 = layernorm_fwd(c, s.ln1, h);
      Act a;
      if (s.qkv1) {
        Act qkv = conv_fwd(c, *s.qkv1, n1, nullptr, p0);
        a = attention_flash_f32_fwd(c, qkv.pf(), qkv.ld, qkv.pf() + C, qkv.ld, (int64_t)T * qkv.ld, qkv.pf() + 2 * C, qkv.ld,
                                    (int64_t)T * qkv.ld, B, s.heads, T, T, s.dh, scale, x.H, x.W, true);
      } else {
        Act qk = conv_fwd(c, *s.qk1, n1, nullptr, p0);
        Act vv = conv_fwd(c, *s.v1, n1, nullptr, p0);
        a = attention_flash_f32_fwd(c, qk.pf(), qk.ld, qk.pf() + C, qk.ld, (int64_t)T * qk.ld, vv.pf(), vv.ld,
                                    (int64_t)T * vv.ld, B, s.heads, T, T, s.dh, scale, x.H, x.W, true);
      }
// ... 39 lines not shown
    }
    c.arena->release(mk);
    return out;
  }
  static const int st_chunk = [] { const char* e = getenv("CYCLEDIFF_ST_CHUNK"); return e ? atoi(e) : 0; }();
  c.arena->release(mk);
  if (!dup && st_chunk > 0 && T >= 4096 && B >= 2 * st_chunk) {
    for (int b0 = 0; b0 < B; b0 += st_chunk) {
      const int n = std::min(st_chunk, B - b0);
      auto view = [&](const Act& a) {
        Act v = a; v.B = n;
        v.p = a.p + (int64_t)b0 * T * a.ld;
        if (a.stats) v.stats = a.stats + ((int64_t)b0 * T / 32) * 2 * a.C;
        if (a.stats_buf) v.stats_buf = a.stats_buf + ((int64_t)b0 * T / 32) * 2 * a.C;
        return v;
      };
      Act xv = view(x_in), ov = view(out);
      st_core16(c, s, xv, xv, ov, b0, 0);
    }
  } else {
    st_core16(c, s, x_in, x, out, 0, dup_tail);
  }
  out.stats = out.stats_buf;
  return out;
}

void UNetOpenAI::st_core16(Ctx& c, STW& s, const Act& x_in, const Act& x, Act& out, int b0, int dup_tail) {
  const bool dup = dup_tail > 0;
  int B = x_in.B;
  const int T = x_in.H * x_in.W, C = s.C;
  const size_t mk = c.arena->mark();
  ConvOpts p0; p0.pad = 0;
  const float scale = 1.0f / sqrtf((float)s.dh);
  const bf16_t* k2c = s.k2c + (int64_t)b0 * ctx_L_ * C;
  const bf16_t* v2c = s.v2c + (int64_t)b0 * ctx_L_ * C;
  Act n = groupnorm_fwd(c, s.norm, x_in, nullptr, false);
  Act h = conv_fwd(c, *s.proj_in, n, nullptr, p0);
  {
    const size_t m2 = c.arena->mark();
    Act n1 = layernorm_fwd(c, s.ln1, h);
    Act a;
    if (s.qkv1) {
      Act qkv = conv_fwd(c, *s.qkv1, n1, nullptr, p0);
      a = attention_fwd(c, qkv.p, qkv.ld, qkv.p + C, qkv.ld, qkv.p + 2 * C, qkv.ld, B, s.heads, T, T, s.dh, scale,
                        x.H, x.W, true);
    } else {
      Act qk = conv_fwd(c, *s.qk1, n1, nullptr, p0);
      const int Tpad = round_up(T, 64);
      bf16_t* vt = (bf16_t*)c.arena->alloc((size_t)B * C * Tpad * 2);
      if (Tpad != T) HIP_CHECK(hipMemsetAsync(vt, 0, (size_t)B * C * Tpad * 2, c.st));
      vt_gemm(c, *s.v1, n1.p, n1.ld, B, T, Tpad, vt);
      a = attention_vt_fwd(c, qk.p, qk.ld, qk.p + C, qk.ld, vt, B, s.heads, T, T, Tpad, s.dh, scale, x.H, x.W,
                           true);
    }
    ConvOpts o; o.pad = 0; o.resid = &h; o.out = h.p; o.out_ld = h.ld;
    conv_fwd(c, *s.o1, a, nullptr, o);
    c.arena->release(m2);
  }
  if (dup) {
    Act h2 = alloc_act(c, B + dup_tail, x_in.H, x_in.W, C);
    dup_rows(c, h.p, h2.p, (int64_t)B * T, (int64_t)dup_tail * T, C);
    h = h2;
    B += dup_tail;
  }
  {
    const size_t m2 = c.arena->mark();
    Act q;
    if (s.q2_ln && conv_ln_fold_available(c, *s.q2_ln, h.rows())) {
      ConvOpts pl; pl.pad = 0; pl.ln_fold = true;
      q = conv_fwd(c, *s.q2_ln, h, nullptr, pl);
    } else {
      Act n2 = layernorm_fwd(c, s.ln2, h);
      q = conv_fwd(c, *s.q2, n2, nullptr, p0);
    }
    Act a = attention_fwd(c, q.p, q.ld, k2c, C, v2c, C, B, s.heads, T, ctx_L_, s.dh, scale, x.H, x.W,
                          true);
    ConvOpts o; o.pad = 0; o.resid = &h; o.out = h.p; o.out_ld = h.ld;
    conv_fwd(c, *s.o2, a, nullptr, o);
    c.arena->release(m2);
  }
  {
    const size_t m2 = c.arena->mark();
    Act g;
    if (s.ff1_ln && conv_ln_fold_available(c, *s.ff1_ln, h.rows())) {
      ConvOpts pl; pl.pad = 0; pl.ln_fold = true;
      g = conv_fwd(c, *s.ff1_ln, h, nullptr, pl);
    } else {
      Act n3 = layernorm_fwd(c, s.ln3, h);
      g = conv_fwd(c, *s.ff1, n3, nullptr, p0);
    }
    ConvOpts o; o.pad = 0; o.resid = &h; o.out = h.p; o.out_ld = h.ld;
    conv_fwd(c, *s.ff2, g, nullptr, o);
    c.arena->release(m2);
  }
  ConvOpts po; po.pad = 0; po.resid = &x; po.out = out.p; po.out_ld = out.ld; po.out_stats = out.stats_buf;
  conv_fwd(c, *s.proj_out, h, nullptr, po);
  c.arena->release(mk);
}

Act UNetOpenAI::ab_fwd(Ctx& c, const ABW& a, const Act& x) {
  const int B = x.B, T = x.H * x.W, C = a.C;
  Act out = alloc_act(c, B, x.H, x.W, C, true);
  const size_t mk = c.arena->mark();
  ConvOpts p0; p0.pad = 0;
  Act n = groupnorm_fwd(c, a.norm, x, nullptr, false);
  Act qk = conv_fwd(c, *a.qk, n, nullptr, p0);
  if (c.f32) {
    Act v = conv_fwd(c, *a.v, n, nullptr, p0);
    Act o = attention_f32_fwd(c, qk, v, a.heads, a.dh, 1.0f / sqrtf((float)a.dh), a.vbias);
    ConvOpts po; po.pad = 0; po.resid = &x; po.out = out.p; po.out_ld = out.ld;
    conv_fwd(c, *a.proj, o, nullptr, po);
    c.arena->release(mk);
    return out;
  }
  const int Tpad = round_up(T, 64);
  bf16_t* vt = (bf16_t*)c.arena->alloc((size_t)B * C * Tpad * 2);
  if (Tpad != T) HIP_CHECK(hipMemsetAsync(vt, 0, (size_t)B * C * Tpad * 2, c.st));
  vt_gemm(c, *a.v, n.p, n.ld, B, T, Tpad, vt);
  Act o = alloc_act(c, B, x.H, x.W, C);
  AttnParams p;
  p.q = qk.p; p.k = qk.p + C; p.vt = vt; p.o = o.p;
  p.B = B; p.H = a.heads; p.Tq = T; p.Tk = T; p.D = a.dh;
  p.ldq = qk.ld; p.ldk = qk.ld; p.ldo = o.ld;
  p.q_bs = (int64_t)T * qk.ld; p.k_bs = (int64_t)T * qk.ld; p.o_bs = (int64_t)T * o.ld;
  p.vt_dpad = a.dh; p.vt_tpad = Tpad; p.scale = 1.0f / sqrtf((float)a.dh); p.obias = a.vbias;
  launch_attention(c.st, p);
  ConvOpts po; po.pad = 0; po.resid = &x; po.out = out.p; po.out_ld = out.ld; po.out_stats = out.stats_buf;
  conv_fwd(c, *a.proj, o, nullptr, po);
  out.stats = out.stats_buf;
  c.arena->release(mk);
  return out;
}

Act UNetOpenAI::run_block(Ctx& c, const Block& b, Act h, const Act* skip, const float* proj, int proj_ld,
                          bool t_shared) {
  bool first = true;
  for (const Layer& l : b.layers) {
    const Act* x2 = first ? skip : nullptr;
    switch (l.kind) {
      case Layer::CONV_IN: { ConvOpts o; o.want_stats = true; h = conv_fwd(c, *l.conv, h, nullptr, o); break; }
      case Layer::RES: h = res_fwd(c, res_[l.idx], h, x2, proj, proj_ld, t_shared); break;
      case Layer::ST: h = st_fwd(c, st_[l.idx], h); break;
      case Layer::AB: h = ab_fwd(c, ab_[l.idx], h); break;
      case Layer::DOWN_CONV: { ConvOpts o; o.stride = 2; o.want_stats = true; h = conv_fwd(c, *l.conv, h, nullptr, o); break; }
      case Layer::UP_CONV: { ConvOpts o; o.up = true; o.want_stats = true; h = conv_fwd(c, *l.conv, h, nullptr, o); break; }
    }
    first = false;
  }
  return h;
}

void UNetOpenAI::refresh_ln_folds(Ctx& c) {
  if (folded_version_ == params.version) return;
  for (STW& s : st_) {
    if (!s.q2_ln) continue;
    struct { const ConvW* src; ConvW* dst; const LNW* ln; } jobs[2] = {{s.q2, s.q2_ln, &s.ln2}, {s.ff1, s.ff1_ln, &s.ln3}};
    for (auto& j : jobs) {
      launch_fold_ln(c.st, j.src->w, j.src->Ktot(), j.ln->g, j.ln->b, j.src->b, j.dst->w, j.dst->b, j.src->Npad,
                     j.src->Cpad);
      launch_pack_wfrag(c.st, j.dst->w, j.dst->Ktot(), j.dst->wfrag, j.dst->Npad);
    }
  }
  folded_version_ = params.version;
}

void UNetOpenAI::forward(Ctx& c, const UNetIO& io) {
  const size_t mk0 = c.arena->mark();
  c.f32 = f32; c.x3 = x3;
  refresh_ln_folds(c);
  const int B = io.B, R = image_size;
  const int tB = io.t_shared ? 1 : B;
  float* sinu = (float*)c.arena->alloc((size_t)tB * mc_ * 4);
  float* e1 = (float*)c.arena->alloc((size_t)tB * hidden_ * 4);
  float* emb = (float*)c.arena->alloc((size_t)tB * hidden_ * 4);
  float* proj = (float*)c.arena->alloc((size_t)tB * te_.proj_total * 4);
  launch_timestep_embedding(c.st, io.tab, io.step_ptr, io.step, io.t_explicit, sinu, tB, mc_, 0);
  launch_vec_linear(c.st, sinu, mc_, te_.w0, te_.b0, e1, hidden_, tB, mc_, hidden_, 0, 1);
  launch_vec_linear(c.st, e1, hidden_, te_.w1, te_.b1, emb, hidden_, tB, hidden_, hidden_, 0, 0);
  launch_vec_linear(c.st, emb, hidden_, te_.proj_w, te_.proj_b, proj, te_.proj_total, tB, hidden_,
                    te_.proj_total, 1, 0);
  const int proj_ld = te_.proj_total;
  Act x; x.p = (bf16_t*)io.xin; x.B = B; x.H = R; x.W = R; x.C = in_cpad; x.ld = in_cpad; x.f32 = f32;
  if (x3) { x.split = true; x.ld = 2 * in_cpad; }
  std::vector<Act> hs;
  Act h = x;
  size_t first_full = 0;
  static const bool cfg_share = [] { const char* e = getenv("CYCLEDIFF_CFG_SHARE"); return !(e && e[0] == '0'); }();
  CD_CHECK(!(io.cfg_dup && io.dup_tail) && io.dup_tail >= 0 && 2 * io.dup_tail <= B, "U-Net: repeated-row description");
  const int dtail = io.cfg_dup ? (B % 2 == 0 ? B / 2 : 0) : io.dup_tail;
  if (dtail > 0 && cfg_share && !f32 && io.t_shared && in_blocks_.size() >= 2 &&
      in_blocks_[0].layers.size() == 1 && in_blocks_[0].layers[0].kind == Layer::CONV_IN &&
      in_blocks_[1].layers.size() == 2 && in_blocks_[1].layers[0].kind == Layer::RES &&
      in_blocks_[1].layers[1].kind == Layer::ST) {
    const int Bh = B - dtail;
    Act xh = x; xh.B = Bh;
    Act h0 = run_block(c, in_blocks_[0], xh, nullptr, proj, proj_ld, true);
    Act h0f = alloc_act(c, B, h0.H, h0.W, h0.C, h0.stats != nullptr);
    CD_CHECK(h0.ld == h0.C, "conv_in output: dense tensor expected");
    const int64_t rows_tail = (int64_t)dtail * h0.H * h0.W;
    dup_rows(c, h0.p, h0f.p, h0.rows(), rows_tail, h0.C);
    if (h0.stats) {
      dup_rows(c, (const bf16_t*)h0.stats, (bf16_t*)h0f.stats_buf, (h0.rows() / 32) * 2, (rows_tail / 32) * 2, h0.C * 2);
      h0f.stats = h0f.stats_buf;
    }
    hs.push_back(h0f);
    const Layer& lr = in_blocks_[1].layers[0];
    const Layer& lt = in_blocks_[1].layers[1];
    Act hr = res_fwd(c, res_[lr.idx], h0, nullptr, proj, proj_ld, true);
    h = st_fwd(c, st_[lt.idx], hr, dtail);
    hs.push_back(h);
    first_full = 2;
  }
  for (size_t bi = first_full; bi < in_blocks_.size(); ++bi) {
    h = run_block(c, in_blocks_[bi], h, nullptr, proj, proj_ld, io.t_shared);
    hs.push_back(h);
  }
  h = run_block(c, mid_, h, nullptr, proj, proj_ld, io.t_shared);
  for (const Block& b : out_blocks_) {
    Act skip = hs.back(); hs.pop_back();
    h = run_block(c, b, h, &skip, proj, proj_ld, io.t_shared);
  }
  Act hn = groupnorm_fwd(c, out_norm_, h, nullptr, true);
  ConvOpts oo; oo.out_f32 = true; oo.out = io.out; oo.out_ld = io.out_ld;
  conv_fwd(c, *out_conv_, hn, nullptr, oo);
  c.arena->release(mk0);
  c.f32 = false; c.x3 = false;
}

}

std::unique_ptr<UNet> make_unet_openai(const cd_net_desc& d) { return std::unique_ptr<UNet>(new UNetOpenAI(d)); }

}
```

include/cyclediff.h:

```cpp
#ifndef CYCLEDIFF_H
#define CYCLEDIFF_H
#include <stddef.h>
#include <stdint.h>

#ifdef __cplusplus
extern "C" {
#endif

typedef struct cd_engine* cd_handle;

enum { CD_NET_UNET_OPENAI = 1, CD_NET_UNET_HO = 2, CD_NET_VAE_KL = 3, CD_NET_CLIP_TEXT = 4, CD_NET_BERT_XTR = 5,
       CD_NET_OCLIP_TEXT = 6, CD_NET_OCLIP_VISION = 7, CD_NET_INCEPTION_FID = 8 };
enum { CD_SCHED_DDIM = 0, CD_SCHED_DDPM = 1 };
enum { CD_PREC_16 = 0, CD_PREC_F32 = 1, CD_PREC_F32X3 = 2 };
enum { CD_MASK_QSAMPLE = 0, CD_MASK_ENCODER = 1 };

typedef struct cd_net_desc {
  int kind;
  int image_size;
  int in_channels, out_channels;
  int model_channels;
  int num_res_blocks;
  int n_mult;  int channel_mult[8];
  int n_attn;  int attn[8];
  int num_heads;
  int num_head_channels;
  int use_spatial_transformer, context_dim, transformer_depth;
  int use_scale_shift_norm, resblock_updown, conv_resample;
  int z_channels, embed_dim, double_z;
  int precision;
  int n_embed;
  int reserved[6];
} cd_net_desc;

typedef struct cd_step_coef {
  float sa, s1a, sap, dirc, sigma, r, t_mask;
  int32_t t;
} cd_step_coef;

const char* cd_last_error(void);
int cd_version(void);
int cd_act_format(void);

int cd_engine_create(void* hip_stream, size_t workspace_bytes, cd_handle* out);
int cd_engine_destroy(cd_handle h);
int cd_engine_workspace_high_water(cd_handle h, size_t* bytes);
int cd_engine_synchronize(cd_handle h);
int cd_prof_enable(cd_handle h, int on);
int cd_prof_collect(cd_handle h, int* launches, double* total_ms, double* total_flops);

int cd_net_create(cd_handle h, const cd_net_desc* desc, int* net_id);
int cd_net_param_count(cd_handle h, int net, int* n);
int cd_net_param_info(cd_handle h, int net, int index, char* name, int name_cap, int* ndim, int64_t shape[4]);
int cd_net_load_param(cd_handle h, int net, const char* name, const float* data_host, int ndim,
                      const int64_t* shape);
int cd_net_missing_params(cd_handle h, int net, int* n_missing, char* first_name, int name_cap);

int cd_unet_forward(cd_handle h, int net, const float* x, const float* t, const float* ctx, int B,
                    int ctx_len, float* eps_out);

int cd_text_encode(cd_handle h, int net, const int32_t* tokens, int B, int L, float* out);

int cd_inception_features(cd_handle h, int net, const float* img, int B, int stop_block, float* out);
int cd_clip_text_features(cd_handle h, int net, const int32_t* tokens, int B, int L, float* out);
int cd_clip_image_features(cd_handle h, int net, const float* img, int B, float* out);

int cd_vae_encode(cd_handle h, int net, const float* img, const float* noise, uint64_t seed, int B, int R,
                  int sample, float scale, float* z0);
int cd_vae_decode(cd_handle h, int net, const float* z0, int B, int hlat, float scale, float out_mul,
                  float out_add, float* img);

int cd_dpm_encode(cd_handle h, int net, int sched_kind, const float* x0, const float* ctx_c,
                  const float* ctx_uc, int ctx_len, float guidance, int B, int K,
                  const cd_step_coef* coef_host, const float* noise, uint64_t seed,
                  int last_uses_x0, float* z_out);

int cd_ddim_decode(cd_handle h, int net, int sched_kind, const float* z, int z_slots, int n_eps,
                   const float* ctx_c, const float* ctx_uc, int ctx_len, float guidance, int B, int K,
                   const cd_step_coef* coef_host, const float* noise_tail, uint64_t seed, float* x_out);

int cd_ddim_decode_v(cd_handle h, int net, int sched_kind, const float* z, int z_slots, int n_eps,
                     const float* ctx_c, const float* ctx_uc, int ctx_len, const float* guidance_per_sample, int B,
                     int K, const cd_step_coef* coef_host, const float* noise_tail, uint64_t seed, float* x_out);

int cd_ddim_invert(cd_handle h, int net, int sched_kind, const float* x0, const float* ctx_c, const float* ctx_uc,
                   int ctx_len, float guidance, int B, int K, const cd_step_coef* coef_host, float* x_out,
                   float* traj_out);

int cd_cycle_translate(cd_handle h, int net, int sched_kind, const float* x0, const float* enc_ctx_c,
                       const float* enc_ctx_uc, float enc_guidance, const float* dec_ctx_c, const float* dec_ctx_uc,
                       float dec_guidance, const float* dec_guidance_per_sample, int ctx_len, int B, int n_dec, int K,
                       const cd_step_coef* coef_enc_host, const cd_step_coef* coef_dec_host, const float* noise,
                       uint64_t seed, int last_uses_x0, float* z_out, float* x_out);

int cd_ddim_decode_masked(cd_handle h, int net, int sched_kind, const float* z, int z_slots, int n_eps, const float* ctx_c,
                          const float* ctx_uc, int ctx_len, float guidance, const float* guidance_per_sample, int B, int K,
                          const cd_step_coef* coef_host, const float* noise_tail, uint64_t seed, const float* mask,
                          const float* x0, int B_mask, int mask_source, const float* qsample_coef_host,
                          const float* mask_noise, uint64_t mask_seed, float* x_out);

int cd_cycle_translate_masked(cd_handle h, int net, int sched_kind, const float* x0, const float* enc_ctx_c,
                              const float* enc_ctx_uc, float enc_guidance, const float* dec_ctx_c, const float* dec_ctx_uc,
                              float dec_guidance, const float* dec_guidance_per_sample, int ctx_len, int B, int n_dec, int K,
                              const cd_step_coef* coef_enc_host, const cd_step_coef* coef_dec_host, const float* noise,
                              uint64_t seed, int last_uses_x0, const float* mask, const float* mask_x0, int B_mask,
                              int mask_source, const float* qsample_coef_host, const float* mask_noise, uint64_t mask_seed,
                              float* z_out, float* x_out);

int cd_pix_refine(cd_handle h, int net, int sched_kind, float* x, int B, int R,
                  const cd_step_coef* coef_host, const float* noise, uint64_t seed);

int cd_op_pack_conv_weight(cd_handle h, const float* w_host, int N, int Cin, int KH, int KW, int geglu,
                           void** packed_dev, int* Npad, int* Cpad);
int cd_op_free(cd_handle h, void* dev);
int cd_op_conv2d(cd_handle h, const float* x0, int C0, const float* x1, int C1, int B, int H, int W,
                 const void* packed_w, int N, int KH, int KW, int stride, int pad, int asym_pad, int up,
                 const float* bias, const float* rowvec, const float* resid, int act, int tile, float* y);
int cd_op_conv2d_16(cd_handle h, const float* x0, int C0, const float* x1, int C1, int B, int H, int W,
                    const void* packed_w, int N, int KH, int KW, int stride, int pad, int asym_pad, int up,
                    const float* bias, const float* rowvec, const float* resid, int act, int tile, float* y,
                    float* stats);
int cd_op_last_gemm_config(cd_handle h, int* tile_id, int* bk, int* splitk, int* chm, int* tile_group);
int cd_op_groupnorm(cd_handle h, const float* x, int B, int C, int H, int W, int G, float eps,
                    const float* gamma, const float* beta, const float* film, int silu, float* y);
int cd_op_layernorm(cd_handle h, const float* x, int rows, int C, const float* gamma, const float* beta,
                    float eps, float* y);
int cd_op_attention(cd_handle h, const float* q, const float* k, const float* v, int B, int H, int Tq,
                    int Tk, int D, float scale, int use_transpose_kernel, float* o);
int cd_op_softmax_rows(cd_handle h, const float* s, int64_t rows, int cols, float* p);
int cd_op_timestep_embedding(cd_handle h, const float* t, int B, int dim, int mode, float* out);
int cd_op_sched_step(cd_handle h, int mode, int sched_kind, const cd_step_coef* coef_host, const float* x0,
                     float* xt, const float* eps_hat, int cfg, float guidance, const float* noise,
                     const float* eps_in, int is_last, int B, int C, int HW, float* z_slot);
int cd_op_sched_step_masked(cd_handle h, int mode, const cd_step_coef* coef_host, float* x, const float* eps_hat, int cfg,
                            float guidance, const float* eps_in, const float* mask, const float* src, int B_mask,
                            int mask_source, float qa, float qb, const float* mask_noise, int blend, int B, int C, int HW,
                            void* xin16_out, int cfg_dup);
int cd_op_bench_conv(cd_handle h, int B, int H, int W, int C0, int C1, int N, int k, int stride, int up,
                     int act, int tile, int iters, float* ms_out);
int cd_op_bench_mfma_sustained(cd_handle h, int target_ms, float* tflops_out, float* ghz_out);
int cd_op_probe(cd_handle h, int which, const void* in, void* out, size_t n);

#ifdef __cplusplus
}
#endif
#endif
```

Before: 3.431 images/s.

## Compute nearest-upsample 3x3 convs as four 2x2 phase convolutions

Replaces the upsample-then-3x3-conv path in U-Net up blocks with a polyphase decomposition. Each of the four output phases is a 2x2 conv on the low-resolution input using pre-summed weights, run as one GEMM with M covering all phases, followed by a reorder kernel that interleaves the phases into the high-resolution output. This cuts conv FLOPs from 9 to 4 taps per output and avoids reading the upsampled input. In exchange it adds a temporary buffer, an extra reorder pass, weight preprocessing refreshed on each parameter version, and bf16 rounding of the summed weights.

```diff
diff --git a/cycle-diffusion_amd/_ffi.py b/cycle-diffusion_amd/_ffi.py
--- a/cycle-diffusion_amd/_ffi.py
+++ b/cycle-diffusion_amd/_ffi.py
@@ -78,6 +78,7 @@
     "cd_op_conv2d_16": [_VP, _VP, _I, _VP, _I, _I, _I, _I, _VP, _I, _I, _I, _I, _I, _I, _I, _VP, _VP, _VP, _I, _I, _VP,
                         _VP],
     "cd_op_last_gemm_config": [_VP] + [C.POINTER(_I)] * 5,
+    "cd_op_up_phase_reorder": [_VP, _VP, _I, _I, _I, _I, _VP],
     "cd_op_groupnorm": [_VP, _VP, _I, _I, _I, _I, _I, _F, _VP, _VP, _VP, _I, _VP],
     "cd_op_layernorm": [_VP, _VP, _I, _I, _VP, _VP, _F, _VP],
     "cd_op_attention": [_VP, _VP, _VP, _VP, _I, _I, _I, _I, _I, _F, _I, _VP],
diff --git a/cycle-diffusion_amd/csrc/capi.hip b/cycle-diffusion_amd/csrc/capi.hip
--- a/cycle-diffusion_amd/csrc/capi.hip
+++ b/cycle-diffusion_amd/csrc/capi.hip
@@ -874,6 +874,11 @@
   CD_CHECK(h && x0 && packed_w && y, "bad argument");
   ArenaScope arena_scope(h->arena);
   Ctx c = h->ctx();
+  if (up && out16) {
+    ConvW* pw = (ConvW*)const_cast<void*>(packed_w);
+    h->op_params.add_up_phase(pw);
+    h->op_params.refresh_up_phase(h->st, pw);
+  }
   ConvW w = *(const ConvW*)packed_w;
   CD_CHECK(w.N == N && w.KH == KH && w.KW == KW, "packed weight does not match the call");
   w.b = const_cast<float*>(bias);
@@ -932,6 +937,20 @@
   enter_engine(h);
   op_conv2d(h, x0, C0, x1, C1, B, H, W, packed_w, N, KH, KW, stride, pad, asym_pad, up, bias, rowvec, resid, act, tile,
             true, y, stats);
+  CD_API_END
+}
+
+int cd_op_up_phase_reorder(cd_handle h, const float* x, int B, int C, int H, int W, float* y) {
+  CD_API_BEGIN
+  enter_engine(h);
+  CD_CHECK(h && x && y && B > 0 && H > 0 && W > 0 && C > 0 && C % 8 == 0, "bad argument");
+  ArenaScope arena_scope(h->arena);
+  Ctx c = h->ctx();
+  Act a = alloc_act(c, 4 * B, H, W, C);
+  launch_nchw_to_nhwc(h->st, x, a.p, 4 * B, C, H * W, C, 1.f, 0.f, 0);
+  Act o = alloc_act(c, B, 2 * H, 2 * W, C);
+  launch_up_phase_reorder(h->st, a.p, o.p, B, H, W, C, o.ld);
+  launch_nhwc_to_nchw(h->st, o.p, 0, o.ld, y, B, C, 4 * H * W, 1.f, 0.f);
   CD_API_END
 }
 
diff --git a/cycle-diffusion_amd/csrc/conv_gemm.hip b/cycle-diffusion_amd/csrc/conv_gemm.hip
--- a/cycle-diffusion_amd/csrc/conv_gemm.hip
+++ b/cycle-diffusion_amd/csrc/conv_gemm.hip
@@ -157,11 +157,18 @@
   const int sh_hw = 31 - __builtin_clz(HWo), sh_w = 31 - __builtin_clz(p.Wout);
   int b_first = pow2 ? (m0 >> sh_hw) : (m0 / HWo);
   CD_PROBE_ONLY(if (p.dbg & 4) b_first = 0;)
+  int pad_t = p.pad_t, pad_l = p.pad_l, w_ph = 0;
+  if (p.up_phase) {
+    const int ph = b_first & 3;
+    b_first >>= 2;
+    pad_t = 1 - (ph >> 1); pad_l = 1 - (ph & 1);
+    w_ph = ph * p.w_ps;
+  }
   const int64_t samp0 = (int64_t)b_first * p.Hs * p.Ws;
   const bf16_t* base0 = p.src0 + (int64_t)zb * p.a_bs + samp0 * p.ld0;
   const bf16_t* base1 = p.src1 ? p.src1 + (int64_t)zb * p.a_bs + samp0 * p.ld1 : base0;
   const __amdgpu_buffer_rsrc_t rsw =
-      __builtin_amdgcn_make_buffer_rsrc((void*)(p.wgt + (int64_t)zb * p.w_bs), 0, kRange, 0x00020000);
+      __builtin_amdgcn_make_buffer_rsrc((void*)(p.wgt + (int64_t)zb * p.w_bs + w_ph), 0, kRange, 0x00020000);
 
   const int srow = lane / CPR;
   const int pchunk = lane % CPR;
@@ -187,8 +194,9 @@
         const int rem = m - b * HWo;
         oy = rem / p.Wout; ox = rem - oy * p.Wout;
       }
-      a_iy0[i] = oy * p.stride - p.pad_t;
-      a_ix0[i] = ox * p.stride - p.pad_l;
+      if (p.up_phase) b >>= 2;
+      a_iy0[i] = oy * p.stride - pad_t;
+      a_ix0[i] = ox * p.stride - pad_l;
       a_boff[i] = (b - b_first) * p.Hs * p.Ws;
     } else {
       a_iy0[i] = -(1 << 28);
@@ -859,7 +867,7 @@
 
 inline bool takes_channel_major(const ConvGemmParams& p) {
   const int64_t a_bytes = (int64_t)p.B * p.Hs * p.Ws * (p.C0 + p.C1) * 2;
-  return p.korder != 0 && p.KH * p.KW > 1 && p.KH <= 8 && p.KW <= 8 && !p.up &&
+  return p.korder != 0 && p.KH * p.KW > 1 && p.KH <= 8 && p.KW <= 8 && !p.up && !p.up_phase &&
          (p.korder == 2 || (p.Hs * p.Ws >= 4096 && a_bytes >= (32ll << 20)));
 }
 
@@ -1107,7 +1115,7 @@
   const int nout = (p.act == ACT_GEGLU) ? p.N / 2 : p.N;
   const size_t need = (size_t)p.M * nout * (p.out_f32 ? 4 : 2) * p.nbatch;
   if (need > tu.scratch_bytes) return pick_config(p);
-  ShapeKey key = {{p.M, p.N, p.Ktot, p.KH, p.C0, p.C1, p.stride, p.up, p.act, p.nbatch, p.out_f32, p.Hout, p.Wout,
+  ShapeKey key = {{p.M, p.N, p.Ktot, p.KH, p.C0, p.C1, p.stride, p.up | (p.up_phase << 1), p.act, p.nbatch, p.out_f32, p.Hout, p.Wout,
                    (p.resid ? 1 : 0) | (p.rowvec ? 2 : 0)}};
   auto& tab = tune_table();
   auto it = tab.find(key);
@@ -1194,6 +1202,10 @@
   CD_CHECK(((uintptr_t)p.src0 & 15) == 0 && ((uintptr_t)p.wgt & 15) == 0, "conv_gemm: 16-B alignment");
   CD_CHECK((p.ld0 % 8) == 0 && (p.src1 == nullptr || (p.ld1 % 8) == 0), "conv_gemm: ld must be a multiple of 8");
   if (p.act == ACT_GEGLU) CD_CHECK(p.N % 64 == 0, "GEGLU needs packed N %% 64 == 0");
+  if (p.up_phase)
+    CD_CHECK(p.KH == 2 && p.KW == 2 && p.stride == 1 && !p.up && !p.src1 && p.nbatch == 1 && p.Hout == p.Hs && p.Wout == p.Ws &&
+                 (p.Hs * p.Ws) % 256 == 0 && p.M == 4 * p.B * p.Hs * p.Ws && p.w_ps > 0 && p.Hin == p.Hs && p.Win == p.Ws,
+             "conv_gemm: phase form of an x2 conv on %d x %d", p.Hs, p.Ws);
   bool k64 = (p.C0 % 64 == 0) && (p.C1 % 64 == 0);
   if (p.ln_fold) CD_CHECK(p.tile == kLinStreamTile, "conv_gemm: a LayerNorm-folded layer runs on lin_stream only");
   int id = p.tile ? p.tile : tuned_config(st, p, k64);
@@ -1240,7 +1252,7 @@
   static const bool trace = [] { const char* e = getenv("CYCLEDIFF_GEMM_TRACE"); return e && e[0] == '1'; }();
   if (trace) {
     const bool chm = id != kLinStreamTile && takes_channel_major(pk);
-    fprintf(stderr, "[gemm_trace] %d %d %d %d %d %d %d %d %d %d %d %d | %s x%d\n", p.M, p.N, p.Ktot, p.KH, p.stride, p.up,
+    fprintf(stderr, "[gemm_trace] %d %d %d %d %d %d %d %d %d %d %d %d | %s x%d\n", p.M, p.N, p.Ktot, p.KH, p.stride, p.up | (p.up_phase << 1),
             p.src1 ? 1 : 0, p.nbatch, p.act, p.resid ? 1 : 0, p.out_f32, chm ? 1 : 0, ci->name, pk.splitk > 1 ? pk.splitk : 1);
   }
   KernelProfiler* prof = g_conv_prof;
@@ -1249,7 +1261,7 @@
     char what[112] = "";
     if (prof->verbose)
       snprintf(what, sizeof(what), "M%d N%d K%d k%d s%d%s%s z%d act%d | %s x%d", p.M, p.N, p.Ktot, p.KH, p.stride,
-               p.up ? " up" : "", p.src1 ? " cat" : "", p.nbatch, p.act, ci->name, pk.splitk > 1 ? pk.splitk : 1);
+               p.up ? " up" : (p.up_phase ? " up-phase" : ""), p.src1 ? " cat" : "", p.nbatch, p.act, ci->name, pk.splitk > 1 ? pk.splitk : 1);
     if (prof->verbose && !k64) strncat(what, " bk32", sizeof(what) - strlen(what) - 1);
     prof->next_pair(&e0, &e1, 2.0 * (double)p.M * (double)p.N * (double)p.Ktot * (double)p.nbatch * p.prof_flop_scale,
                     what);
@@ -1291,6 +1303,32 @@
   }
 }
 
+__global__ void k_up_phase_weights(const bf16_t* __restrict__ w, bf16_t* __restrict__ out, int Npad, int Cpad) {
+  const int64_t total = (int64_t)16 * Npad * Cpad;
+  for (int64_t i = blockIdx.x * (int64_t)blockDim.x + threadIdx.x; i < total;
+       i += (int64_t)gridDim.x * blockDim.x) {
+    const int c = (int)(i % Cpad);
+    int64_t t = i / Cpad;
+    const int dx = (int)(t & 1), dy = (int)((t >> 1) & 1); t >>= 2;
+    const int n = (int)(t % Npad);
+    const int ph = (int)(t / Npad);
+    const int a = ph >> 1, b = ph & 1;
+    const int r0 = dy ? 1 + a : 0, r1 = dy ? 2 : a;
+    const int s0 = dx ? 1 + b : 0, s1 = dx ? 2 : b;
+    float v = 0.0f;
+    for (int r = r0; r <= r1; ++r)
+      for (int s = s0; s <= s1; ++s) v += bf2f(w[((int64_t)n * 9 + r * 3 + s) * Cpad + c]);
+    out[i] = f2bf(v);
+  }
+}
+
+void launch_up_phase_weights(hipStream_t st, const bf16_t* w, bf16_t* out, int Npad, int Cpad) {
+  const int64_t total = (int64_t)16 * Npad * Cpad;
+  int grid = (int)((total + 255) / 256);
+  if (grid > 4096) grid = 4096;
+  hipLaunchKernelGGL(k_up_phase_weights, dim3(grid), dim3(256), 0, st, w, out, Npad, Cpad);
+}
+
 void launch_repack_weight(hipStream_t st, const float* w, bf16_t* out, int N, int Cin, int KH,
                           int KW, int Npad, int Cpad, int geglu, int64_t src_row_offset) {
   const int64_t total = (int64_t)Npad * KH * KW * Cpad;
diff --git a/cycle-diffusion_amd/csrc/elementwise.hip b/cycle-diffusion_amd/csrc/elementwise.hip
--- a/cycle-diffusion_amd/csrc/elementwise.hip
+++ b/cycle-diffusion_amd/csrc/elementwise.hip
@@ -222,6 +222,22 @@
   }
 }
 
+__global__ void k_up_phase_reorder(const bf16_t* __restrict__ x, bf16_t* __restrict__ y, int B, int H, int W, int C, int ldy) {
+  const int Ho = H * 2, Wo = W * 2, nvec = C / 8;
+  const int64_t n = (int64_t)B * Ho * Wo * nvec;
+  for (int64_t i = blockIdx.x * (int64_t)blockDim.x + threadIdx.x; i < n;
+       i += (int64_t)gridDim.x * blockDim.x) {
+    const int v = (int)(i % nvec);
+    int64_t t = i / nvec;
+    const int ox = (int)(t % Wo); t /= Wo;
+    const int oy = (int)(t % Ho);
+    const int b = (int)(t / Ho);
+    const int ph = (oy & 1) * 2 + (ox & 1);
+    *(uint4*)(y + (((int64_t)b * Ho + oy) * Wo + ox) * ldy + v * 8) =
+        *(const uint4*)(x + ((((int64_t)b * 4 + ph) * H + (oy >> 1)) * W + (ox >> 1)) * C + v * 8);
+  }
+}
+
 __global__ void k_posterior_sample(const float* __restrict__ mom, int ld, const float* __restrict__ noise,
                                    uint64_t seed, float* __restrict__ z, int B, int zc, int HW,
                                    float scale, int use_mean) {
@@ -327,6 +343,11 @@
   const int64_t n = (int64_t)B * (H / 2) * (W / 2) * (C / 8);
   hipLaunchKernelGGL(k_avgpool2, dim3(ew_grid(n)), dim3(256), 0, st, x, y, B, H, W, C);
 }
+void launch_up_phase_reorder(hipStream_t st, const bf16_t* x, bf16_t* y, int B, int H, int W, int C, int ldy) {
+  CD_CHECK(C % 8 == 0 && ldy % 8 == 0 && (((uintptr_t)x | (uintptr_t)y) & 15) == 0, "up_phase_reorder: 16-byte vectors");
+  const int64_t n = (int64_t)B * H * 2 * W * 2 * (C / 8);
+  hipLaunchKernelGGL(k_up_phase_reorder, dim3(ew_grid(n)), dim3(256), 0, st, x, y, B, H, W, C, ldy);
+}
 void launch_upsample2(hipStream_t st, const bf16_t* x, bf16_t* y, int B, int H, int W, int C) {
   const int64_t n = (int64_t)B * H * 2 * W * 2 * (C / 8);
   hipLaunchKernelGGL(k_upsample2, dim3(ew_grid(n)), dim3(256), 0, st, x, y, B, H, W, C);
diff --git a/cycle-diffusion_amd/csrc/engine.h b/cycle-diffusion_amd/csrc/engine.h
--- a/cycle-diffusion_amd/csrc/engine.h
+++ b/cycle-diffusion_amd/csrc/engine.h
@@ -41,6 +41,8 @@
   bf16_t* w = nullptr;
   bf16_t* wfrag = nullptr;
   bf16_t* w3 = nullptr;
+  bf16_t* wphase = nullptr;
+  int wphase_version = -1;
   bool f32 = false;
   float* b = nullptr;
   int N = 0, Cin = 0, Cpad = 0, KH = 1, KW = 1, Npad = 0;
@@ -76,6 +78,8 @@
   int version = 0;
   ConvW* new_conv(int N, int Cin, int KH, int KW, bool bias, bool geglu = false);
   float* new_vec(int n, float init = 0.f);
+  void add_up_phase(ConvW* c);
+  void refresh_up_phase(hipStream_t st, ConvW* c);
   ParamDecl& declare(const std::string& name, std::vector<int64_t> shape);
   void conv_weight(const std::string& name, ConvW* c, int ref_ndim = 0, float scale = 1.f);
   void conv_weight_t(const std::string& name, ConvW* c);
@@ -138,6 +142,7 @@
 Act split_rows_f32_fwd(Ctx& c, const Act& x, const Act* x2 = nullptr);
 Act alloc_act(Ctx& c, int B, int H, int W, int C, bool with_stats = false);
 Act conv_fwd(Ctx& c, const ConvW& w, const Act& x, const Act* x2, const ConvOpts& o);
+bool conv_up_phase_taken(const Ctx& c, const ConvW& w, const Act& x, const Act* x2, const ConvOpts& o);
 bool conv_ln_fold_available(const Ctx& c, const ConvW& w, int64_t rows);
 
 struct GNW { float* g = nullptr; float* b = nullptr; int C = 0; float eps = 1e-5f; };
diff --git a/cycle-diffusion_amd/csrc/engine.hip b/cycle-diffusion_amd/csrc/engine.hip
--- a/cycle-diffusion_amd/csrc/engine.hip
+++ b/cycle-diffusion_amd/csrc/engine.hip
@@ -46,6 +46,16 @@
   if (f32 && x3) c->w3 = (bf16_t*)dmalloc((size_t)c->Npad * c->Ktot() * 3 * sizeof(bf16_t));
   if (bias) c->b = (float*)dmalloc((size_t)c->Npad * sizeof(float));
   return c;
+}
+void ParamStore::add_up_phase(ConvW* c) {
+  if (f32 || c->wphase || c->KH != 3 || c->KW != 3 || c->geglu) return;
+  c->wphase = (bf16_t*)dmalloc((size_t)4 * c->Npad * 4 * c->Cpad * sizeof(bf16_t));
+  c->wphase_version = -1;
+}
+void ParamStore::refresh_up_phase(hipStream_t st, ConvW* c) {
+  if (!c->wphase || c->wphase_version == version) return;
+  launch_up_phase_weights(st, c->w, c->wphase, c->Npad, c->Cpad);
+  c->wphase_version = version;
 }
 float* ParamStore::new_vec(int n, float init) {
   float* p = (float*)dmalloc((size_t)n * sizeof(float));
@@ -267,7 +277,45 @@
   return y;
 }
 
+bool conv_up_phase_taken(const Ctx& c, const ConvW& w, const Act& x, const Act* x2, const ConvOpts& o) {
+  if (!o.up || c.f32 || x.split || x2 || !w.wphase || w.KH != 3 || w.KW != 3 || o.stride != 1 || o.pad != 1 || o.asym ||
+      o.resid || o.out_f32 || o.ln_fold || w.geglu || o.act != ACT_NONE)
+    return false;
+  if ((x.H * x.W) % 256 != 0 || w.N % 8 != 0 || (o.out && o.out_ld % 8 != 0)) return false;
+  const char* e = getenv("CYCLEDIFF_UP_PHASE");
+  return !(e && e[0] == '0');
+}
+
+static Act conv_up_phase_fwd(Ctx& c, const ConvW& w, const Act& x, const ConvOpts& o) {
+  ConvGemmParams p;
+  p.src0 = x.p; p.C0 = round_up(x.C, 32); p.ld0 = x.ld;
+  CD_CHECK(p.C0 == w.Cpad && x.ld >= p.C0, "conv: input channels %d do not match weight Cpad %d", p.C0, w.Cpad);
+  p.B = x.B; p.Hs = x.H; p.Ws = x.W; p.Hin = x.H; p.Win = x.W; p.Hout = x.H; p.Wout = x.W;
+  p.KH = 2; p.KW = 2; p.stride = 1; p.pad_t = 1; p.pad_l = 1;
+  p.up_phase = 1; p.w_ps = w.Npad * 4 * w.Cpad;
+  p.M = 4 * x.B * x.H * x.W;
+  p.wgt = w.wphase; p.Ktot = 4 * w.Cpad; p.N = w.N;
+  p.alpha = o.alpha; p.bias = w.b;
+  p.rowvec = o.rowvec; p.rowvec_ld = o.rowvec_ld; p.rows_per_vec = o.rows_per_vec;
+  Act y; y.B = x.B; y.H = 2 * x.H; y.W = 2 * x.W; y.C = w.N; y.f32 = false;
+  if (o.out) { y.p = (bf16_t*)o.out; y.ld = o.out_ld; }
+  else { y.ld = w.N; y.p = (bf16_t*)c.arena->alloc((size_t)p.M * w.N * 2); }
+  if (o.out && o.out_stats) y.stats_buf = o.out_stats;
+  else if (!o.out && o.want_stats) y.stats_buf = (float*)c.arena->alloc((size_t)(p.M / 32) * 2 * w.N * sizeof(float));
+  p.stats = y.stats_buf;
+  y.stats = y.stats_buf;
+  const size_t mk = c.arena->mark();
+  bf16_t* tmp = (bf16_t*)c.arena->alloc((size_t)p.M * w.N * 2);
+  p.out = tmp; p.out_ld = w.N;
+  p.zeros = c.zeros; p.tile = o.tile;
+  launch_conv_gemm(c.st, p);
+  launch_up_phase_reorder(c.st, tmp, y.p, x.B, x.H, x.W, w.N, y.ld);
+  c.arena->release(mk);
+  return y;
+}
+
 Act conv_fwd(Ctx& c, const ConvW& w, const Act& x, const Act* x2, const ConvOpts& o) {
+  if (conv_up_phase_taken(c, w, x, x2, o)) return conv_up_phase_fwd(c, w, x, o);
   if (x.split) {
     CD_CHECK(!x2, "conv: a split activation cannot be concatenated");
     return conv_split_fwd(c, w, x, o);
diff --git a/cycle-diffusion_amd/csrc/kernels.h b/cycle-diffusion_amd/csrc/kernels.h
--- a/cycle-diffusion_amd/csrc/kernels.h
+++ b/cycle-diffusion_amd/csrc/kernels.h
@@ -97,6 +97,8 @@
   int dephase_ticks = 0;
   int num_cus = 256;
   int dbg = 0;
+  int up_phase = 0;
+  int w_ps = 0;
 };
 constexpr int kProbeWords = 48;
 extern thread_local unsigned long long* g_conv_probe;
@@ -117,6 +119,7 @@
   int tile_group = 0;
 };
 GemmLaunchInfo conv_gemm_last_launch();
+void launch_up_phase_weights(hipStream_t st, const bf16_t* w, bf16_t* out, int Npad, int Cpad);
 int conv_gemm_num_configs();
 const char* conv_gemm_config_name(int id);
 
@@ -224,6 +227,7 @@
                        float* y, int ldy, int B, int K, int N, int silu_in, int silu_out);
 void launch_avgpool2(hipStream_t st, const bf16_t* x, bf16_t* y, int B, int H, int W, int C);
 void launch_upsample2(hipStream_t st, const bf16_t* x, bf16_t* y, int B, int H, int W, int C);
+void launch_up_phase_reorder(hipStream_t st, const bf16_t* x, bf16_t* y, int B, int H, int W, int C, int ldy);
 void launch_posterior_sample(hipStream_t st, const float* mom, int ld, const float* noise,
                              uint64_t seed, float* z, int B, int zc, int HW, float scale,
                              int use_mean);
diff --git a/cycle-diffusion_amd/csrc/unet_openai.hip b/cycle-diffusion_amd/csrc/unet_openai.hip
--- a/cycle-diffusion_amd/csrc/unet_openai.hip
+++ b/cycle-diffusion_amd/csrc/unet_openai.hip
@@ -252,7 +252,7 @@
         Layer u;
         const std::string up = pfx + "." + std::to_string(sub);
         if (d.resblock_updown) { u.kind = Layer::RES; u.idx = add_res_named(up, ch, ch, true, false); }
-        else { u.kind = Layer::UP_CONV; u.conv = make_conv(params, up + ".conv", ch, ch, 3, true); }
+        else { u.kind = Layer::UP_CONV; u.conv = make_conv(params, up + ".conv", ch, ch, 3, true); params.add_up_phase(u.conv); }
         b.layers.push_back(u);
         ds /= 2;
       }
@@ -598,6 +598,9 @@
 
 void UNetOpenAI::refresh_ln_folds(Ctx& c) {
   if (folded_version_ == params.version) return;
+  for (const Block& b : out_blocks_)
+    for (const Layer& l : b.layers)
+      if (l.kind == Layer::UP_CONV) params.refresh_up_phase(c.st, l.conv);
   for (STW& s : st_) {
     if (!s.q2_ln) continue;
     struct { const ConvW* src; ConvW* dst; const LNW* ln; } jobs[2] = {{s.q2, s.q2_ln, &s.ln2}, {s.ff1, s.ff1_ln, &s.ln3}};
diff --git a/include/cyclediff.h b/include/cyclediff.h
--- a/include/cyclediff.h
+++ b/include/cyclediff.h
@@ -121,6 +121,7 @@
                     const float* bias, const float* rowvec, const float* resid, int act, int tile, float* y,
                     float* stats);
 int cd_op_last_gemm_config(cd_handle h, int* tile_id, int* bk, int* splitk, int* chm, int* tile_group);
+int cd_op_up_phase_reorder(cd_handle h, const float* x, int B, int C, int H, int W, float* y);
 int cd_op_groupnorm(cd_handle h, const float* x, int B, int C, int H, int W, int G, float eps,
                     const float* gamma, const float* beta, const float* film, int silu, float* y);
 int cd_op_layernorm(cd_handle h, const float* x, int rows, int C, const float* gamma, const float* beta,
```

Result: faster. 3.509 images/s (median of 6 runs) (+2.3%).
